# groupeLIAMG/ttcr

Hardware: AMD Instinct MI355X
Metric: Mnodes/s per sweep-iteration (512^3 fp32 grid, first-order FSM) (higher is better)
Workload: dtype f32

## Files before the change

### include/ttcr_amd.h

```cpp
#ifndef TTCR_AMD_H
#define TTCR_AMD_H

#include <stddef.h>
#include <stdint.h>

#ifdef __cplusplus
extern "C" {
#endif

typedef struct ttcr_fsm_grid ttcr_fsm_grid;

enum { TTCR_F32 = 0, TTCR_F64 = 1 };

enum {
    TTCR_OK = 0,
    TTCR_ERR_VALUE = 1,
    TTCR_ERR_RUNTIME = 2,
    TTCR_ERR_DEVICE = 3,
    TTCR_ERR_UNSUPPORTED = 4
};

int ttcr_fsm_device_count(void);

const char* ttcr_fsm_last_error(void);
// ... 142 lines not shown
                        int dtt_on_device, void* dfields, int df_on_device, int schedule, int* passes);
int ttcr_fsm_rjoint_gn(const ttcr_fsm_adjoint* t, const void* v, int v_on_device, const void* v_rcv, int vr_on_device, const void* row_weight,
                       int rw_on_device, const double* rcv_scale, void* out, int out_on_device, void* out_rcv, int or_on_device,
                       int schedule, int* passes_jvp, int* passes_vjp);
int ttcr_fsm_rjoint_solve(ttcr_fsm_adjoint* t, const void* rhs, int rhs_on_device, const void* rhs_rcv, int rr_on_device,
                          const void* row_weight, int rw_on_device, double smooth, const double* smooth_weights, double damp,
                          const double* rcv_damp, const double* rcv_scale, int maxiter, double rtol, int schedule, void* x,
                          int x_on_device, void* x_rcv, int xr_on_device, int* status, int* iterations, double* rho, double* pq, int* passes);
int ttcr_fsm_rcv_release(ttcr_fsm_adjoint* t);

int ttcr_fsm_loc_geometry(const ttcr_fsm_adjoint* t, int* nn, double* dx, double* origin);
int ttcr_fsm_loc_shape(const ttcr_fsm_adjoint* t, int* node_tile, int* hypo_chunk, int* staged);
int ttcr_fsm_loc_grid(const ttcr_fsm_adjoint* t, size_t n_hypo, const long long* hypo_off, const int* pick_field, const double* pick_time,
                      const double* pick_weight, const int* box, long long* node_out, double* t0_out, double* misfit_out,
                      void* volume_out, int volume_on_device);
int ttcr_fsm_loc_release(ttcr_fsm_adjoint* t);

int ttcr_fsm_dd_pairs(ttcr_fsm_adjoint* t, const int* set_row_a, const int* set_row_b, size_t set_n_pairs, size_t* n_pairs, int* row_a,
                      int* row_b, long long* bad_pair);
int ttcr_fsm_dd_apply(const ttcr_fsm_adjoint* t, int mode, const void* x, int x_on_device, const void* row_weight, int rw_on_device,
                      const void* pair_weight, int pw_on_device, void* out, int out_on_device);
int ttcr_fsm_dd_gn(const ttcr_fsm_adjoint* t, int system, int newton, const void* v, int v_on_device, const void* v_b, int vb_on_device,
                   const void* row_weight, int rw_on_device, const void* pair_weight, int pw_on_device, const double* b_scale, void* out,
                   int out_on_device, void* out_b, int ob_on_device, int schedule, int* passes_jvp, int* passes_vjp);
int ttcr_fsm_dd_solve(ttcr_fsm_adjoint* t, int system, const void* rhs, int rhs_on_device, const void* rhs_b, int rb_on_device,
                      const void* row_weight, int rw_on_device, const void* pair_weight, int pw_on_device, double smooth,
                      const double* smooth_weights, double damp, const double* b_damp, const double* b_scale, const void* x0,
                      int x0_on_device, int maxiter, double rtol, int newton, int schedule, void* x, int x_on_device, void* x_b,
                      int xb_on_device, int* status, int* iterations, double* rho, double* pq, int* passes);
int ttcr_fsm_dd_release(ttcr_fsm_adjoint* t);

int ttcr_fsm_raytrace_l(ttcr_fsm_grid* g, int slot, int n_tx, const void* tx, const void* t0, int n_rx,
                        const void* rx, void* tt_out, int with_rays);
int ttcr_fsm_slot_l_size(const ttcr_fsm_grid* g, int slot, size_t* n_rows, size_t* nnz);
int ttcr_fsm_get_slot_l(const ttcr_fsm_grid* g, int slot, long long* row_off, long long* cell, void* v);
int ttcr_fsm_raytrace_multi_l(ttcr_fsm_grid* g, int n_src, const int* tx_off, const void* tx, const void* t0, const int* rx_off,
                              const void* rx, void* tt_out, int with_rays);
int ttcr_fsm_multi_l_size(const ttcr_fsm_grid* g, size_t* n_rows, size_t* nnz);
int ttcr_fsm_get_multi_l(const ttcr_fsm_grid* g, long long* row_off, long long* cell, void* v);

typedef struct {
    double sweep_ms;
    double total_ms;
    long long kernel_launches;
    long long node_updates;
    long long evaluated_updates;
    int iterations;
    int n_sources;
} ttcr_fsm_timing;
int ttcr_fsm_last_timing(const ttcr_fsm_grid* g, ttcr_fsm_timing* out);
int ttcr_fsm_stopping_stats(const ttcr_fsm_grid* g, long long* reference_sums, long long* reference_sums_missed, long long* rounds);
int ttcr_fsm_prefill_swaps(const ttcr_fsm_grid* g, long long* swaps);
int ttcr_fsm_prefill_inline_fills(const ttcr_fsm_grid* g, long long* fills);
int ttcr_fsm_reference_change(ttcr_fsm_grid* g, const void* times, const void* field, int parallel, void* out);
int ttcr_fsm_last_kernel(const ttcr_fsm_grid* g, char* buf, size_t n);
int ttcr_fsm_unit_order(int dim, int dtype, int stage, int by_time, uint32_t nnx, uint32_t nny, uint32_t nnz, uint32_t* out,
                        size_t capacity, size_t* n_units);
int ttcr_fsm_prefill_slice(int dtype, uint64_t n_el, uint32_t n_tickets, uint32_t ticket, uint64_t* slice_len, uint64_t* begin, uint64_t* end);
const char* ttcr_fsm_build_id(void);

#ifdef __cplusplus
}
#endif
#endif
```

### ttcr_amd/_lib.py

```python
import ctypes as C
import os

HERE = os.path.dirname(os.path.abspath(__file__))
LIB_PATH = os.environ.get("TTCR_AMD_LIB") or os.path.join(HERE, "libttcr_amd.so")

TTCR_F32, TTCR_F64 = 0, 1
OK, ERR_VALUE, ERR_RUNTIME, ERR_DEVICE, ERR_UNSUPPORTED = 0, 1, 2, 3, 4

_P = C.c_void_p
_U32 = C.c_uint32
_D = C.c_double
_I = C.c_int


class Timing(C.Structure):
    _fields_ = [("sweep_ms", C.c_double), ("total_ms", C.c_double), ("kernel_launches", C.c_longlong),
                ("node_updates", C.c_longlong), ("evaluated_updates", C.c_longlong), ("iterations", C.c_int),
                ("n_sources", C.c_int)]


SYMBOLS = {
    "ttcr_fsm_device_count": (_I, []),
    "ttcr_fsm_last_error": (C.c_char_p, []),
    "ttcr_fsm3d_create": (_I, [C.POINTER(_P), _I, _I, _U32, _U32, _U32, _D, _D, _D, _D, _D, _I, _I, _I, _I, _I]),
    "ttcr_fsm2d_create": (_I, [C.POINTER(_P), _I, _I, _U32, _U32, _D, _D, _D, _D, _D, _I, _I, _I, _I, _I]),
    "ttcr_fsm3d_create_multi": (_I, [C.POINTER(_P), _I, _I, _U32, _U32, _U32, _D, _D, _D, _D, _D, _I, _I, _I, _I, C.POINTER(_I), _I]),
    "ttcr_fsm2d_create_multi": (_I, [C.POINTER(_P), _I, _I, _U32, _U32, _D, _D, _D, _D, _D, _I, _I, _I, _I, C.POINTER(_I), _I]),
    "ttcr_fsm_n_devices": (_I, [_P]),
    "ttcr_fsm_destroy": (None, [_P]),
    "ttcr_fsm_set_slowness": (_I, [_P, _P, C.c_size_t]),
    "ttcr_fsm_set_slowness_device": (_I, [_P, _P, C.c_size_t]),
    "ttcr_fsm_set_slowness_c_order": (_I, [_P, _P, C.c_size_t]),
    "ttcr_fsm_get_slowness": (_I, [_P, _P, C.c_size_t]),
    "ttcr_fsm_raytrace": (_I, [_P, _I, _I, _P, _P, _I, _P, _P]),
    "ttcr_fsm_raytrace_multi": (_I, [_P, _I, _P, _P, _P, _P, _P, _P]),
    "ttcr_fsm_get_tt": (_I, [_P, _I, _P, C.c_size_t]),
    "ttcr_fsm_get_tt_device": (_I, [_P, _I, C.POINTER(_P)]),
    "ttcr_fsm_get_tt_device_view": (_I, [_P, _I, C.POINTER(_P), C.POINTER(C.c_size_t)]),
    "ttcr_fsm_interp": (_I, [_P, _I, _I, _P, _P]),
    "ttcr_fsm_compute_slowness": (_I, [_P, _I, _P, _I, _P]),
    "ttcr_fsm_get_niter": (_I, [_P, _I, C.POINTER(_I), C.POINTER(_I)]),
    "ttcr_fsm_get_changes": (_I, [_P, _I, C.POINTER(_D), _I, C.POINTER(_D), _I]),
    "ttcr_fsm_get_reference_changes": (_I, [_P, _I, C.POINTER(_D), _I, C.POINTER(_D), _I]),
    "ttcr_fsm_n_slots": (_I, [_P]),
    "ttcr_fsm_n_nodes": (C.c_size_t, [_P]),
    "ttcr_fsm_n_cells": (C.c_size_t, [_P]),
    "ttcr_fsm_set_option": (_I, [_P, C.c_char_p, _D]),
    "ttcr_fsm_last_timing": (_I, [_P, C.POINTER(Timing)]),
    "ttcr_fsm_last_kernel": (_I, [_P, C.c_char_p, C.c_size_t]),
    "ttcr_fsm_build_id": (C.c_char_p, []),
    "ttcr_fsm_unit_order": (_I, [_I, _I, _I, _I, _U32, _U32, _U32, C.POINTER(_U32), C.c_size_t, C.POINTER(C.c_size_t)]),
    "ttcr_fsm_stopping_stats": (_I, [_P, C.POINTER(C.c_longlong), C.POINTER(C.c_longlong), C.POINTER(C.c_longlong)]),
    "ttcr_fsm_prefill_swaps": (_I, [_P, C.POINTER(C.c_longlong)]),
    "ttcr_fsm_prefill_inline_fills": (_I, [_P, C.POINTER(C.c_longlong)]),
    "ttcr_fsm_prefill_slice": (_I, [_I, C.c_uint64, _U32, _U32, C.POINTER(C.c_uint64), C.POINTER(C.c_uint64), C.POINTER(C.c_uint64)]),
    "ttcr_fsm_reference_change": (_I, [_P, C.c_void_p, C.c_void_p, C.c_int, C.c_void_p]),
    "ttcr_fsm_rays_size": (_I, [_P, C.POINTER(C.c_size_t), C.POINTER(C.c_size_t)]),
    "ttcr_fsm_get_rays": (_I, [_P, _P, _P]),
    "ttcr_fsm_raytrace_rays": (_I, [_P, _I, _I, _P, _P, _I, _P, _P]),
    "ttcr_fsm_slot_rays_size": (_I, [_P, _I, C.POINTER(C.c_size_t), C.POINTER(C.c_size_t)]),
    "ttcr_fsm_get_slot_rays": (_I, [_P, _I, _P, _P]),
    "ttcr_fsm_raytrace_m": (_I, [_P, _I, _I, _P, _P, _I, _P, _P]),
    "ttcr_fsm_raytrace_rm": (_I, [_P, _I, _I, _P, _P, _I, _P, _P]),
    "ttcr_fsm_raytrace_multi_m": (_I, [_P, _I, _P, _P, _P, _P, _P, _P, _I]),
    "ttcr_fsm_multi_m_size": (_I, [_P, C.POINTER(C.c_size_t), C.POINTER(C.c_size_t)]),
    "ttcr_fsm_get_multi_m": (_I, [_P, _P, _P, _P]),
    "ttcr_fsm_raytrace_multi_tape": (_I, [_P, _I, _P, _P, _P, _P, _P, _P, C.POINTER(_P)]),
    "ttcr_fsm_tape_size": (_I, [_P, C.POINTER(C.c_size_t), C.POINTER(C.c_size_t), C.POINTER(C.c_size_t)]),
    "ttcr_fsm_tape_bytes": (_I, [_P, C.POINTER(C.c_size_t)]),
    "ttcr_fsm_tape_device": (_I, [_P, C.POINTER(_I)]),
    "ttcr_fsm_tape_get_csr": (_I, [_P, _P, _P, _P]),
    "ttcr_fsm_tape_vjp": (_I, [_P, _P, _I, _P, _I]),
    "ttcr_fsm_tape_free": (_I, [_P]),
    "ttcr_fsm_raytrace_multi_adjoint": (_I, [_P, _I, _P, _P, _P, _P, _P, _P, C.POINTER(_P)]),
    "ttcr_fsm_raytrace_multi_adjoint_cells": (_I, [_P, _I, _P, _P, _P, _P, _P, _P, C.POINTER(_P)]),
    "ttcr_fsm_adjoint_model": (_I, [_P, C.POINTER(_I), C.POINTER(C.c_size_t), C.POINTER(C.c_size_t)]),
    "ttcr_fsm_adjoint_size": (_I, [_P, C.POINTER(C.c_size_t), C.POINTER(C.c_size_t), C.POINTER(C.c_size_t)]),
    "ttcr_fsm_adjoint_bytes": (_I, [_P, C.POINTER(C.c_size_t)]),
    "ttcr_fsm_adjoint_device": (_I, [_P, C.POINTER(_I)]),
    "ttcr_fsm_adjoint_get_field": (_I, [_P, C.c_size_t, _P]),
    "ttcr_fsm_adjoint_vjp": (_I, [_P, _P, _I, _P, _I, _P, _I, _I, C.POINTER(_I)]),
    "ttcr_fsm_adjoint_jvp": (_I, [_P, _P, _I, _P, _I, _P, _I, _I, C.POINTER(_I)]),
    "ttcr_fsm_adjoint_gn": (_I, [_P, _P, _I, _P, _I, _P, _I, _I, C.POINTER(_I), C.POINTER(_I)]),
    "ttcr_fsm_adjoint_points": (_I, [_P, C.POINTER(C.c_size_t), _P]),
    "ttcr_fsm_adjoint_jvp_source": (_I, [_P, _P, _I, _I, _P, _I, _P, _I, _I, C.POINTER(_I)]),
    "ttcr_fsm_adjoint_vjp_source": (_I, [_P, _P, _I, _P, _I, _P, _I, _P, _I, _I, C.POINTER(_I)]),
    "ttcr_fsm_adjoint_hold": (_I, [_P, _P, _I, _P, _I, _P, _I, _I, C.POINTER(_I)]),
    "ttcr_fsm_adjoint_release": (_I, [_P]),
    "ttcr_fsm_adjoint_hvp": (_I, [_P, _P, _I, _P, _I, _I, C.POINTER(_I), C.POINTER(_I)]),
    "ttcr_fsm_adjoint_newton": (_I, [_P, _P, _I, _P, _I, _P, _I, _I, C.POINTER(_I), C.POINTER(_I)]),
    "ttcr_fsm_adjoint_jvp_block": (_I, [_P, _I, _P, _I, _P, _I, _P, _I, _I, C.POINTER(_I)]),
    "ttcr_fsm_adjoint_vjp_block": (_I, [_P, _I, _P, _I, _P, _I, _I, C.POINTER(_I)]),
    "ttcr_fsm_adjoint_gn_block": (_I, [_P, _I, _P, _I, _P, _I, _I, _P, _I, _I, C.POINTER(_I), C.POINTER(_I)]),
    "ttcr_fsm_adjoint_block_release": (_I, [_P]),
    "ttcr_fsm_adjoint_free": (_I, [_P]),
    "ttcr_fsm_normal_tile_edge": (_I, [_I]),
    "ttcr_fsm_normal_smooth": (_I, [_P, _P, _I, C.POINTER(_D), _P, _I]),
    "ttcr_fsm_normal_dot": (_I, [_P, _P, _I, _P, _I, C.POINTER(_D)]),
    "ttcr_fsm_normal_solve": (_I, [_P, _P, _I, _P, _I, _D, C.POINTER(_D), _D, _P, _I, _I, _D, _I, _I, _P, _I, C.POINTER(_I),
                                   C.POINTER(_I), C.POINTER(_D), C.POINTER(_D), C.POINTER(_I)]),
    "ttcr_fsm_normal_release": (_I, [_P]),
    "ttcr_fsm_joint_jvp": (_I, [_P, _P, _I, _P, _I, _P, _I, _P, _I, _I, C.POINTER(_I)]),
    "ttcr_fsm_joint_gn": (_I, [_P, _P, _I, _P, _I, _P, _I, C.POINTER(_D), _P, _I, _P, _I, _I, C.POINTER(_I), C.POINTER(_I)]),
    "ttcr_fsm_joint_solve": (_I, [_P, _P, _I, _P, _I, _P, _I, _D, C.POINTER(_D), _D, C.POINTER(_D), C.POINTER(_D), _I, _D, _I, _P, _I, _P, _I,
                                  C.POINTER(_I), C.POINTER(_I), C.POINTER(_D), C.POINTER(_D), C.POINTER(_I)]),
    "ttcr_fsm_joint_release": (_I, [_P]),
    "ttcr_fsm_rcv_eval": (_I, [_P, C.c_size_t, _P, _I, C.POINTER(_I), _P, _I, _P, _I]),
# ... 84 lines not shown
```

### ttcr_amd/csrc/fsm_capi.hip

```cpp
#include <hip/hip_runtime.h>

#include <algorithm>
#include <atomic>
#include <chrono>
#include <condition_variable>
#include <cmath>
#include <cstdio>
#include <cstdlib>
#include <cstring>
#include <limits>
#include <map>
#include <memory>
#include <mutex>
#include <sstream>
#include <stdexcept>
#include <string>
#include <thread>
#include <vector>

#include "../../include/ttcr_amd.h"
#include "fsm_kernels.h"
#include "fsm_fast_api.h"
#include "fsm_tape_api.h"
#include "fsm_adjoint_api.h"
// ... 78 lines not shown
                                     void* tt_out, TapeRows& out) = 0;
    virtual void raytrace_multi_adjoint(int n_src, const int* tx_off, const void* tx, const void* t0, const int* rx_off, const void* rx,
                                        void* tt_out, AdjSink& sink) = 0;
    virtual void adjoint_geometry(int* nn3, double* spacing, bool wrt_cells) const = 0;
    AdjSink* adj_sink = nullptr;
    std::vector<int> adj_src, adj_row;
    virtual void raytrace_l(int slot, int n_tx, const void* tx, const void* t0, int n_rx, const void* rx, void* tt_out, bool with_rays) = 0;
    virtual void slot_l_size(int slot, size_t* n_rows, size_t* nnz) const = 0;
    virtual void get_slot_l(int slot, long long* row_off, long long* cell, void* v) const = 0;
    virtual void raytrace_multi_l(int n_src, const int* tx_off, const void* tx, const void* t0, const int* rx_off, const void* rx,
                                  void* tt_out, bool with_rays) = 0;
    virtual void multi_l_size(size_t* n_rows, size_t* nnz) const = 0;
    virtual void get_multi_l(long long* row_off, long long* cell, void* v) const = 0;
    virtual void validate_points(int n_tx, const void* tx, int n_rx, const void* rx) = 0;
    struct Request {
        int slot, n_tx, n_rx;
        const void *tx, *t0, *rx;
        void* tt;
        int status = TTCR_OK;
        std::string err;
        bool done = false;
    };
    std::mutex q_mu;
    std::condition_variable q_cv;
    std::vector<Request*> queue;
    bool leader_active = false;
    bool had_company = false;
    std::atomic<int> combine_window_us{200};
    size_t elem_size = 4;
    virtual void get_tt(int slot, void* out, size_t n) = 0;
    virtual void* tt_device(int slot) = 0;
    virtual void* tt_device_view(int slot, size_t* stride) = 0;
    std::mutex mu;
    virtual void interp(int slot, int n, const void* pts, void* out) = 0;
    virtual void compute_slowness(int n, const void* pts, bool translated, void* out) = 0;
    virtual void rays_size(size_t* n_rays, size_t* n_points) const = 0;
    virtual void get_rays(long long* offsets, void* pts) const = 0;
    int dim = 3, dtype = 0, n_slots = 1, device = 0;
    size_t n_nodes = 0, n_cells = 0;
    std::vector<int> niter, niterw;
    std::vector<int> phys;
    int P(int slot) const { return phys.empty() ? slot : phys[slot]; }
    int stopping_shortcuts = 3;
    int stopping_rule = 1;
    long long reference_sums = 0, reference_sums_missed = 0;
    long long refsum_rounds = 0;
    virtual void stopping_stats(long long* sums, long long* missed, long long* rounds) const {
        if (sums) *sums = reference_sums;
        if (missed) *missed = reference_sums_missed;
        if (rounds) *rounds = refsum_rounds;
    }
    virtual void reference_change_host(const void* times, const void* field, bool parallel, void* out) = 0;
    int pair_by_distance = 1;
    virtual void set_pair_layout(int) {}
    virtual long long prefill_inline_count() const { return 0; }
    virtual long long prefill_swap_count() const { return 0; }
    int lone_chunk = 16;
    int arith = 0;
    int prefill = -1;
    int prefill_inline = -1;
    std::vector<std::vector<double>> change_hist, change_histw;
    std::vector<std::vector<double>> ref_hist, ref_histw;
    virtual void get_reference_changes(int slot, double* first, int n_first, double* wen, int n_weno) const {
        if (slot < 0 || slot >= n_slots) throw ValueError("Thread number is larger than number of threads");
        slot = P(slot);
        for (int q = 0; q < n_first; ++q) first[q] = (!ref_hist.empty() && q < (int)ref_hist[slot].size()) ? ref_hist[slot][q] : std::nan("");
        for (int q = 0; q < n_weno; ++q) wen[q] = (!ref_histw.empty() && q < (int)ref_histw[slot].size()) ? ref_histw[slot][q] : std::nan("");
    }
    virtual void get_changes(int slot, double* first, int n_first, double* wen, int n_weno) const {
        if (slot < 0 || slot >= n_slots) throw ValueError("Thread number is larger than number of threads");
        slot = P(slot);
        for (int q = 0; q < n_first; ++q) first[q] = (!change_hist.empty() && q < (int)change_hist[slot].size()) ? change_hist[slot][q] : 0.0;
        for (int q = 0; q < n_weno; ++q) wen[q] = (!change_histw.empty() && q < (int)change_histw[slot].size()) ? change_histw[slot][q] : 0.0;
    }
    bool weno = false;
    bool sweep45_strips = false;
    bool rotated = false;
    int ttrp = 0, interp_vel = 0;
    std::atomic<int> return_rays{0};
    int fixed_iters = 0, max_batch = 0, use_graph = 1;
    int skip = -1;
    int mode = 2;
    Timing timing;
    std::string last_kernel;
    virtual std::string kernel_name() const { return last_kernel; }
    long walk_step_limit = 1000000;
    long walk_records = 0;
    long walk_room(long extent) const { return std::min<long>(walk_step_limit, walk_records > 0 ? walk_records : extent); }
    virtual void apply_option(const std::string& k, double value) {
        if (k == "fixed_iters") fixed_iters = (int)value;
        else if (k == "max_batch") max_batch = (int)value;
        else if (k == "use_graph") use_graph = (int)value;
        else if (k == "combine_window_us") combine_window_us = (int)value;
        else if (k == "mode") mode = (int)value;
        else if (k == "skip") skip = (int)value;
        else if (k == "tt_from_rp") ttrp = value != 0;
        else if (k == "interp_vel") interp_vel = value != 0;
        else if (k == "return_rays") return_rays = value != 0;
        else if (k == "pair_sources") pair_by_distance = value != 0;
        else if (k == "pair_layout") {
            if (value != -1 && value != 0 && value != 1) throw ValueError("option 'pair_layout': -1 (default), 0 or 1");
            set_pair_layout((int)value);
        }
        else if (k == "stopping_rule") stopping_rule = (int)value;
        else if (k == "stopping_shortcuts") { if (value < 0 || value > 3 || value != (double)(int)value) throw ValueError("option stopping_shortcuts: 0 ... 3"); stopping_shortcuts = (int)value; }
        else if (k == "prefill") {
            if (value != -1 && value != 0 && value != 1) throw ValueError("option 'prefill': -1 (default), 0 or 1");
            prefill = (int)value;
        } else if (k == "prefill_inline") {
            if (value != -1 && value != 0 && value != 1) throw ValueError("option 'prefill_inline': -1 (default), 0 or 1");
            prefill_inline = (int)value;
        } else if (k == "lone_chunk") {
            if (value != 8 && value != 16) throw ValueError("option 'lone_chunk': 8 or 16");
            lone_chunk = (int)value;
        }
        else if (k == "arith") {
            if (value != 0 && value != 1 && value != 2)
                throw ValueError("option 'arith': 0 (the reference's arithmetic), 1 (tolerance-grade fp32 where it stays within 1e-5 s RMS) or 2 (the WENO stage as well)");
            arith = (int)value;
        }
        else if (k == "walk_records") {
            if (value != 0 && !(value >= 1 && value <= (double)walk_step_limit && value == (double)(long)value))
                throw ValueError("option 'walk_records': 0 (default) or a whole number from 1 to the step limit of a walk");
            walk_records = (long)value;
        }
        else throw ValueError("unknown option '" + k + "'");
    }
    virtual void get_niter(int slot, int* it, int* itw) const {
        if (slot < 0 || slot >= n_slots) throw ValueError("Thread number is larger than number of threads");
        if (it) *it = niter[P(slot)];
        if (itw) *itw = niterw[P(slot)];
    }
};

template <typename T, int DIM> struct TileCfg;
#ifndef FSM_PJ3
#define FSM_PJ3 16
#endif
#ifndef FSM_PK3
#define FSM_PK3 16
#endif
template <> struct TileCfg<float, 3> { static constexpr int PJ = FSM_PJ3, PK = FSM_PK3, BL = 16; };
template <> struct TileCfg<double, 3> { static constexpr int PJ = 16, PK = 8, BL = 16; };
#ifndef FSM_PJ2
#define FSM_PJ2 64
#endif
#ifndef FSM_CHUNK2
#define FSM_CHUNK2 16
#endif
template <> struct TileCfg<float, 2> { static constexpr int PJ = FSM_PJ2, PK = 1, BL = 32; };
template <> struct TileCfg<double, 2> { static constexpr int PJ = FSM_PJ2, PK = 1, BL = 32; };
template <typename T, int DIM> struct ChunkCfg { static constexpr int C = DIM == 3 ? FSM_CHUNK3 : FSM_CHUNK2; };

template <typename T>
class GridT : public GridBase {
   public:
    uint32_t ncx, ncy, ncz;
    T dx, dz, xmin, ymin, zmin, xmax, ymax, zmax, ox = 0, oy = 0, oz = 0;
    T epsilon;
    int nitermax;
    bool cell, translate;
    bool have_slowness = false;

    hipStream_t stream = nullptr;
    hipEvent_t ev0 = nullptr, ev1 = nullptr;
    DevBuf<T> d_s, d_cells, d_tt, d_rx, d_out;
    DevBuf<T> d_tt_alt;
    bool alt_filled = false;
    hipStream_t fill_stream = nullptr;
    hipEvent_t ev_fill = nullptr;
    long long prefill_swaps = 0;
    long long prefill_swap_count() const override { return prefill_swaps; }
    long long prefill_inline_fills = 0;
    long long prefill_inline_count() const override { return prefill_inline_fills; }
    void set_pair_layout(int v) override { pair_layout = v; }
    DevBuf<int> d_rslot;
    DevBuf<RaySrc> d_rdesc;
    int weno_ch4_min = 8;
    int weno_c16_below = 3;
    int f64_c16_below = 5;
    int pre_min = 2;
    size_t xs_lds_bytes = 40000;
    int xs_lds_below = 2;
    size_t xs_dyn_lds(int batch) const { return (dim == 3 && stage == 0 && batch < xs_lds_below) ? xs_lds_bytes : 0; }
    int time_order_below = 1 << 30;
    DevBuf<T> d_gather;
    DevBuf<T> d_rsrc, d_rt0;
    DevBuf<int> d_rstat;
    DevBuf<T> d_ssh;
    size_t ssh_stride = 0;
    DevBuf<uint32_t> d_mask;
    DevBuf<int> d_bbox, d_slots, d_lmask;
    int* h_lmask = nullptr;
    DevBuf<uint32_t> d_tiles;
    std::vector<int> tile_off, tile_cnt;
    DevBuf<double> d_change;
    DevBuf<unsigned long long> d_prof;
    size_t prof_words = 0;
    DevBuf<uint32_t> d_order;
    DevBuf<uint32_t> d_order_xs[2][2];
    DevBuf<int> d_sync;
    int n_patches = 0;
    int* h_abort = nullptr;
    DevBuf<int> d_stamp;
    DevBuf<unsigned long long> d_cmap;
    int cmap_words = 1;
    DevBuf<unsigned long long> d_sw;
    int sw_sweeps = 0;
    DevBuf<int> d_iter;
    DevBuf<unsigned long long> d_evals;
    int* h_iter = nullptr;
    unsigned launch_epoch = 1;
    bool sync_clean = true;
    size_t sync_words = 0;
    unsigned long long* h_evals = nullptr;
    int nbf = 0, nbj = 0, nbk = 0;
    size_t n_bricks = 0;
    DevBuf<InitPoint<T>> d_pts;
    double* h_change = nullptr;
    int* h_slots = nullptr;
    size_t mask_words = 0;
    SweepGeom geom;
    int n_launch = 0;
    hipGraph_t graphs[2] = {nullptr, nullptr};
    hipGraphExec_t graph_execs[2] = {nullptr, nullptr};
    int graph_batches[2] = {0, 0}, graph_modes[2] = {-1, -1};

    GridT(int dim_, bool cell_, uint32_t nx, uint32_t ny, uint32_t nz, double ddx, double ddz, double minx,
          double miny, double minz, double eps, int maxit, int nslots, bool translate_, int dev, bool weno_) {
        dim = dim_;
        weno = weno_;
        dtype = sizeof(T) == 4 ? TTCR_F32 : TTCR_F64;
        elem_size = sizeof(T);
        cell = cell_;
        translate = translate_;
        ncx = nx; ncy = ny; ncz = nz;
        dx = (T)ddx;
        dz = (T)ddz;
        xmin = (T)minx; ymin = (T)miny; zmin = (T)minz;
        xmax = xmin + (T)nx * dx;
        if (dim == 3) {
            ymax = ymin + (T)ny * dx;
            zmax = zmin + (T)nz * dx;
        } else {
            ymax = ymin;
            zmax = zmin + (T)nz * dz;
        }
        if (translate) {
            ox = xmin; oy = ymin; oz = zmin;
            xmax -= xmin; ymax -= ymin; zmax -= zmin;
            xmin = 0; ymin = 0; zmin = 0;
        }
        n_nodes = dim == 3 ? (size_t)(nx + 1) * (ny + 1) * (nz + 1) : (size_t)(nx + 1) * (nz + 1);
        n_cells = dim == 3 ? (size_t)nx * ny * nz : (size_t)nx * nz;
        if (n_nodes >= (1ull << 32)) throw ValueError("grid too large: node index must fit uint32 (reference T2)");
        epsilon = (T)eps;
        epsilon *= (T)n_nodes;
        nitermax = maxit;
        n_slots = nslots;
        niter.assign(n_slots, 0);
        niterw.assign(n_slots, 0);
        phys.resize(n_slots);
        for (int q = 0; q < n_slots; ++q) phys[q] = q;
        max_batch = n_slots;
        device = dev;
        HIP_CHECK(hipSetDevice(device));
        {
            int cus = 0;
            HIP_CHECK(hipDeviceGetAttribute(&cus, hipDeviceAttributeMultiprocessorCount, device));
            persist_wgs = 8 * std::max(cus, 1);
        }
        HIP_CHECK(hipStreamCreateWithFlags(&stream, hipStreamNonBlocking));
        HIP_CHECK(hipEventCreate(&ev0));
        HIP_CHECK(hipEventCreate(&ev1));
        d_s.reserve(n_nodes, 64);
        {
            long long pair_units_min = 6144;
            if (const char* e = std::getenv("TTCR_FSM_PAIR_UNITS")) pair_units_min = std::atoll(e);
            const long long patches = dim == 3 ? (long long)((ny + 1 + TileCfg<T, 3>::PJ - 1) / TileCfg<T, 3>::PJ) * ((nz + 1 + TileCfg<T, 3>::PK - 1) / TileCfg<T, 3>::PK) : 0;
            NS = (n_slots >= 2 && dim == 3 && !weno && (long long)n_slots * patches > pair_units_min) ? 2 : 1;
            ns_window = NS == 2 && (long long)n_slots * patches <= (5 * pair_units_min) / 2;
        }
        if (const char* e = std::getenv("TTCR_FSM_PAIR")) { NS = (std::atoi(e) != 0 && n_slots >= 2) ? 2 : 1; ns_window = false; }
        if (const char* e = std::getenv("TTCR_FSM_LAYOUT_LO")) layout_lo = std::atof(e);
        if (const char* e = std::getenv("TTCR_FSM_LAYOUT_HI")) layout_hi = std::atof(e);
        d_tt.reserve(n_nodes * tt_fields(), 64);
        mask_words = (n_nodes + 31) / 32;
        d_mask.reserve(mask_words * (size_t)n_slots);
        d_bbox.reserve(6 * (size_t)n_slots);
        d_slots.reserve(n_slots);
        d_lmask.reserve(n_slots);
        HIP_CHECK(hipHostMalloc((void**)&h_lmask, sizeof(int) * n_slots));
        d_change.reserve(n_slots);
        if (std::getenv("TTCR_FSM_PROF")) {
            prof_words = 8 + 4 * (size_t)(1 << 20);
            d_prof.reserve(prof_words);
            HIP_CHECK(hipMemset(d_prof.p, 0, prof_words * sizeof(unsigned long long)));
        }
        HIP_CHECK(hipHostMalloc((void**)&h_change, sizeof(double) * n_slots));
        HIP_CHECK(hipHostMalloc((void**)&h_slots, sizeof(int) * n_slots));
        HIP_CHECK(hipHostMalloc((void**)&h_abort, sizeof(int)));
        *h_abort = 0;
        HIP_CHECK(hipHostMalloc((void**)&h_iter, 2 * sizeof(int)));
        HIP_CHECK(hipHostMalloc((void**)&h_evals, sizeof(unsigned long long) * n_slots));
        HIP_CHECK(hipMemsetAsync(d_tt.p, 0, n_nodes * tt_fields() * sizeof(T), stream));

        if (dim == 3) {
            using C = TileCfg<T, 3>;
            geom.NF = nx + 1; geom.NJ = ny + 1; geom.NK = nz + 1;
            geom.npj = (geom.NJ + C::PJ - 1) / C::PJ;
            geom.npk = (geom.NK + C::PK - 1) / C::PK;
            n_launch = count_launches(C::BL);
        } else {
            using C = TileCfg<T, 2>;
            geom.NF = nz + 1; geom.NJ = nx + 1; geom.NK = 1;
            geom.npj = (geom.NJ + C::PJ - 1) / C::PJ;
            geom.npk = 1;
            n_launch = count_launches(C::BL);
        }
        geom.n_nodes = (uint32_t)n_nodes;
        geom.M = (std::max(geom.NF, geom.NJ) + 1) & ~1;
        geom.MP = geom.M + FSM_XPAD;
        geom.SR = dim == 3 ? ((geom.NJ + 15) / 16) * 32 : 0;
        ssh_stride = (size_t)geom.NK * shear_plane(geom);
        if ((double)(dim == 3 ? 16 : 1) * (double)shear_plane(geom) * sizeof(T) >= 4294967296.0)
            throw ValueError("grid too large for the slowness offsets of the sweep kernel (16 planes of max(nx, ny) x ny nodes must stay below 4 GiB)");
        d_ssh.reserve(ssh_stride * (dim == 3 ? 4 : 2));
        HIP_CHECK(hipMemsetAsync(d_ssh.p, 0, ssh_stride * (dim == 3 ? 4 : 2) * sizeof(T), stream));
        if (dim == 3) build_tile_lists(TileCfg<T, 3>::PJ, TileCfg<T, 3>::PK, TileCfg<T, 3>::BL);
        else build_tile_lists(TileCfg<T, 2>::PJ, TileCfg<T, 2>::PK, TileCfg<T, 2>::BL);
        build_persistent_lists();
        nbf = (geom.NF + FSM_BRICK - 1) / FSM_BRICK;
        nbj = (geom.NJ + FSM_BRICK - 1) / FSM_BRICK;
        nbk = (geom.NK + FSM_BRICK - 1) / FSM_BRICK;
        n_bricks = (size_t)nbf * nbj * nbk;
        d_stamp.reserve(n_bricks * n_slots);
        {
            const int PJ = dim == 3 ? TileCfg<T, 3>::PJ : TileCfg<T, 2>::PJ, PK = dim == 3 ? TileCfg<T, 3>::PK : 1;
            const int max_chunks = (geom.NF + 2 * (PJ + PK)) / 4 + 4;
            cmap_words = max_chunks / 32 + 1;
            d_cmap.reserve((size_t)n_patches * n_slots * (dim == 3 ? 8 : 4) * 2 * cmap_words);
            HIP_CHECK(hipMemset(d_cmap.p, 0, (size_t)n_patches * n_slots * (dim == 3 ? 8 : 4) * 2 * cmap_words * sizeof(unsigned long long)));
            sw_sweeps = (dim == 3 ? 8 : 4) * (2 * std::min(nitermax, 256) + 2);
            d_sw.reserve((size_t)sw_sweeps * n_slots);
        }
        d_iter.reserve(2);
        d_evals.reserve(n_slots);
        if (dim == 2)
            HIP_CHECK(hipFuncSetAttribute(reinterpret_cast<const void*>(&fsm_sweep45_rows<T>),
                                          hipFuncAttributeMaxDynamicSharedMemorySize, 156 * 1024));
        if (const char* e = std::getenv("TTCR_FSM_SWEEP45")) sweep45_strips = std::string(e) == "strips";
        if (const char* e = std::getenv("TTCR_FSM_WENO_CH4_MIN")) weno_ch4_min = std::atoi(e);
        if (const char* e = std::getenv("TTCR_FSM_WENO_C16_BELOW")) weno_c16_below = std::atoi(e);
        if (const char* e = std::getenv("TTCR_FSM_F64_C16_BELOW")) f64_c16_below = std::atoi(e);
        if (const char* e = std::getenv("TTCR_FSM_TIME_ORDER_BELOW")) time_order_below = std::atoi(e);
        if (const char* e = std::getenv("TTCR_FSM_PRE_MIN")) pre_min = std::atoi(e);
        if (const char* e = std::getenv("TTCR_FSM_SKIP")) skip = std::atoi(e);
        if (const char* e = std::getenv("TTCR_FSM_SKIP_UNITS")) skip_units_min = std::atoi(e);
        if (const char* e = std::getenv("TTCR_FSM_SKIP_PROBE_UNITS")) skip_probe_min = std::atoi(e);
        if (const char* e = std::getenv("TTCR_FSM_RS_FIELDS")) rs_fields_max = (size_t)std::max(0, std::atoi(e));
        if (const char* e = std::getenv("TTCR_FSM_WGS")) persist_wgs = std::atoi(e);
        if (const char* e = std::getenv("TTCR_FSM_XS_LDS")) xs_lds_bytes = (size_t)std::atol(e);
        if (const char* e = std::getenv("TTCR_FSM_XS_LDS_BELOW")) xs_lds_below = std::atoi(e);
        if (const char* e = std::getenv("TTCR_FSM_MODE")) mode = std::atoi(e);
        if (const char* e = std::getenv("TTCR_FSM_PREFILL")) prefill = std::atoi(e);
        if (const char* e = std::getenv("TTCR_FSM_LONE_CHUNK")) lone_chunk = std::atoi(e) == 8 ? 8 : 16;
        if (const char* e = std::getenv("TTCR_FSM_ARITH")) arith = std::max(0, std::min(2, std::atoi(e)));
    }

    void build_persistent_lists() {
        const std::vector<uint32_t> order = fsm_diag_order(geom.npj, geom.npk);
        n_patches = (int)order.size();
        d_order.reserve(order.size());
        HIP_CHECK(hipMemcpy(d_order.p, order.data(), order.size() * sizeof(uint32_t), hipMemcpyHostToDevice));
        sync_words = 8 + (size_t)n_patches * n_slots * (dim == 3 ? 8 : 4);
        d_sync.reserve(sync_words);
        HIP_CHECK(hipMemset(d_sync.p, 0, sync_words * sizeof(int)));
        if (geom.npj >= (1 << 14) || geom.npk >= (1 << 14)) throw ValueError("grid too large for the patch index of the sweep kernel");
        for (int st = 0; st < 2; ++st)
            for (int tm = 0; tm < 2; ++tm) {
                const std::vector<uint32_t> xs = xs_order(order, tm != 0, st == 0 ? 1 : 2);
                d_order_xs[st][tm].reserve(xs.size());
                HIP_CHECK(hipMemcpy(d_order_xs[st][tm].p, xs.data(), xs.size() * sizeof(uint32_t), hipMemcpyHostToDevice));
            }
    }

    std::vector<uint32_t> xs_order(const std::vector<uint32_t>& diag_order, bool by_time, int H) const {
        const int PJ = dim == 3 ? TileCfg<T, 3>::PJ : TileCfg<T, 2>::PJ, PK = dim == 3 ? TileCfg<T, 3>::PK : 1;
        const int C = dim == 3 ? ChunkCfg<T, 3>::C : ChunkCfg<T, 2>::C;
        return fsm_xs_order(dim, geom.NF, geom.NJ, geom.NK, PJ, PK, C, H, by_time, diag_order);
    }

    template <int DIM, int H>
    void launch_sweeps_persistent(int batch) {
        constexpr int C0 = ChunkCfg<T, DIM>::C;
        if constexpr (DIM == 3 && C0 == 8) {
            const int below = H == 2 ? weno_c16_below : sizeof(T) == 4 ? std::numeric_limits<int>::max() : f64_c16_below;
            if (NS == 1 && mode == 2 && (lone_chunk == 16 || fast_now<H>()) && batch < below) {
                launch_sweeps_persistent_ns<DIM, H, 1, 16, true>(batch);
                return;
            }
        }
        if (H == 2 && DIM == 3 && NS == 2 && batch >= weno_ch4_min && C0 == 8) {
            if (NS == 2) launch_sweeps_persistent_ns<DIM, H, 2, (H == 2 && DIM == 3) ? 4 : C0>(batch);
            else launch_sweeps_persistent_ns<DIM, H, 1, (H == 2 && DIM == 3) ? 4 : C0>(batch);
        } else {
            if (NS == 2) launch_sweeps_persistent_ns<DIM, H, 2, C0>(batch); else launch_sweeps_persistent_ns<DIM, H, 1, C0>(batch);
        }
    }

    template <int DIM, int H, int NSV, int CH, bool XS_ONLY = false>
    void launch_sweeps_persistent_ns(int batch) {
        using C = TileCfg<T, DIM>;
        PersistArgs<T> pa;
        SweepArgs<T>& a = pa.s;
        constexpr bool NO_PRE = CH == 16 && H == 1 && DIM == 3;
        const size_t dyn_lds = NO_PRE ? 0 : xs_dyn_lds(batch);
        a.tt = d_tt.p;
        a.ts = NS;
        a.lmask = d_lmask.p;
        a.frozen = d_mask.p;
        a.bbox = d_bbox.p;
        a.change = d_change.p;
        a.slots = d_slots.p;
        a.tiles = nullptr;
        a.g = geom;
        a.prof = d_prof.p;
        a.mask_words = (uint32_t)mask_words;
        a.dx = dx;
        a.dz = dz;
        a.w = 0;
        a.variant = DIM == 3 ? 0 : (dx == dz ? 1 : 2);
        pa.order = d_order.p;
        pa.sync = d_sync.p;
        pa.n_patches = n_patches;
        pa.batch = batch;
        pa.timeout_ticks = 300000000ull;
        pa.stamp = d_stamp.p;
        pa.iter_ptr = d_iter.p;
        pa.evals = d_evals.p;
        pa.nbf = nbf; pa.nbj = nbj; pa.nbk = nbk;
        pa.ndir = DIM == 3 ? 8 : 4;
        pa.skip = skip_now(batch) ? (std::getenv("TTCR_FSM_SKIP_ALL_DIRTY") ? 2 : 1) : 0;
        pa.cmap = d_cmap.p;
        pa.cw = cmap_words;
        pa.sw = std::getenv("TTCR_FSM_NO_SW") ? nullptr : d_sw.p;
        pa.n_sw_groups = n_groups();
        pa.n_sw_sweeps = sw_sweeps;
        pa.fill_dst = nullptr;
        pa.fill_slice = 0;
        pa.fill_n = 0;

        const size_t wg_cap = (fsm_looped(DIM == 3, H) && persist_wgs > 0) ? (size_t)persist_wgs : ~(size_t)0;
        const dim3 block(C::PJ * C::PK), grid((unsigned)std::min<size_t>((size_t)n_patches * batch, wg_cap));
        const int ndir = DIM == 3 ? 8 : 4;
        {
            const bool pre_ = mode == 2 && !NO_PRE && (DIM == 2 || batch >= pre_min || dyn_lds > 0);
            char nm[160];
            std::snprintf(nm, sizeof nm, "fsm_sweep_persistent<%s,%d,%d,%d,%s,%s,%d,%d,%s,%s>", sizeof(T) == 4 ? "float" : "double", C::PJ, C::PK, CH,
                          DIM == 3 ? "true" : "false", skip_now(batch) ? "true" : "false", H, NSV, mode == 2 ? "true" : "false", pre_ ? "true" : "false");
            last_kernel = nm;
        }
        if (mode == 2) {
            pa.ssh = d_ssh.p;
            pa.ssh_stride = ssh_stride;
            pa.dir = 0;
            a.rf = a.rj = a.rk = a.rev = 0;
            a.s_sheared = nullptr;
            pa.timeout_ticks = 1000000000ull;
            const dim3 gridx((unsigned)std::min<size_t>((size_t)n_patches * batch * ndir, wg_cap));
            pa.order = d_order_xs[H == 2 ? 1 : 0][batch < time_order_below ? 1 : 0].p;
            const bool pre = DIM == 2 || batch >= pre_min || dyn_lds > 0;
            if (fill_arm) {
                pa.fill_dst = d_tt_alt.p;
                pa.fill_n = n_nodes * tt_fields();
                pa.fill_slice = fsm_fill_slice_len(pa.fill_n, (size_t)n_patches * batch * ndir, 16 / sizeof(T));
                fill_arm = false;
                fill_in_flight = true;
            }
            if constexpr (std::is_same<T, float>::value) {
                if (fast_now<H>() && (H == 1 || NSV == 1)) {
                    const FastCfg fc{H, DIM, NSV, CH, skip_now(batch), NO_PRE ? false : pre};
                    last_kernel.insert(last_kernel.size() - 1, ",1");
                    const hipError_t e = fsm_fast_launch(pa, fc, gridx.x, dyn_lds, stream);
                    if (e == hipErrorInvalidValue) throw std::logic_error("arith = 1: no such kernel (" + last_kernel + ")");
                    HIP_CHECK(e);
                    return;
                }
            }
            if constexpr (NO_PRE) {
                (void)pre;
                if (skip_now(batch))
                    fsm_sweep_persistent<T, C::PJ, C::PK, CH, DIM == 3, true, H, NSV, true><<<gridx, block, dyn_lds, stream>>>(pa);
                else
                    fsm_sweep_persistent<T, C::PJ, C::PK, CH, DIM == 3, false, H, NSV, true><<<gridx, block, dyn_lds, stream>>>(pa);
            } else {
                if (skip_now(batch) && pre)
                    fsm_sweep_persistent<T, C::PJ, C::PK, CH, DIM == 3, true, H, NSV, true, true><<<gridx, block, dyn_lds, stream>>>(pa);
// ... 248 lines not shown
                q.i = (int)(c / ncz);
                q.k = (int)(c - (long)q.i * ncz);
            }
        }
        return q;
    }

    template <int DIM>
    void launch_sweeps(int batch) {
        using C = TileCfg<T, DIM>;
        if (fast_now<1>()) throw ValueError("option 'arith' = 1 needs whole-iteration launches (option 'mode' = 2)");
        SweepArgs<T> a;
        a.tt = d_tt.p;
        a.ts = NS;
        a.lmask = nullptr;
        a.frozen = d_mask.p;
        a.bbox = d_bbox.p;
        a.change = d_change.p;
        a.slots = d_slots.p;
        a.g = geom;
        a.prof = d_prof.p;
        a.mask_words = (uint32_t)mask_words;
        a.dx = dx;
        a.dz = dz;
        a.variant = DIM == 3 ? 0 : (dx == dz ? 1 : 2);
        const dim3 block(C::PJ * C::PK);
        const int ndir = DIM == 3 ? 8 : 4;
        static const int RX2[4] = {0, 1, 1, 0}, RZ2[4] = {0, 0, 1, 1};
        for (int d = 0; d < ndir; ++d) {
            int fam;
            if (DIM == 3) {
                a.rf = d & 1; a.rj = (d >> 1) & 1; a.rk = (d >> 2) & 1;
                a.rev = a.rk;
                fam = (a.rf ^ a.rk) | ((a.rj ^ a.rk) << 1);
            } else {
                a.rj = RX2[d]; a.rf = RZ2[d]; a.rk = 0;
                a.rev = a.rj;
                fam = a.rf ^ a.rj;
            }
            a.s_sheared = d_ssh.p + (size_t)fam * ssh_stride;
            for (int w = 0; w < n_launch; ++w) {
                if (tile_cnt[w] == 0) continue;
                a.w = w;
                a.tiles = d_tiles.p + tile_off[w];
                const dim3 grid(tile_cnt[w], 1, batch);
                fsm_sweep_tile<T, C::PJ, C::PK, C::BL, DIM == 3><<<grid, block, 0, stream>>>(a);
            }
        }
        last_kernel = std::string("fsm_sweep_tile<") + (sizeof(T) == 4 ? "float" : "double") + "," + std::to_string(C::PJ) + "," + std::to_string(C::PK) + "," + std::to_string(C::BL) + "," + (DIM == 3 ? "true" : "false") + ">";
        HIP_CHECK(hipGetLastError());
    }

    int NS = 1;
    bool ns_window = false;
    int pair_layout = -1;
    double last_eval_frac = -1;
    double layout_lo = 0.55, layout_hi = 0.70;
    void choose_layout() {
        if (!ns_window) return;
        int want = NS;
        if (pair_layout >= 0) want = pair_layout ? 2 : 1;
        else if (last_eval_frac >= 0) want = NS == 2 ? (last_eval_frac < layout_lo ? 1 : 2) : (last_eval_frac > layout_hi ? 2 : 1);
        if (want == NS) return;
        NS = want;
        graph_batches[0] = graph_batches[1] = -1;
        for (int q = 0; q < n_slots; ++q) phys[q] = q;
    }
    int n_groups() const { return (n_slots + NS - 1) / NS; }
    size_t tt_fields() const { return (size_t)n_slots + ((ns_window || NS == 2) ? (size_t)(n_slots & 1) : 0); }
    T* tt_ptr(int slot) const { return d_tt.p + (size_t)(slot / NS) * n_nodes * NS + slot % NS; }
    template <int H>
    bool fast_now() const { return sizeof(T) == 4 && (arith == 2 || (arith == 1 && !weno)); }
    bool prefill_on() const {
        if (prefill >= 0) return prefill != 0;
        const size_t bytes = n_nodes * tt_fields() * sizeof(T);
        if (bytes < ((size_t)64 << 20)) return false;
        size_t free_b = 0, total_b = 0;
        if (hipMemGetInfo(&free_b, &total_b) != hipSuccess) return false;
        return d_tt_alt.p || (2 * bytes <= total_b / 2 && bytes + ((size_t)1 << 30) <= free_b);
    }
    bool fill_arm = false;
    bool fill_in_flight = false;
    bool inline_fill_now(int entries) const {
        if (prefill_inline == 0 || !d_tt_alt.p || d_tt_alt.n < n_nodes * tt_fields()) return false;
        if (mode != 2 || stage != 0 || use_graph >= 2) return false;
        if (prefill_inline == 1) return true;
        return dim == 3 && !fast_now<1>() && (long long)n_patches * entries >= skip_units_min;
    }

    int stage = 0;
    int skip_units_min = 2048;
    int skip_probe_min = 1024;
    bool probe_skip = true;
    int probe_off_calls = 0;
    int persist_wgs = 2048;
    bool in_probe_window(int entries) const {
        const long long u = (long long)n_patches * entries;
        return dim == 3 && sizeof(T) == 4 && u >= skip_probe_min && u < skip_units_min;
    }
    int skip_default(int entries) const {
        if (dim != 3) return 1;
        if (stage == 1) return 1;
        if (in_probe_window(entries)) return probe_skip ? 1 : 0;
        return (long long)n_patches * entries >= skip_units_min ? 1 : 0;
    }
    bool persistent_now() const { return mode >= 1 || stage == 1; }
// ... 1 lines not shown
        const int on = skip < 0 ? skip_default(entries) : skip;
        const bool fits = (long long)geom.NF + geom.NJ + geom.NK < (1ll << 22) && nbf <= 32 * FSM_SLAB_WORDS;
        return on != 0 && fits && !(dim == 2 && rotated && !weno && dx == dz);
    }

    void launch_sweep45(int batch) {
        Sweep45Args<T> a;
        a.tt = d_tt.p;
        a.s = d_s.p;
        a.frozen = d_mask.p;
        a.change = d_change.p;
        a.slots = d_slots.p;
        a.lmask = d_lmask.p;
        a.ts = NS;
        a.by_group = persistent_now() ? 1 : 0;
        a.nnx = (int)ncx + 1;
        a.nnz = (int)ncz + 1;
        a.n_nodes = n_nodes;
        a.mask_words = (uint32_t)mask_words;
        a.dx = dx;
        const int blocks = a.by_group ? batch * NS : batch;
        const size_t smem = 4 * ((size_t)a.nnz + 2) * sizeof(T);
        if (smem <= 156 * 1024 && !sweep45_strips) {
            const int threads = (int)std::min<size_t>(1024, (((size_t)a.nnz + 63) / 64) * 64);
            fsm_sweep45_rows<T><<<blocks, threads, smem, stream>>>(a);
        } else {
            constexpr int NTMAX = sizeof(T) == 4 ? 1024 : 512;
            if (a.nnx + 2 <= 256) fsm_sweep45<T, 256><<<blocks, 256, 0, stream>>>(a);
            else fsm_sweep45<T, NTMAX><<<blocks, NTMAX, 0, stream>>>(a);
        }
        HIP_CHECK(hipGetLastError());
    }

    void issue_sweeps(int batch) {
        issue_sweeps_axis(batch);
        if (dim == 2 && rotated && !weno && dx == dz) launch_sweep45(batch);
    }

    void issue_sweeps_axis(int batch) {
        if (stage == 1) {
            if (dim == 3) launch_sweeps_persistent<3, 2>(batch); else launch_sweeps_persistent<2, 2>(batch);
        } else if (mode >= 1) {
            if (dim == 3) launch_sweeps_persistent<3, 1>(batch); else launch_sweeps_persistent<2, 1>(batch);
        } else {
            if (dim == 3) launch_sweeps<3>(batch); else launch_sweeps<2>(batch);
        }
    }

    void run_iteration(int batch) {
        const int ndir = dim == 3 ? 8 : 4;
        if (use_graph >= 2 || (use_graph == 1 && !persistent_now())) {
            hipGraph_t& graph = graphs[stage];
            hipGraphExec_t& graph_exec = graph_execs[stage];
            const int key = mode * 2 + (skip_now(batch) ? 1 : 0);
            if (!graph_exec || graph_batches[stage] != batch || graph_modes[stage] != key) {
                if (graph_exec) { (void)hipGraphExecDestroy(graph_exec); graph_exec = nullptr; }
                if (graph) { (void)hipGraphDestroy(graph); graph = nullptr; }
                HIP_CHECK(hipStreamBeginCapture(stream, hipStreamCaptureModeThreadLocal));
                try {
                    issue_sweeps(batch);
                } catch (...) {
                    hipGraph_t junk = nullptr;
                    (void)hipStreamEndCapture(stream, &junk);
                    if (junk) (void)hipGraphDestroy(junk);
                    throw;
                }
                HIP_CHECK(hipStreamEndCapture(stream, &graph));
                HIP_CHECK(hipGraphInstantiate(&graph_exec, graph, nullptr, nullptr, 0));
                graph_batches[stage] = batch;
                graph_modes[stage] = key;
            }
            HIP_CHECK(hipGraphLaunch(graph_exec, stream));
        } else {
            issue_sweeps(batch);
        }
        timing.launches += mode == 2 ? 1 : persistent_now() ? (long long)ndir : (long long)ndir * n_launch;
    }

    std::map<int, DevBuf<T>> snap;
    std::vector<int> snap_iter;
    std::vector<double> prev_change;
    std::vector<double> prev2_change;
    bool snap_always = false;
    std::vector<int> snap_T;
    bool stamps_ok = false;
    int iter_T = 0;
    bool stamps_live_for(int entries) const { return (stopping_shortcuts & 1) && dim == 3 && !weno && persistent_now() && skip_now(entries) && n_nodes * (size_t)NS < ((size_t)1 << 31); }
    void terms_pass(int gi, T* x0, T* x1, unsigned* c0, unsigned* c1, int since_T) {
        RefTermsArgs<T> ta;
        ta.cur = d_tt.p + (size_t)gi * n_nodes * NS;
        ta.old = snap[gi].p;
        ta.x[0] = x0; ta.x[1] = x1;
        ta.cnt[0] = c0; ta.cnt[1] = c1;
        ta.n_nodes = (uint32_t)n_nodes;
        ta.ns = NS;
        constexpr int V = 16 / (int)sizeof(T);
        const size_t n_el = n_nodes * (size_t)NS;
        const bool vec = n_el % V == 0 && ((uintptr_t)ta.cur | (uintptr_t)ta.old) % 16 == 0;
        const int nodes_per_vec = vec ? std::max(1, V / NS) : 1;
        const bool bricks = since_T >= 0 && geom.NF % nodes_per_vec == 0;
        ta.stamp = bricks ? d_stamp.p + (size_t)gi * n_bricks : nullptr;
        ta.thr = (dim == 3 ? 8 : 4) * since_T + 1;
        ta.NF = geom.NF; ta.NJ = geom.NJ; ta.nbf = nbf; ta.nbj = nbj;
        const unsigned nblk = (unsigned)((n_nodes + FSM_REFSUM_CB - 1) / FSM_REFSUM_CB);
        const unsigned blocks = std::min(nblk, 8192u);
        if (vec) fsm_refsum_terms<T, V><<<blocks, 256, 0, stream>>>(ta);
        else fsm_refsum_terms<T, 1><<<blocks, 256, 0, stream>>>(ta);
// ... 232 lines not shown
                    }
                    need.push_back(f);
                }
                if (!need.empty()) {
                    fsm_refsum_compact<T><<<cgrid, 256, 0, stream>>>(d_rs_x.p, d_rs_xc.p, pitch, n_nodes, d_rs_cnt.p, d_rs_off.p, nblk);
                    HIP_CHECK(hipGetLastError());
                    std::vector<const T*> c2(need.size()), o2(need.size(), nullptr);
                    std::vector<unsigned long long> m2(need.size());
                    for (size_t q = 0; q < need.size(); ++q) { c2[q] = curs[need[q]]; m2[q] = h_m[need[q]]; }
                    d_rs_n2.reserve(std::max<size_t>(need.size(), 64));
                    HIP_CHECK(hipMemcpyAsync(d_rs_n2.p, m2.data(), need.size() * sizeof(unsigned long long), hipMemcpyHostToDevice, stream));
                    const std::vector<T> r = reference_changes(c2, o2, 1, false, epsilon, d_rs_n2.p, &m2);
                    for (size_t q = 0; q < need.size(); ++q) { res[a0 + need[q]] = r[q]; res_known[a0 + need[q]] = 1; }
                }
                a0 = a1;
            }
        }
        for (size_t a = 0; a < ask.size(); ++a) {
            go[ask[a]] = res_known[a] ? res[a] >= epsilon : res_go[a] != 0;
            if (res_known[a]) ref_change_last[active[ask[a]]] = (double)res[a];
            ++reference_sums;
        }
        return go;
    }
    std::vector<double> ref_change_last;

    bool host_prof = std::getenv("TTCR_FSM_HOST_PROF") != nullptr;
    std::chrono::steady_clock::time_point hp_t = std::chrono::steady_clock::now();
    void hp_mark(const char* what) {
        if (!host_prof) return;
        const auto now = std::chrono::steady_clock::now();
        std::fprintf(stderr, "[host] %-28s %8.3f ms\n", what, std::chrono::duration<double, std::milli>(now - hp_t).count());
        hp_t = now;
    }
    void solve_batch(const std::vector<int>& slot_ids, const std::vector<int>& src_ids, const int* tx_off,
                     const T* tx, const T* t0) {
        const int nb = (int)slot_ids.size();
        hp_mark("(before solve_batch)");
        const int nc = ncoord();
        const long long node_updates_before = timing.node_updates;
        size_t tot_pts = 0;
        for (int b = 0; b < nb; ++b) tot_pts += tx_off[src_ids[b] + 1] - tx_off[src_ids[b]];
        std::vector<InitPoint<T>> pts;
        pts.reserve(tot_pts);
        std::vector<size_t> first(nb);
        for (int b = 0; b < nb; ++b) {
            first[b] = pts.size();
            for (int n = tx_off[src_ids[b]]; n < tx_off[src_ids[b] + 1]; ++n) pts.push_back(locate(tx + (size_t)nc * n, t0[n]));
        }
        d_pts.reserve(std::max<size_t>(tot_pts, 1));
        HIP_CHECK(hipMemcpyAsync(d_pts.p, pts.data(), pts.size() * sizeof(InitPoint<T>), hipMemcpyHostToDevice, stream));
        for (int b = 0; b < nb; ++b)
            HIP_CHECK(hipMemsetAsync(d_stamp.p + (size_t)(slot_ids[b] / NS) * n_bricks, 0xFF, n_bricks * sizeof(int), stream));
        std::vector<char> group_filled(n_groups(), 0);
        const bool all_slots = nb == n_slots && prefill_on();
        fill_arm = fill_in_flight = false;
        bool inline_filled = false;
        if (all_slots && alt_filled) {
            HIP_CHECK(hipStreamWaitEvent(stream, ev_fill, 0));
            std::swap(d_tt.p, d_tt_alt.p);
            std::swap(d_tt.n, d_tt_alt.n);
            std::swap(d_tt.guard, d_tt_alt.guard);
            alt_filled = false;
            ++prefill_swaps;
            graph_batches[0] = graph_batches[1] = -1;
            std::fill(group_filled.begin(), group_filled.end(), 1);
        }
        if (NS > 1) {
            std::vector<int> cnt(n_groups(), 0);
            for (int b = 0; b < nb; ++b) cnt[slot_ids[b] / NS] += 1;
            for (int gi = 0; gi < n_groups(); ++gi) {
                if (cnt[gi] != NS || group_filled[gi]) continue;
                const size_t n_el = n_nodes * (size_t)NS;
                const int blocks = (int)std::min<size_t>((n_el + 255) / 256, 16384);
                fsm_fill<T><<<blocks, 256, 0, stream>>>(d_tt.p + (size_t)gi * n_el, n_el, real_traits<T>::max(), 1);
                group_filled[gi] = 1;
            }
        }
        for (int b = 0; b < nb; ++b) {
            const int slot = slot_ids[b];
            T* tt = tt_ptr(slot);
            const int blocks = (int)std::min<size_t>((n_nodes + 255) / 256, 8192);
            if (!group_filled[slot / NS]) fsm_fill<T><<<blocks, 256, 0, stream>>>(tt, n_nodes, real_traits<T>::max(), NS);
            HIP_CHECK(hipMemsetAsync(d_mask.p + (size_t)slot * mask_words, 0, mask_words * sizeof(uint32_t), stream));
            InitArgs<T> ia;
            ia.tt = tt;
            ia.ts = NS;
            ia.slowness = d_s.p;
            ia.frozen = d_mask.p + (size_t)slot * mask_words;
            ia.bbox = d_bbox.p + 6 * (size_t)slot;
            ia.pts = d_pts.p + first[b];
            ia.n_pts = tx_off[src_ids[b] + 1] - tx_off[src_ids[b]];
            ia.npts = weno ? 2 : 1;
            ia.nnx = ncx + 1;
            ia.nny = dim == 3 ? ncy + 1 : 1;
            ia.nnz = ncz + 1;
            ia.dx = dx; ia.dz = dz; ia.xmin = xmin; ia.ymin = ymin; ia.zmin = zmin;
            ia.dim = dim;
            ia.stamp = d_stamp.p + (size_t)(slot / NS) * n_bricks;
            ia.nbf = nbf; ia.nbj = nbj; ia.nbk = nbk;
            fsm_init_source<T><<<1, 128, 0, stream>>>(ia);
            niter[slot] = 0;
            niterw[slot] = 0;
            if (change_hist.empty()) { change_hist.resize(n_slots); change_histw.resize(n_slots); }
            if (ref_hist.empty()) { ref_hist.resize(n_slots); ref_histw.resize(n_slots); }
            change_hist[slot].clear();
            change_histw[slot].clear();
            ref_hist[slot].clear();
            ref_histw[slot].clear();
        }
        HIP_CHECK(hipGetLastError());
        hp_mark("reinit + initFSM issued");
        HIP_CHECK(hipStreamSynchronize(stream));
        hp_mark("reinit + initFSM done");

        const int maxit = fixed_iters > 0 ? fixed_iters : nitermax;
        const int ndir = dim == 3 ? 8 : 4;
        if (!sync_clean || launch_epoch > 0xfffff000u) {
            HIP_CHECK(hipMemsetAsync(d_sync.p, 0, sync_words * sizeof(int), stream));
            HIP_CHECK(hipMemsetAsync(d_cmap.p, 0, (size_t)n_patches * n_slots * ndir * 2 * cmap_words * sizeof(unsigned long long), stream));
            HIP_CHECK(hipStreamSynchronize(stream));
            launch_epoch = 1;
        }
        sync_clean = false;
        snap_always = false;
        if (persistent_now() || weno) HIP_CHECK(hipMemsetAsync(d_sync.p + 8, 0, (sync_words - 8) * sizeof(int), stream));
        if (persistent_now() || weno) HIP_CHECK(hipMemsetAsync(d_sync.p + 4, 0, sizeof(int), stream));
        HIP_CHECK(hipMemsetAsync(d_evals.p, 0, sizeof(unsigned long long) * n_slots, stream));
        HIP_CHECK(hipMemsetAsync(d_sw.p, 0, sizeof(unsigned long long) * (size_t)sw_sweeps * n_groups(), stream));
        HIP_CHECK(hipEventRecord(ev0, stream));
        int it_total = 0;
        for (stage = 0; stage < (weno ? 2 : 1); ++stage) {
            std::vector<int> active(slot_ids);
            int it = 0;
            prev_change.assign(n_slots, std::numeric_limits<double>::infinity());
            prev2_change.assign(n_slots, std::numeric_limits<double>::infinity());
            snap_iter.assign(n_groups(), 0);
            snap_T.assign(n_groups(), -1);
            stamps_ok = false;
            if ((int)ref_change_last.size() != n_slots) ref_change_last.assign(n_slots, std::nan(""));
            std::vector<int> groups;
            for (int s2 : slot_ids)
                if (groups.empty() || groups.back() != s2 / NS) groups.push_back(s2 / NS);
            while (!active.empty() && it < maxit) {
                int n_entries;
                if (persistent_now()) {
                    n_entries = (int)groups.size();
                    for (int b = 0; b < n_entries; ++b) {
                        int m2 = 0;
                        for (int s2 : active)
                            if (s2 / NS == groups[b]) m2 |= 1 << (s2 % NS);
                        h_slots[b] = m2 ? groups[b] : -1;
                        h_lmask[b] = m2;
                    }
                } else {
                    n_entries = nb;
                    for (int b = 0; b < nb; ++b) { h_slots[b] = b < (int)active.size() ? active[b] : -1; h_lmask[b] = 1; }
                }
                HIP_CHECK(hipMemcpyAsync(d_slots.p, h_slots, sizeof(int) * n_entries, hipMemcpyHostToDevice, stream));
                HIP_CHECK(hipMemcpyAsync(d_lmask.p, h_lmask, sizeof(int) * n_entries, hipMemcpyHostToDevice, stream));
                HIP_CHECK(hipMemsetAsync(d_change.p, 0, sizeof(double) * n_slots, stream));
                iter_T = it_total;
                snapshots_before_iteration(active, it + 1);
                if (host_prof) { HIP_CHECK(hipStreamSynchronize(stream)); hp_mark("snapshots"); }
                stamps_ok = (it == 0 ? true : stamps_ok) && stamps_live_for(n_entries);
                h_iter[0] = it_total;
                h_iter[1] = (int)launch_epoch;
                launch_epoch += (persistent_now() && mode == 2) ? 1u : (unsigned)ndir;
                HIP_CHECK(hipMemcpyAsync(d_iter.p, h_iter, 2 * sizeof(int), hipMemcpyHostToDevice, stream));
                fill_arm = it_total == 0 && all_slots && !alt_filled && inline_fill_now(n_entries);
                run_iteration(n_entries);
                fill_arm = false;
                HIP_CHECK(hipMemcpyAsync(h_change, d_change.p, sizeof(double) * n_slots, hipMemcpyDeviceToHost, stream));
                if (persistent_now()) HIP_CHECK(hipMemcpyAsync(h_abort, d_sync.p + 4, sizeof(int), hipMemcpyDeviceToHost, stream));
                HIP_CHECK(hipStreamSynchronize(stream));
                hp_mark("sweep-iteration");
                if (persistent_now() && *h_abort) {
                    HIP_CHECK(hipMemsetAsync(d_sync.p + 4, 0, sizeof(int), stream));
                    stage = 0;
                    throw DeviceError("persistent sweep kernel: a patch timed out waiting for its upwind neighbour");
                }
                if (fill_in_flight) { inline_filled = true; fill_in_flight = false; }
                ++it;
                ++it_total;
                std::vector<int> next;
                if (fixed_iters > 0) ref_change_last.assign(n_slots, std::nan(""));
                const std::vector<char> go = fixed_iters > 0 ? std::vector<char>(active.size(), 1) : decide_go_on(active, it);
                hp_mark("stopping rule");
                for (size_t q = 0; q < active.size(); ++q) {
                    const int s2 = active[q];
                    (stage == 0 ? niter : niterw)[s2] = it;
                    (stage == 0 ? change_hist : change_histw)[s2].push_back(h_change[s2]);
                    (stage == 0 ? ref_hist : ref_histw)[s2].push_back((int)ref_change_last.size() == n_slots ? ref_change_last[s2] : std::nan(""));
                    timing.node_updates += (long long)n_nodes * ndir;
                    prev2_change[s2] = prev_change[s2];
                    prev_change[s2] = h_change[s2];
                    if (go[q]) next.push_back(s2);
                }
                active.swap(next);
            }
            timing.iterations = std::max(timing.iterations, it_total);
            if (stage == 0 && weno) {
                HIP_CHECK(hipMemsetAsync(d_sw.p, 0, sizeof(unsigned long long) * (size_t)sw_sweeps * n_groups(), stream));
                for (int s2 : slot_ids)
                    HIP_CHECK(hipMemsetD32Async((hipDeviceptr_t)(d_stamp.p + (size_t)(s2 / NS) * n_bricks), it_total * (dim == 3 ? 8 : 4),
                                                n_bricks, stream));
            }
        }
        if (std::getenv("TTCR_FSM_DEBUG_SW")) {
            std::vector<unsigned long long> h((size_t)std::min(sw_sweeps, 40) * n_groups());
            HIP_CHECK(hipMemcpy(h.data(), d_sw.p, h.size() * sizeof(unsigned long long), hipMemcpyDeviceToHost));
            for (size_t q = 0; q < h.size(); ++q) std::fprintf(stderr, "%s%u/%u", q % n_groups() == 0 ? "\n[sw] " : " ", (unsigned)h[q], (unsigned)(h[q] >> 32));
            std::fprintf(stderr, "\n");
        }
        const bool was_persistent = mode >= 1 || weno;
        stage = 0;
        sync_clean = true;
        HIP_CHECK(hipEventRecord(ev1, stream));
        if (all_slots && inline_filled) {
            alt_filled = true;
            ++prefill_inline_fills;
        } else if (all_slots) {
            const size_t n_el = n_nodes * tt_fields();
            if (!fill_stream) {
                int lo = 0, hi = 0;
                HIP_CHECK(hipDeviceGetStreamPriorityRange(&lo, &hi));
                HIP_CHECK(hipStreamCreateWithPriority(&fill_stream, hipStreamNonBlocking, lo));
                HIP_CHECK(hipEventCreateWithFlags(&ev_fill, hipEventDisableTiming));
            }
            bool have_alt = true;
            try {
                d_tt_alt.reserve(n_el, 64);
            } catch (const DeviceError&) {
                (void)hipGetLastError();
                have_alt = false;
                prefill = 0;
            }
            if (have_alt) {
            HIP_CHECK(hipStreamWaitEvent(fill_stream, ev1, 0));
            const int blocks = (int)std::min<size_t>((n_el + 255) / 256, 16384);
            fsm_fill<T><<<blocks, 256, 0, fill_stream>>>(d_tt_alt.p, n_el, real_traits<T>::max(), 1);
            HIP_CHECK(hipEventRecord(ev_fill, fill_stream));
            alt_filled = true;
            }
        }
        HIP_CHECK(hipEventSynchronize(ev1));
        if (d_prof.p) {
            unsigned long long h[8];
            HIP_CHECK(hipMemcpy(h, d_prof.p, sizeof(h), hipMemcpyDeviceToHost));
            if (const char* tp = std::getenv("TTCR_FSM_PROF_TRACE")) {
                std::vector<unsigned long long> tr(prof_words);
                HIP_CHECK(hipMemcpy(tr.data(), d_prof.p, prof_words * sizeof(unsigned long long), hipMemcpyDeviceToHost));
                if (FILE* f = std::fopen(tp, "wb")) { std::fwrite(tr.data() + 8, sizeof(unsigned long long), prof_words - 8, f); std::fclose(f); }
            }
            HIP_CHECK(hipMemset(d_prof.p, 0, sizeof(h)));
            if (mode >= 1) {
                const double nb_ = (double)std::max<unsigned long long>(h[7], 1), nu_ = (double)std::max<unsigned long long>(h[6], 1);
                std::fprintf(stderr, "[ttcr_amd prof] units %llu chunks %llu  per unit (us): start %.2f total %.2f | per chunk (us): top %.3f  wait %.3f  stage %.3f  march %.3f  writeback %.3f\n",
                             h[6], h[7], h[5] * 0.01 / nu_, (h[0] + h[1] + h[2] + h[3] + h[4] + h[5]) * 0.01 / nu_, h[0] * 0.01 / nb_,
                             h[1] * 0.01 / nb_, h[2] * 0.01 / nb_, h[3] * 0.01 / nb_, h[4] * 0.01 / nb_);
            } else {
                const double nb_ = (double)std::max<unsigned long long>(h[4], 1);
                std::fprintf(stderr, "[ttcr_amd prof] tiles %llu  per tile (us): setup %.2f  stage %.2f  march %.2f  writeback %.2f\n",
                             h[4], h[0] * 0.01 / nb_, h[1] * 0.01 / nb_, h[2] * 0.01 / nb_, h[3] * 0.01 / nb_);
            }
        }
        hp_mark("after the iterations");
        float ms = 0;
        HIP_CHECK(hipEventElapsedTime(&ms, ev0, ev1));
        timing.sweep_ms += ms;
        const long long evaluated_before = timing.evaluated_updates;
        if (was_persistent) {
            HIP_CHECK(hipMemcpy(h_evals, d_evals.p, sizeof(unsigned long long) * n_slots, hipMemcpyDeviceToHost));
            for (int s2 : slot_ids) timing.evaluated_updates += (long long)h_evals[s2];
        } else {
            timing.evaluated_updates += timing.node_updates - node_updates_before;
        }
        const bool skipped_now = skip_now(n_groups());
        if (nb == n_slots && timing.node_updates > node_updates_before && skipped_now)
            last_eval_frac = (double)(timing.evaluated_updates - evaluated_before) / (double)(timing.node_updates - node_updates_before);
        if (skip < 0 && !weno && in_probe_window((nb + NS - 1) / NS) && timing.node_updates > node_updates_before) {
            if (skipped_now) {
                probe_skip = (double)(timing.evaluated_updates - evaluated_before) / (double)(timing.node_updates - node_updates_before) < 0.6;
                probe_off_calls = 0;
            } else if (++probe_off_calls >= 8) {
                probe_skip = true;
                probe_off_calls = 0;
            }
        }
    }

    void interp(int slot, int n, const void* pts, void* out) override {
        HIP_CHECK(hipSetDevice(device));
        check_slot(slot);
        if (n <= 0) return;
        const int nc = ncoord();
        std::vector<T> p((const T*)pts, (const T*)pts + (size_t)nc * n);
        if (translate)
            for (int m = 0; m < n; ++m) { p[3 * m] -= ox; p[3 * m + 1] -= oy; p[3 * m + 2] -= oz; }
        check_pts(p.data(), n);
        interp_grid_coords(P(slot), n, p.data(), (T*)out);
    }

    void compute_slowness(int n, const void* pts, bool translated, void* out) override {
        HIP_CHECK(hipSetDevice(device));
        if (!have_slowness) throw std::runtime_error("Error: slowness has not been assigned.");
        if (n <= 0) return;
        const int nc = ncoord();
        std::vector<T> p((const T*)pts, (const T*)pts + (size_t)nc * n);
        if (translate && !translated)
            for (int m = 0; m < n; ++m) { p[3 * m] -= ox; p[3 * m + 1] -= oy; p[3 * m + 2] -= oz; }
        check_pts(p.data(), n);
        d_rx.reserve((size_t)nc * n);
        d_out.reserve(n);
        HIP_CHECK(hipMemcpyAsync(d_rx.p, p.data(), sizeof(T) * nc * n, hipMemcpyHostToDevice, stream));
        const int blocks = (n + 63) / 64;
        if (dim == 3) {
            RayGeom<T> rg;
            rg.nnx = ncx + 1; rg.nny = ncy + 1; rg.nnz = ncz + 1;
            rg.dx = dx; rg.xmin = xmin; rg.ymin = ymin; rg.zmin = zmin; rg.xmax = xmax; rg.ymax = ymax; rg.zmax = zmax;
            rg.interp_vel = interp_vel;
            fsm_compute_slowness3d<T><<<blocks, 64, 0, stream>>>(rg, d_s.p, d_rx.p, n, d_out.p);
        } else {
            RayGeom2<T> rg2;
            rg2.nnx = ncx + 1; rg2.nnz = ncz + 1;
            rg2.dx = dx; rg2.dz = dz; rg2.xmin = xmin; rg2.zmin = zmin; rg2.xmax = xmax; rg2.zmax = zmax;
            fsm_compute_slowness2d<T><<<blocks, 64, 0, stream>>>(rg2, d_s.p, d_rx.p, n, d_out.p);
// ... 949 lines not shown
};

class MultiGrid : public GridBase {
   public:
    std::vector<std::unique_ptr<GridBase>> rep;
    int spd = 1;
    std::vector<long long> rays_off{0};
    std::vector<char> rays_pts;
    size_t pt_bytes = 12;

    template <typename Make>
    MultiGrid(int n_slots_, const std::vector<int>& devs, Make&& make) {
        n_slots = n_slots_;
        const int nd = std::min<int>((int)devs.size(), n_slots);
        spd = (n_slots + nd - 1) / nd;
        for (int r = 0; r * spd < n_slots; ++r) rep.emplace_back(make(std::min(spd, n_slots - r * spd), devs[r]));
        const GridBase& g0 = *rep[0];
        dim = g0.dim; dtype = g0.dtype; device = g0.device; n_nodes = g0.n_nodes; n_cells = g0.n_cells;
        elem_size = g0.elem_size; weno = g0.weno;
        pt_bytes = elem_size * (dim == 3 ? 3 : 2);
        niter.assign(n_slots, 0);
        niterw.assign(n_slots, 0);
        for (size_t a = 0; a < rep.size(); ++a)
            for (size_t b = 0; b < rep.size(); ++b)
                if (rep[a]->device != rep[b]->device) {
                    (void)hipSetDevice(rep[a]->device);
                    (void)hipDeviceEnablePeerAccess(rep[b]->device, 0);
                    (void)hipGetLastError();
                }
    }
    GridBase& of(int slot, int& local) const {
        if (slot < 0 || slot >= n_slots) throw ValueError("Thread number is larger than number of threads");
        local = slot % spd;
        return *rep[slot / spd];
    }
    void apply_option(const std::string& k, double value) override {
        GridBase::apply_option(k, value);
        for (auto& r : rep) r->apply_option(k, value);
    }
    void set_slowness(const void* s, size_t n, bool on_device, bool c_order = false) override {
        for (auto& r : rep) r->set_slowness(s, n, on_device, c_order);
    }
    void get_slowness(void* out, size_t n) override { rep[0]->get_slowness(out, n); }
    void validate_points(int n_tx, const void* tx, int n_rx, const void* rx) override { rep[0]->validate_points(n_tx, tx, n_rx, rx); }
    void get_tt(int slot, void* out, size_t n) override { int l; GridBase& g = of(slot, l); g.get_tt(l, out, n); }
    void* tt_device(int slot) override { int l; GridBase& g = of(slot, l); return g.tt_device(l); }
    void* tt_device_view(int slot, size_t* stride) override { int l; GridBase& g = of(slot, l); return g.tt_device_view(l, stride); }
    void interp(int slot, int n, const void* pts, void* out) override { int l; GridBase& g = of(slot, l); g.interp(l, n, pts, out); }
    void compute_slowness(int n, const void* pts, bool translated, void* out) override { rep[0]->compute_slowness(n, pts, translated, out); }
    void get_niter(int slot, int* it, int* itw) const override { int l; GridBase& g = of(slot, l); g.get_niter(l, it, itw); }
    std::string kernel_name() const override { return rep[0]->kernel_name(); }
    long long prefill_swap_count() const override { long long a = 0; for (const auto& r : rep) a += r->prefill_swap_count(); return a; }
    long long prefill_inline_count() const override { long long a = 0; for (const auto& r : rep) a += r->prefill_inline_count(); return a; }
    void stopping_stats(long long* sums, long long* missed, long long* rounds) const override {
        long long a = 0, b = 0, c = 0;
        for (const auto& r : rep) { long long x = 0, y = 0, z = 0; r->stopping_stats(&x, &y, &z); a += x; b += y; c += z; }
        if (sums) *sums = a;
        if (missed) *missed = b;
        if (rounds) *rounds = c;
    }
    void reference_change_host(const void* times, const void* field, bool parallel, void* out) override { rep[0]->reference_change_host(times, field, parallel, out); }
    void get_changes(int slot, double* first, int n_first, double* wen, int n_weno) const override {
        int l; GridBase& g = of(slot, l); g.get_changes(l, first, n_first, wen, n_weno);
    }
    void get_reference_changes(int slot, double* first, int n_first, double* wen, int n_weno) const override {
        int l; GridBase& g = of(slot, l); g.get_reference_changes(l, first, n_first, wen, n_weno);
    }
    void rays_size(size_t* n_rays, size_t* n_points) const override { *n_rays = rays_off.size() - 1; *n_points = (size_t)rays_off.back(); }
    void get_rays(long long* offsets, void* pts) const override {
        std::memcpy(offsets, rays_off.data(), rays_off.size() * sizeof(long long));
        if (!rays_pts.empty()) std::memcpy(pts, rays_pts.data(), rays_pts.size());
    }
    void raytrace_rays(int slot, int n_tx, const void* tx, const void* t0, int n_rx, const void* rx, void* tt_out) override {
        int l; GridBase& g = of(slot, l);
        g.raytrace_rays(l, n_tx, tx, t0, n_rx, rx, tt_out);
        timing = g.timing;
    }
    void raytrace_m(int slot, int n_tx, const void* tx, const void* t0, int n_rx, const void* rx, void* tt_out, bool both) override {
        int l; GridBase& g = of(slot, l);
        g.raytrace_m(l, n_tx, tx, t0, n_rx, rx, tt_out, both);
        timing = g.timing;
    }
    void slot_m_size(int slot, size_t* n_rows, size_t* nnz) const override { int l; GridBase& g = of(slot, l); g.slot_m_size(l, n_rows, nnz); }
    std::vector<long long> mm_off{0}, mm_idx;
    std::vector<char> mm_val;
    template <typename Call, typename Size, typename Get>
    void sharded_matrix_call(int n_src, const int* tx_off, const void* tx_v, const void* t0_v, const int* rx_off, const void* rx_v, void* tt_out_v,
                             Call&& call, Size&& size_of, Get&& get_of) {
        const auto wall0 = std::chrono::steady_clock::now();
        timing = Timing();
        timing.n_sources = n_src;
        mm_off.assign(1, 0); mm_idx.clear(); mm_val.clear();
        rays_off.assign(1, 0); rays_pts.clear();
        if (n_src <= 0) return;
        const char* tx = (const char*)tx_v; const char* t0 = (const char*)t0_v; const char* rx = (const char*)rx_v;
        char* tt_out = (char*)tt_out_v;
        const int nd = (int)rep.size();
        std::vector<int> first(nd + 1, 0);
        {
            long long before = 0;
            for (int d = 0; d < nd; ++d) {
                first[d] = (int)((long long)n_src * before / n_slots);
                before += rep[d]->n_slots;
            }
            first[nd] = n_src;
        }
// ... 1678 lines not shown
}
int ttcr_fsm_get_niter(ttcr_fsm_grid* g, int slot, int* niter, int* niterw) {
    return guarded_on(g, [&] { g->impl->get_niter(slot, niter, niterw); });
}
int ttcr_fsm_get_changes(ttcr_fsm_grid* g, int slot, double* first_order, int n_first, double* weno, int n_weno) {
    return guarded_on(g, [&] {
        if ((n_first > 0 && !first_order) || (n_weno > 0 && !weno) || n_first < 0 || n_weno < 0) throw ValueError("bad output buffers");
        g->impl->get_changes(slot, first_order, n_first, weno, n_weno);
    });
}
int ttcr_fsm_get_reference_changes(ttcr_fsm_grid* g, int slot, double* first_order, int n_first, double* weno, int n_weno) {
    return guarded_on(g, [&] {
        if ((n_first > 0 && !first_order) || (n_weno > 0 && !weno) || n_first < 0 || n_weno < 0) throw ValueError("bad output buffers");
        g->impl->get_reference_changes(slot, first_order, n_first, weno, n_weno);
    });
}
int ttcr_fsm_n_slots(const ttcr_fsm_grid* g) { return g->impl->n_slots; }
size_t ttcr_fsm_n_nodes(const ttcr_fsm_grid* g) { return g->impl->n_nodes; }
size_t ttcr_fsm_n_cells(const ttcr_fsm_grid* g) { return g->impl->n_cells; }

int ttcr_fsm_set_option(ttcr_fsm_grid* g, const char* key, double value) {
    return guarded_on(g, [&] { g->impl->apply_option(std::string(key ? key : ""), value); });
}

int ttcr_fsm_rays_size(const ttcr_fsm_grid* g, size_t* n_rays, size_t* n_points) {
    return guarded_on(g, [&] { g->impl->rays_size(n_rays, n_points); });
}
int ttcr_fsm_get_rays(const ttcr_fsm_grid* g, long long* offsets, void* pts) {
    return guarded_on(g, [&] { g->impl->get_rays(offsets, pts); });
}

int ttcr_fsm_last_timing(const ttcr_fsm_grid* g, ttcr_fsm_timing* out) {
    return guarded_on(g, [&] {
        const Timing& t = g->impl->timing;
        out->sweep_ms = t.sweep_ms;
        out->total_ms = t.total_ms;
        out->kernel_launches = t.launches;
        out->node_updates = t.node_updates;
        out->evaluated_updates = t.evaluated_updates;
        out->iterations = t.iterations;
        out->n_sources = t.n_sources;
    });
}

int ttcr_fsm_stopping_stats(const ttcr_fsm_grid* g, long long* reference_sums, long long* reference_sums_missed, long long* rounds) {
    return guarded_on(g, [&] { g->impl->stopping_stats(reference_sums, reference_sums_missed, rounds); });
}
int ttcr_fsm_prefill_swaps(const ttcr_fsm_grid* g, long long* swaps) {
    return guarded_on(g, [&] { if (swaps) *swaps = g->impl->prefill_swap_count(); });
}
int ttcr_fsm_prefill_inline_fills(const ttcr_fsm_grid* g, long long* fills) {
    return guarded_on(g, [&] { if (fills) *fills = g->impl->prefill_inline_count(); });
}
int ttcr_fsm_reference_change(ttcr_fsm_grid* g, const void* times, const void* field, int parallel, void* out) {
    return guarded_on(g, [&] {
        if (!times || !field || !out) throw ValueError("ttcr_fsm_reference_change: null argument");
        g->impl->reference_change_host(times, field, parallel != 0, out);
    });
}

int ttcr_fsm_last_kernel(const ttcr_fsm_grid* g, char* buf, size_t n) {
    return guarded_on(g, [&] {
        if (!buf || n == 0) throw ValueError("ttcr_fsm_last_kernel: no buffer");
        const std::string k = g->impl->kernel_name();
        std::snprintf(buf, n, "%s", k.c_str());
    });
}

#ifndef TTCR_BUILD_ID
#define TTCR_BUILD_ID "unknown"
#endif
int ttcr_fsm_unit_order(int dim, int dtype, int stage, int by_time, uint32_t nnx, uint32_t nny, uint32_t nnz, uint32_t* out,
                        size_t capacity, size_t* n_units) {
    return guarded([&] {
        if (dim != 2 && dim != 3) throw ValueError("dim must be 2 or 3");
        if (dtype != TTCR_F32 && dtype != TTCR_F64) throw ValueError("dtype must be TTCR_F32 or TTCR_F64");
        if (stage != 0 && stage != 1) throw ValueError("stage must be 0 (first order) or 1 (WENO)");
        if (nnx < 2 || nnz < 2 || (dim == 3 && nny < 2)) throw ValueError("grid needs at least two nodes per axis");
        if (!n_units) throw ValueError("null unit count");
        const uint32_t NF = dim == 3 ? nnx : nnz, NJ = dim == 3 ? nny : nnx, NK = dim == 3 ? nnz : 1;
        int PJ, PK, C;
        if (dtype == TTCR_F32) {
            PJ = dim == 3 ? TileCfg<float, 3>::PJ : TileCfg<float, 2>::PJ; PK = dim == 3 ? TileCfg<float, 3>::PK : 1;
            C = dim == 3 ? ChunkCfg<float, 3>::C : ChunkCfg<float, 2>::C;
        } else {
            PJ = dim == 3 ? TileCfg<double, 3>::PJ : TileCfg<double, 2>::PJ; PK = dim == 3 ? TileCfg<double, 3>::PK : 1;
            C = dim == 3 ? ChunkCfg<double, 3>::C : ChunkCfg<double, 2>::C;
        }
        const uint64_t npj = ((uint64_t)NJ + PJ - 1) / PJ, npk = ((uint64_t)NK + PK - 1) / PK;
        if (NF >= (1u << 30) || npj >= (1u << 14) || npk >= (1u << 14)) throw ValueError("grid too large for the patch index of the sweep kernel");
        *n_units = (size_t)(npj * npk) * (dim == 3 ? 8 : 4);
        if (!out) return;
        if (capacity < *n_units) throw ValueError("output buffer too small for the units of the launch");
        const std::vector<uint32_t> xs = fsm_xs_order(dim, (int)NF, (int)NJ, (int)NK, PJ, PK, C, stage == 0 ? 1 : 2, by_time != 0,
                                                      fsm_diag_order((int)npj, (int)npk));
        std::copy(xs.begin(), xs.end(), out);
    });
}

int ttcr_fsm_prefill_slice(int dtype, uint64_t n_el, uint32_t n_tickets, uint32_t ticket, uint64_t* slice_len, uint64_t* begin, uint64_t* end) {
    return guarded([&] {
        if (dtype != TTCR_F32 && dtype != TTCR_F64) throw ValueError("dtype must be TTCR_F32 or TTCR_F64");
        if (n_tickets == 0) throw ValueError("a launch has at least one ticket");
        const size_t slice = fsm_fill_slice_len((size_t)n_el, n_tickets, dtype == TTCR_F32 ? 4 : 2);
        size_t b = 0, e = 0;
        fsm_fill_slice_range((size_t)n_el, slice, ticket, &b, &e);
        if (slice_len) *slice_len = slice;
        if (begin) *begin = b;
        if (end) *end = e;
    });
}

const char* ttcr_fsm_build_id(void) { return TTCR_BUILD_ID; }

}
```

### ttcr_amd/csrc/fsm_kernels.h

```cpp
#pragma once
#include <hip/hip_runtime.h>
#include <stdint.h>
#include <type_traits>

#include "fsm_prefill_slices.h"

namespace ttcr_amd {

constexpr int FSM_BRICK = 16;

template <typename T> struct real_traits;
template <> struct real_traits<float> {
    static __host__ __device__ constexpr float max() { return 3.402823466e+38f; }
    static __device__ __forceinline__ float inf() { return __builtin_huge_valf(); }
};
template <> struct real_traits<double> {
    static __host__ __device__ constexpr double max() { return 1.7976931348623157e+308; }
    static __device__ __forceinline__ double inf() { return __builtin_huge_val(); }
};

__device__ __forceinline__ uint32_t idx_u32(double v) { return v < 0 ? 0u : (v >= 4294967295.0 ? 4294967295u : (uint32_t)v); }

__device__ __forceinline__ float rmin(float a, float b) { return a < b ? a : b; }
__device__ __forceinline__ double rmin(double a, double b) { return a < b ? a : b; }
// ... 365 lines not shown
            const T ak = vmin(Tt[(row - RJ) * RS + q - 1], Tt[(row + RJ) * RS + q + 1]);
            t = update3(ak, aj, af, s, dx, __builtin_amdgcn_ballot_w64(active));
        } else {
            t = variant == 1 ? update2(aj, af, s, dx) : update2_xz(aj, af, s, dx, dz);
        }
        const bool acc = active & (t < c);
        const T nv = acc ? t : c;
        dec += acc ? c - t : (T)0;
        changed |= acc;
        own[q] = nv;
        Tt[row * RS + q] = nv;
        __syncthreads();
    }

    FSM_PROF_MARK(2)
    if (FSM_ENABLE_PROF && a.prof && tid == 0) atomicAdd(a.prof + 4, 1ull);
    if (__syncthreads_or(changed)) {
        for (int f = tid; f < NT * BL; f += NT) {
            const int c = f / BL, q = f - c * BL;
            const int cj = c % PJ, ck = c / PJ;
            const int jq = j0 + cj, kq = k0 + ck;
            const int ip = L0 + q - jq - kq;
            if (jq < NJ && kq < NK && ip >= 0 && ip < NF) {
                const int i = rf ? NF - 1 - ip : ip;
                const int j = rj ? NJ - 1 - jq : jq;
                const int k = rk ? NK - 1 - kq : kq;
                const int r2 = IS3D ? (ck + 1) * RJ + cj + 1 : cj + 1;
                Tg[(size_t)(((uint32_t)k * NJ + j) * NF + i) * ts] = Tt[r2 * RS + q + 1];
            }
        }
        double accd = (double)dec;
#pragma unroll
        for (int off = 32; off > 0; off >>= 1) accd += __shfl_down(accd, off, 64);
        if ((tid & 63) == 0 && accd != 0.0) atomicAdd(a.change + slot, accd);
        FSM_PROF_MARK(3)
    }
}

template <typename T>
struct PersistArgs {
    SweepArgs<T> s;
    const uint32_t* order;
    int* sync;
    int n_patches, batch;
    unsigned long long timeout_ticks;
    int* stamp;
    const int* iter_ptr;
    unsigned long long* evals;
    int nbf, nbj, nbk;
    int dir, ndir;
    int skip;
    unsigned long long* cmap;
    int cw;
    unsigned long long* sw;
    int n_sw_groups, n_sw_sweeps;
    const T* ssh;
    size_t ssh_stride;
    T* fill_dst;
    size_t fill_slice;
    size_t fill_n;
};



__device__ __forceinline__ float ld_sc1(const float* p) {
    return __uint_as_float(__hip_atomic_load((const unsigned int*)p, __ATOMIC_RELAXED, __HIP_MEMORY_SCOPE_AGENT));
}
__device__ __forceinline__ double ld_sc1(const double* p) {
    return __longlong_as_double(__hip_atomic_load((const long long*)p, __ATOMIC_RELAXED, __HIP_MEMORY_SCOPE_AGENT));
}
__device__ __forceinline__ void st_sc1(float* p, float v) {
    __hip_atomic_store((unsigned int*)p, __float_as_uint(v), __ATOMIC_RELAXED, __HIP_MEMORY_SCOPE_AGENT);
}
__device__ __forceinline__ void st_sc1(double* p, double v) {
    __hip_atomic_store((long long*)p, __double_as_longlong(v), __ATOMIC_RELAXED, __HIP_MEMORY_SCOPE_AGENT);
}

__device__ __forceinline__ double div_h2(double x, double h2, double r2) {
    const double q0 = x * r2;
    return __builtin_fma(__builtin_fma(-q0, h2, x), r2, q0);
}

__device__ __forceinline__ float weno_fwd(float v1, float v2, float v3, float v4, float h, double r2) {
    const float eps = 1.1920928955078125e-07f;
    const float num = (float)(((double)v4 - 2.0 * (double)v3) + (double)v2);
    const float den = (float)(((double)v3 - 2.0 * (double)v2) + (double)v1);
    const float r = (eps + num * num) / (eps + den * den);
    const float w = (float)(1.0 / (1.0 + (2.0 * (double)r) * (double)r));
    const float d31 = v3 - v1;
    const double h2 = 2.0 * (double)h;
    const double ap = div_h2((1.0 - (double)w) * (double)d31, h2, r2) +
                      div_h2((double)w * ((-(double)v4 + 4.0 * (double)v3) - 3.0 * (double)v2), h2, r2);
    return v2 + h * (float)ap;
}
__device__ __forceinline__ float weno_bwd(float v0, float v1, float v2, float v3, float h, double r2) {
    const float eps = 1.1920928955078125e-07f;
    const float num = (float)(((double)v2 - 2.0 * (double)v1) + (double)v0);
    const float den = (float)(((double)v3 - 2.0 * (double)v2) + (double)v1);
    const float r = (eps + num * num) / (eps + den * den);
    const float w = (float)(1.0 / (1.0 + (2.0 * (double)r) * (double)r));
    const float d31 = v3 - v1;
    const double h2 = 2.0 * (double)h;
    const double am = div_h2((1.0 - (double)w) * (double)d31, h2, r2) +
                      div_h2((double)w * ((3.0 * (double)v2 - 4.0 * (double)v1) + (double)v0), h2, r2);
    return v2 - h * (float)am;
}
// ... 164 lines not shown
        t = 0.5 * (a1 + a2 + __builtin_sqrt(2. * fh * fh - (a1 - a2) * (a1 - a2)));
        if (t > a3) {
            t = 1. / 3. * ((a1 + a2 + a3) + __builtin_sqrt(-2. * a1 * a1 + 2. * a1 * a2 - 2. * a2 * a2 + 2. * a1 * a3 +
                                                            2. * a2 * a3 - 2. * a3 * a3 + 3. * fh * fh));
        }
    }
    return t;
}

__device__ __forceinline__ float weno_axis_fast(float m2, float m1, float c, float p1, float p2, int idx, int n) {
    const float eps = 1.1920928955078125e-07f;
    const float d0 = c - m1, d1 = p1 - c, d2 = p2 - p1, dm = m1 - m2;
    const float den = d1 - d0, nF = d2 - d1, nB = d0 - dm;
    const float y = __builtin_amdgcn_rcpf(__builtin_fmaf(den, den, eps));
    const float rF = __builtin_fmaf(nF, nF, eps) * y, rB = __builtin_fmaf(nB, nB, eps) * y;
    const float wF = __builtin_amdgcn_rcpf(__builtin_fmaf(2.0f * rF, rF, 1.0f));
    const float wB = __builtin_amdgcn_rcpf(__builtin_fmaf(2.0f * rB, rB, 1.0f));
    const float d31 = p1 - m1;
    const float F = __builtin_fmaf(0.5f, __builtin_fmaf(wF, __builtin_fmaf(3.0f, d1, -d2) - d31, d31), c);
    const float B = __builtin_fmaf(-0.5f, __builtin_fmaf(wB, __builtin_fmaf(3.0f, d0, -dm) - d31, d31), c);
    const bool c0 = idx == 0;
    const bool c1 = !c0 && idx == 1;
    const bool cn = !c0 && !c1 && idx == n;
    const bool cm = !c0 && !c1 && !cn && idx == n - 1;
    float a = cm ? B : F;
    const float t = c1 ? m1 : (cm ? p1 : B);
    a = a < t ? a : t;
    return c0 ? p1 : (cn ? m1 : a);
}
__device__ __forceinline__ float solve3_literal_fast(float a1, float a2, float a3, float fh) {
    if (a1 > a2) { const float w = a1; a1 = a2; a2 = w; }
    if (a1 > a3) { const float w = a1; a1 = a3; a3 = w; }
    if (a2 > a3) { const float w = a2; a2 = a3; a3 = w; }
    const float t1 = a1 + fh;
    const float df = a1 - a2, d3 = a3 - a1;
    const float df2 = df * df;
    const float t2 = 0.5f * ((a1 + a2) + __builtin_amdgcn_sqrtf(__builtin_fmaf(2.0f * fh, fh, -df2)));
    const float e = d3 + df;
    const float disc3 = __builtin_fmaf(3.0f * fh, fh, -(df2 + __builtin_fmaf(d3, d3, e * e)));
    const float t3 = __builtin_fmaf(1.0f / 3.0f, (d3 - df) + __builtin_amdgcn_sqrtf(disc3), a1);
    return t1 > a2 ? (t2 > a3 ? t3 : t2) : t1;
}

#ifndef FSM_POLL_SLEEP
#define FSM_POLL_SLEEP 2
#endif
#ifndef FSM_MINW
#define FSM_MINW 1
#endif
#ifndef FSM_SLAB_WORDS
#define FSM_SLAB_WORDS 32
#endif
#define FSM_FIN 0x3ffffff0
#ifndef FSM_SKIP_ABL
#define FSM_SKIP_ABL 0
#endif
#ifndef FSM_EARLY_PUB
#define FSM_EARLY_PUB 0
#endif
__device__ __forceinline__ float lane_below(float x, float edge) {
    return __uint_as_float((unsigned)__builtin_amdgcn_update_dpp((int)__float_as_uint(edge), (int)__float_as_uint(x), 0x138, 0xf, 0xf, false));
}
__device__ __forceinline__ float lane_above(float x, float edge) {
    return __uint_as_float((unsigned)__builtin_amdgcn_update_dpp((int)__float_as_uint(edge), (int)__float_as_uint(x), 0x130, 0xf, 0xf, false));
}
__device__ __forceinline__ double lane_below(double x, double edge) {
    const unsigned long long u = (unsigned long long)__double_as_longlong(x), e = (unsigned long long)__double_as_longlong(edge);
    const unsigned lo = (unsigned)__builtin_amdgcn_update_dpp((int)(unsigned)e, (int)(unsigned)u, 0x138, 0xf, 0xf, false);
    const unsigned hi = (unsigned)__builtin_amdgcn_update_dpp((int)(unsigned)(e >> 32), (int)(unsigned)(u >> 32), 0x138, 0xf, 0xf, false);
    return __longlong_as_double((long long)(((unsigned long long)hi << 32) | lo));
}
__device__ __forceinline__ double lane_above(double x, double edge) {
    const unsigned long long u = (unsigned long long)__double_as_longlong(x), e = (unsigned long long)__double_as_longlong(edge);
    const unsigned lo = (unsigned)__builtin_amdgcn_update_dpp((int)(unsigned)e, (int)(unsigned)u, 0x130, 0xf, 0xf, false);
    const unsigned hi = (unsigned)__builtin_amdgcn_update_dpp((int)(unsigned)(e >> 32), (int)(unsigned)(u >> 32), 0x130, 0xf, 0xf, false);
    return __longlong_as_double((long long)(((unsigned long long)hi << 32) | lo));
}

template <typename T, int NS> struct Pack;
template <typename T> struct Pack<T, 1> { T v[1]; };
template <typename T> struct alignas(2 * sizeof(T)) Pack<T, 2> { T v[2]; };

template <typename T, int NS>
__device__ __forceinline__ Pack<T, NS> pack_fill(T x) {
    Pack<T, NS> p;
#pragma unroll
    for (int l = 0; l < NS; ++l) p.v[l] = x;
    return p;
}
__device__ __forceinline__ Pack<float, 1> ld_sc1(const Pack<float, 1>* p) { Pack<float, 1> r; r.v[0] = ld_sc1(&p->v[0]); return r; }
__device__ __forceinline__ Pack<double, 1> ld_sc1(const Pack<double, 1>* p) { Pack<double, 1> r; r.v[0] = ld_sc1(&p->v[0]); return r; }
__device__ __forceinline__ Pack<float, 2> ld_sc1(const Pack<float, 2>* p) {
    const unsigned long long u = __hip_atomic_load((const unsigned long long*)p, __ATOMIC_RELAXED, __HIP_MEMORY_SCOPE_AGENT);
    Pack<float, 2> r;
    r.v[0] = __uint_as_float((unsigned)u);
    r.v[1] = __uint_as_float((unsigned)(u >> 32));
    return r;
}
__device__ __forceinline__ Pack<double, 2> ld_sc1(const Pack<double, 2>* p) {
    Pack<double, 2> r;
    r.v[0] = ld_sc1(&p->v[0]);
    r.v[1] = ld_sc1(&p->v[1]);
    return r;
}
__device__ __forceinline__ void st_sc1(Pack<float, 1>* p, Pack<float, 1> x) { st_sc1(&p->v[0], x.v[0]); }
__device__ __forceinline__ void st_sc1(Pack<double, 1>* p, Pack<double, 1> x) { st_sc1(&p->v[0], x.v[0]); }
__device__ __forceinline__ void st_sc1(Pack<float, 2>* p, Pack<float, 2> x) {
    const unsigned long long u = (unsigned long long)__float_as_uint(x.v[0]) | ((unsigned long long)__float_as_uint(x.v[1]) << 32);
    __hip_atomic_store((unsigned long long*)p, u, __ATOMIC_RELAXED, __HIP_MEMORY_SCOPE_AGENT);
}
__device__ __forceinline__ void st_sc1(Pack<double, 2>* p, Pack<double, 2> x) {
    st_sc1(&p->v[0], x.v[0]);
    st_sc1(&p->v[1], x.v[1]);
}

__host__ __device__ constexpr bool fsm_looped(bool is3d, int h) { return is3d && h == 1; }

__device__ __forceinline__ int kmaxp_of(int k0, int NK, int PK) { return (k0 + PK < NK ? k0 + PK : NK) - 1; }
template <typename T, int PJ, int PK, int C, bool IS3D, bool SKIP, int H, int NS, bool XS, bool PRE, int AR = 0>
__device__ __forceinline__ bool fsm_sweep_unit(const PersistArgs<T>& pa) {
    static_assert(AR == 0 || std::is_same<T, float>::value, "tolerance-grade arithmetic: fp32 kernels");
    constexpr bool LOOPED = fsm_looped(IS3D, H);
    using P = Pack<T, NS>;
    constexpr int NT = PJ * PK;
    constexpr int RJ = PJ + 2 * H;
    constexpr int NROWS = IS3D ? RJ * (PK + 2 * H) : RJ;
    constexpr int NQ = C + 2 * H;
    constexpr int RS = NQ | 1;
    constexpr int NUP = IS3D ? H * (PJ + PK) : H;
    constexpr int NDH = IS3D ? H * (PJ + PK) : H;
    constexpr int RPI = NT / C;
    constexpr int NOWN = C;
    constexpr int NHI = (NDH + RPI - 1) / RPI;
    constexpr int NUPI = (NUP + RPI - 1) / RPI;
    static_assert(NT % C == 0 && (IS3D || PK == 1) && C <= FSM_BRICK && (H == 1 || H == 2), "tile shape");
    static_assert(C - 1 <= FSM_XPAD, "the rows of a chunk are read from the sheared copies without a wrap");
    static_assert(!(SKIP && FSM_EARLY_PUB > 0), "FSM_EARLY_PUB is a tuning option of the kernels without exact skipping");
    const SweepArgs<T>& a = pa.s;
    const unsigned epoch = (unsigned)pa.iter_ptr[1] + (XS ? 0u : (unsigned)pa.dir);
    const int e2 = (int)(epoch % 3u) + 1;
    auto dec_prog = [&](int raw_) -> int { return (int)((unsigned)raw_ >> 30) == e2 ? (raw_ & 0x3fffffff) : 0; };
    auto ld_raw = [&](const int* p_) -> int { return __hip_atomic_load(p_, __ATOMIC_RELAXED, __HIP_MEMORY_SCOPE_AGENT); };
    auto ld_prog = [&](const int* p_) -> int { return dec_prog(ld_raw(p_)); };
    auto st_prog = [&](int* p_, int v_) {
        __hip_atomic_store(p_, (int)(((unsigned)e2 << 30) | (unsigned)v_), __ATOMIC_RELAXED, __HIP_MEMORY_SCOPE_AGENT);
    };
    auto ld_cmap = [&](const unsigned long long* p_) -> unsigned {
        const unsigned long long v_ = __hip_atomic_load(p_, __ATOMIC_RELAXED, __HIP_MEMORY_SCOPE_AGENT);
        return (unsigned)(v_ >> 32) == epoch ? (unsigned)v_ : 0u;
    };
    auto st_cmap = [&](unsigned long long* p_, unsigned v_) {
        __hip_atomic_store(p_, ((unsigned long long)epoch << 32) | v_, __ATOMIC_RELAXED, __HIP_MEMORY_SCOPE_AGENT);
    };

    __shared__ P Tt[NROWS * RS];
    __shared__ int s_ticket, s_abort;
    __shared__ int s_anychg;
    constexpr int SLABW = SKIP ? FSM_SLAB_WORDS : 1;
    __shared__ unsigned s_stamped[SKIP ? 9 : 1][SLABW];
    __shared__ unsigned s_slab[SLABW];
    __shared__ int s_next, s_act;
    __shared__ int s_cwi[2], s_cwl[2];
    __shared__ unsigned s_cwv[2];
    __shared__ int s_mywi;
    __shared__ unsigned s_mywv[2];
    enum { U_THR, U_RSJLO, U_RSKLO, U_RSNJ, U_RSNK, U_LCF, U_UPLCF0, U_UPLCF1, U_HIST, U_EVER, U_UCHG, U_PENDV, U_LCHG, U_N };
    __shared__ int s_u[U_N];

    int tid = threadIdx.x;
    if constexpr (LOOPED) asm volatile("" : "+v"(tid));
    unsigned long long prof_t = (FSM_ENABLE_PROF && a.prof) ? wall_clock64() : 0ull;
    unsigned long long pacc[6] = {0, 0, 0, 0, 0, 0};
    unsigned pchunks = 0;
    unsigned long long twait = 0;
    constexpr int FSM_TRACE_UNITS = FSM_ENABLE_PROF == 2 ? (1 << 20) : 65536;
    const unsigned long long trace_t0 = prof_t;
    unsigned long long* prec = nullptr;
    __shared__ unsigned long long s_pacc[FSM_ENABLE_PROF == 2 ? 8 : 1];
    if constexpr (FSM_ENABLE_PROF == 2) {
        if (tid == 0) {
            for (int q = 0; q < 6; ++q) s_pacc[q] = 0;
            s_pacc[6] = prof_t;
        }
    }
#define FSM_PMARK(slot_)                                                          \
    if constexpr (FSM_ENABLE_PROF == 2) {                                         \
        if (a.prof && tid == 0) {                                                 \
            const unsigned long long now_ = wall_clock64();                       \
            s_pacc[slot_] += now_ - s_pacc[6];                                    \
            s_pacc[6] = now_;                                                     \
        }                                                                         \
    }                                                                             \
    if (FSM_ENABLE_PROF == 1 && a.prof && tid == 0) {                             \
        const unsigned long long now_ = wall_clock64();                           \
        pacc[slot_] += now_ - prof_t;                                             \
        prof_t = now_;                                                            \
         \
        if ((slot_) < 5 && prec && pchunks < 80u) prec[pchunks * 5u + (slot_)] = now_; \
    }
    const int NF = a.g.NF, NJ = a.g.NJ, NK = a.g.NK;
    const int npj = a.g.npj;
    auto prev_sweep_counter = [&](int d, int TJ_, int TK_, int z_, int lane) -> const int* {
        const int pd = d - 1;
        int crj, crk, prj, prk;
        if (IS3D) { crj = (d >> 1) & 1; crk = (d >> 2) & 1; prj = (pd >> 1) & 1; prk = (pd >> 2) & 1; }
        else { crj = (d == 1) | (d == 2); crk = 0; prj = (pd == 1) | (pd == 2); prk = 0; }
        const int j0_ = TJ_ * PJ, k0_ = TK_ * PK;
        const int jm_ = (j0_ + PJ < NJ ? j0_ + PJ : NJ) - 1, km_ = (k0_ + PK < NK ? k0_ + PK : NK) - 1;
        int ja = j0_ - 2 * H, jb = jm_ + 2 * H, ka = k0_ - 2 * H, kb = km_ + 2 * H;
        ja = ja < 0 ? 0 : ja; jb = jb > NJ - 1 ? NJ - 1 : jb;
        ka = ka < 0 ? 0 : ka; kb = kb > NK - 1 ? NK - 1 : kb;
        const int ja2 = (crj != prj) ? NJ - 1 - jb : ja, jb2 = (crj != prj) ? NJ - 1 - ja : jb;
        const int ka2 = (crk != prk) ? NK - 1 - kb : ka, kb2 = (crk != prk) ? NK - 1 - ka : kb;
        const int tja = ja2 / PJ, ntj = jb2 / PJ - tja + 1;
        const int tka = IS3D ? ka2 / PK : 0, ntk = IS3D ? kb2 / PK - tka + 1 : 1;
        const int ia = lane & 3, ib = lane >> 2;
        if (ia >= ntj || ib >= ntk) return nullptr;
        return pa.sync + 8 + ((size_t)pd * pa.batch + z_) * pa.n_patches + ((tka + ib) * npj + tja + ia);
    };
// ... 157 lines not shown
    auto lds_row = [&](int cj, int ck) { return (IS3D ? (ck + H) * RJ + cj + H : cj + H) * RS; };
    auto nat_row = [&](int jq, int kq) {
        return ((uint32_t)(rk ? NK - 1 - kq : kq) * NJ + (rj ? NJ - 1 - jq : jq)) * NF;
    };

    const int e = tid % C, rsub = tid / C;
    int ipb[NOWN + NHI];
    uint32_t abase[NOWN + NHI];
    int lrow[NOWN + NHI];
#pragma unroll
    for (int it = 0; it < NOWN + NHI; ++it) {
        int cj, ck;
        bool ok = true;
        if (it < NOWN) {
            const int rid = rsub + RPI * it;
            cj = rid % PJ;
            ck = rid / PJ;
        } else {
            const int h = rsub + RPI * (it - NOWN);
            ok = h < NDH;
            if (IS3D) {
                if (h < H * PK) { cj = PJ + h / PK; ck = h % PK; } else { cj = (h - H * PK) % PJ; ck = PK + (h - H * PK) / PJ; }
            } else {
                cj = PJ + h; ck = 0;
            }
        }
        const int jq = j0 + cj, kq = k0 + ck;
        ok = ok && jq < NJ && kq < NK;
        const int b = H + e - jq - kq;
        ipb[it] = ok ? b : -(1 << 29);
        abase[it] = nat_row(jq, kq) + (uint32_t)(rf ? NF - 1 - b : b);
        lrow[it] = lds_row(cj, ck) + e + 2 * H;
    }
    int uipb[NUPI];
    uint32_t uabase[NUPI];
    int ulrow[NUPI];
#pragma unroll
    for (int it = 0; it < NUPI; ++it) {
        const int h = rsub + RPI * it;
        int cj, ck;
        bool ok = h < NUP;
        if (IS3D) {
            if (h < H * PK) { cj = -1 - h / PK; ck = h % PK; } else { cj = (h - H * PK) % PJ; ck = -1 - (h - H * PK) / PJ; }
        } else {
            cj = -1 - h; ck = 0;
        }
        const int jq = j0 + cj, kq = k0 + ck;
        ok = ok && jq >= 0 && jq < NJ && kq >= 0 && kq < NK;
        const int b = -1 + e - jq - kq;
        uipb[it] = ok ? b : -(1 << 29);
        uabase[it] = nat_row(jq >= 0 ? jq : 0, kq >= 0 ? kq : 0) + (uint32_t)(rf ? NF - 1 - b : b);
        ulrow[it] = (h < NUP) ? lds_row(cj, ck) + e + H - 1 : -1;
    }
    int xipb = -(1 << 29), xlrow = -1;
    uint32_t xabase = 0;
    bool x_up = false;
    if (H == 2) {
        constexpr int NX1 = IS3D ? (PJ + PK) : 1;
        static_assert(H != 2 || 3 * NX1 <= NT, "extras fit one pass");
        if (tid < 3 * NX1) {
            const bool up = tid >= NX1;
            const int dist = tid >= 2 * NX1 ? 2 : 1;
            const int h = tid % NX1;
            int cj, ck;
            if (IS3D) {
                if (h < PK) { cj = up ? -dist : PJ; ck = h; } else { cj = h - PK; ck = up ? -dist : PK; }
            } else {
                cj = up ? -dist : PJ; ck = 0;
            }
            const int jq = j0 + cj, kq = k0 + ck;
            const bool ok = jq >= 0 && jq < NJ && kq >= 0 && kq < NK;
            const int lev = up ? -2 : 1;
            const int b = lev - jq - kq;
            xipb = ok ? b : -(1 << 29);
            xabase = nat_row(jq >= 0 ? jq : 0, kq >= 0 ? kq : 0) + (uint32_t)(rf ? NF - 1 - b : b);
            xlrow = lds_row(cj, ck) + lev + H;
            x_up = up;
        }
    }

    const int m = TJ + TK;
    int Lc = Ls - (((Ls - m) % C + C) % C);

    T sv[C];
    P tv[NOWN + NHI];
    int xs_next = 0, xs_level = -(1 << 30);
    auto issue_static = [&](int L) {
        int x;
        if (L == xs_level) {
            x = xs_next;
        } else {
            x = (rev ? NF + NJ + NK - 3 - L : L) % M;
            x = x < 0 ? x + M : x;
        }
        x = __builtin_amdgcn_readfirstlane(x);
        int xlo = rev ? x - (C - 1) : x;
        if (xlo < 0) { xlo %= M; xlo = xlo < 0 ? xlo + M : xlo; }
        constexpr bool paired = IS3D;
        const uint32_t SRB = (paired ? (uint32_t)a.g.SR : (uint32_t)NJ) * (uint32_t)sizeof(T);
        const char* rowp = reinterpret_cast<const char*>(Sg + (size_t)skx_min * shear_plane(a.g)) + (size_t)(paired ? (uint32_t)xlo >> 1 : (uint32_t)xlo) * SRB;
        auto ld_row = [&](int half) -> T {
            asm volatile("" : "+s"(rowp));
            return *reinterpret_cast<const T*>(rowp + half * 16 * (int)sizeof(T) + stoff);
        };
        if constexpr (paired) {
            if ((xlo & 1) == 0) {
#pragma unroll
                for (int q = 0; q < C; ++q) {
                    sv[q] = ld_row(q & 1);
                    if (q & 1) rowp += SRB;
                }
            } else {
#pragma unroll
                for (int q = 0; q < C; ++q) {
                    if (!(q & 1)) { sv[q] = ld_row(1); rowp += SRB; } else sv[q] = ld_row(0);
                }
            }
        } else {
#pragma unroll
            for (int q = 0; q < C; ++q) {
                sv[q] = ld_row(0);
                rowp += SRB;
            }
        }
        x = rev ? x - C : x + C;
        if (x < 0 || x >= M) { x %= M; x = x < 0 ? x + M : x; }
        xs_next = x;
        xs_level = L + C;
        const int sL = sf * L;
#pragma unroll
        for (int it = 0; it < NOWN + NHI; ++it) {
            P v = PFILL;
            if ((unsigned)(L + ipb[it]) < (unsigned)NF) v = XS ? ld_sc1(Tg + (abase[it] + sL)) : Tg[abase[it] + sL];
            tv[it] = v;
        }
    };

    unsigned long long nevals = 0;

    T dec[NS];
#pragma unroll
    for (int l = 0; l < NS; ++l) dec[l] = 0;
    P carry[2 * H];
#pragma unroll
    for (int q = 0; q < 2 * H; ++q) carry[q] = PFILL;
    bool have_prev = false;
    int pref_for = -(1 << 30);
    int pending = 0;
    int n_done = 0;
    int pre_j = -1, pre_k = -1;
    int smp_j = 0, smp_k = 0;
    P uvn[NUPI];
    int uvn_for = -(1 << 30);
    int near_lo[NS], near_hi[NS];
    {
        const int jlo = rj ? NJ - 1 - jmaxp : j0, jhi = rj ? NJ - 1 - j0 : jmaxp;
        const int klo = rk ? NK - 1 - kmaxp : k0, khi = rk ? NK - 1 - k0 : kmaxp;
#pragma unroll
        for (int l = 0; l < NS; ++l) {
            const int* b6 = bb + 6 * l;
            const int b0 = rf ? NF - 1 - b6[1] : b6[0], b1 = rf ? NF - 1 - b6[0] : b6[1];
            const bool jk = !(jhi < b6[2] || jlo > b6[3] || khi < b6[4] || klo > b6[5]) && b0 <= NF - 1 && b1 >= 0;
            near_lo[l] = jk ? b0 - (C - 1) + j0 + k0 : 1;
            near_hi[l] = jk ? b1 + jmaxp + kmaxp : 0;
        }
    }
    if (!FSM_EXP_NOWAIT && XS && dir > 0 && !chase) {
        if (tid < 16) {
            const int* pp = prev_sweep_counter(dir, TJ, TK, z, tid);
            if (pp) {
                const unsigned long long t0 = wall_clock64();
                int spins = 0;
                while (ld_prog(pp) < (SKIP ? FSM_FIN : 0x3fffffff)) {
                    if ((++spins & 63) == 0) {
                        if (__hip_atomic_load(pa.sync + 4, __ATOMIC_RELAXED, __HIP_MEMORY_SCOPE_AGENT)) break;
                        if (wall_clock64() - t0 > pa.timeout_ticks) {
                            __hip_atomic_store(pa.sync + 4, 1, __ATOMIC_RELAXED, __HIP_MEMORY_SCOPE_AGENT);
                            break;
                        }
                    }
                    __builtin_amdgcn_s_sleep(8);
                }
            }
        }
        __syncthreads();
    }
    if (CHASE_OK && chase) chase_wait(Lc - C, -1, false);
    if (!SKIP) { issue_static(Lc); pref_for = Lc; }
    if constexpr (SKIP) {
        const int nsw = (pa.nbf + 31) >> 5;
        for (int w = tid; w < nsw; w += NT) s_slab[w] = 0u;
        for (int w = tid; w < 9 * SLABW; w += NT) s_stamped[w / SLABW][w % SLABW] = 0u;
        if (tid == 0) {
            s_cwi[0] = -1; s_cwi[1] = -1; s_mywi = -1;
            const int ja = j0 - H < 0 ? 0 : j0 - H, jb = jmaxp + H > NJ - 1 ? NJ - 1 : jmaxp + H;
            const int ka = k0 - H < 0 ? 0 : k0 - H, kb = kmaxp + H > NK - 1 ? NK - 1 : kmaxp + H;
            const int jlo = (rj ? NJ - 1 - jb : ja) / FSM_BRICK, jhi = (rj ? NJ - 1 - ja : jb) / FSM_BRICK;
            const int klo = (rk ? NK - 1 - kb : ka) / FSM_BRICK, khi = (rk ? NK - 1 - ka : kb) / FSM_BRICK;
            s_u[U_RSJLO] = jlo; s_u[U_RSNJ] = jhi - jlo + 1;
            s_u[U_RSKLO] = klo; s_u[U_RSNK] = khi - klo + 1;
            const int sg = pa.ndir * pa.iter_ptr[0] + dir + 1;
            s_u[U_THR] = pa.skip == 2 ? -(1 << 30) : (sg - 1 > 0 ? sg - 1 : 0);
            s_u[U_LCF] = Lc;
            const int lsj = Ls - PJ, lsk = Ls - PK, mu = TJ + TK - 1;
            s_u[U_UPLCF0] = lsj - (((lsj - mu) % C + C) % C);
            s_u[U_UPLCF1] = lsk - (((lsk - mu) % C + C) % C);
            s_u[U_HIST] = 0; s_u[U_EVER] = 0; s_u[U_UCHG] = 0; s_u[U_PENDV] = 0; s_u[U_LCHG] = 0;
        }
        __syncthreads();
        {
            const int jlo = s_u[U_RSJLO], nj = s_u[U_RSNJ], klo = s_u[U_RSKLO], nk = s_u[U_RSNK], thr = s_u[U_THR];
            const int* __restrict__ stamp = pa.stamp + (size_t)grp * pa.nbf * pa.nbj * pa.nbk;
            const int total = pa.nbf * nj * nk;
            for (int b = tid; b < total; b += NT) {
                const int bf = b % pa.nbf, jk = b / pa.nbf;
                const int bj = jlo + jk % nj, bk = klo + jk / nj;
                const int v = __hip_atomic_load(stamp + ((size_t)bk * pa.nbj + bj) * pa.nbf + bf, __ATOMIC_RELAXED, __HIP_MEMORY_SCOPE_AGENT);
                if (v >= thr) atomicOr(&s_slab[bf >> 5], 1u << (bf & 31));
            }
        }
        __syncthreads();
    }
    FSM_PMARK(5)
    const unsigned long long trace_t1 = (FSM_ENABLE_PROF && a.prof) ? wall_clock64() : 0ull;
    auto cmap_of = [&](int pidx, int e) -> unsigned long long* {
        return pa.cmap + ((((size_t)(XS ? dir : 0) * pa.batch + z) * pa.n_patches + (size_t)pidx) * 2 + e) * pa.cw;
    };
    auto slab_any = [&](int flo, int fhi) -> bool {
        const int b0 = flo / FSM_BRICK, b1 = fhi / FSM_BRICK;
        for (int w = b0 >> 5; w <= (b1 >> 5); ++w) {
            const int lo = w == (b0 >> 5) ? (b0 & 31) : 0, hi = w == (b1 >> 5) ? (b1 & 31) : 31;
            const unsigned msk = (hi == 31 ? 0xffffffffu : ((2u << hi) - 1u)) & ~((1u << lo) - 1u);
            if (s_slab[w] & msk) return true;
        }
        return false;
    };
    auto chunk_frange = [&](int L, int ext, int& flo, int& fhi) {
        int ia = L - ext - jmaxp - kmaxp, ib = L + C - 1 + ext - j0 - k0;
        ia = ia < 0 ? 0 : ia;
        ib = ib > NF - 1 ? NF - 1 : ib;
        flo = rf ? NF - 1 - ib : ia;
        fhi = rf ? NF - 1 - ia : ib;
    };
    auto up_dirty = [&](int v, int need, int e) -> bool {
        if (v >= FSM_FIN && !((v >> e) & 1)) return false;
        for (int p2 = 0; p2 < H; ++p2) {
            const int nd = need - p2 * C;
            const int ulcf = s_u[U_UPLCF0 + e];
            const int ciu = (nd - C - ulcf) / C;
            if (nd - C - ulcf < 0) continue;
            int bit;
            const int d = v >= FSM_FIN ? 4 : ((v >> 8) - nd) / C;
            if (d < 4) {
                bit = (v >> (2 * d + e)) & 1;
            } else {
                const int w = ciu >> 5;
                if (w >= pa.cw) continue;
                if (s_cwi[e] != w || s_cwl[e] < nd) {
                    s_cwl[e] = v >= FSM_FIN ? 0x7fffffff : (v >> 8);
                    const unsigned long long* um = cmap_of(e == 0 ? TK * npj + TJ - 1 : (TK - 1) * npj + TJ, e);
                    s_cwv[e] = ld_cmap(um + w);
                    s_cwi[e] = w;
                }
                bit = (s_cwv[e] >> (ciu & 31)) & 1u;
            }
            if (bit) return true;
        }
        return false;
    };
    auto poll_until = [&](const int* ptr, int want, bool& ok) -> int {
        unsigned long long t0 = 0;
        int spins = 0;
        for (;;) {
            const int v = ld_prog(ptr);
            if (v >= want) {
                if (FSM_ENABLE_PROF == 2 && spins) twait += wall_clock64() - t0;
                return v;
            }
            if (spins == 0) t0 = wall_clock64();
            if ((++spins & 63) == 0) {
                if (__hip_atomic_load(pa.sync + 4, __ATOMIC_RELAXED, __HIP_MEMORY_SCOPE_AGENT)) { ok = false; return v; }
                if (wall_clock64() - t0 > pa.timeout_ticks) {
                    __hip_atomic_store(pa.sync + 4, 1, __ATOMIC_RELAXED, __HIP_MEMORY_SCOPE_AGENT);
                    ok = false;
                    return v;
                }
            }
            __builtin_amdgcn_s_sleep(FSM_POLL_SLEEP);
        }
    };
    for (; Lc <= Le; Lc += C) {
        if constexpr (PRE) {
            pre_j = dec_prog(smp_j);
            pre_k = dec_prog(smp_k);
        }
        if constexpr (SKIP) {
            FSM_PMARK(0)
            if (tid == 0) {
                int L = Lc, act = 1, h = s_u[U_HIST];
                const int lcf = s_u[U_LCF];
                const bool follow = s_u[U_LCHG] != 0 && L <= Le;
                s_u[U_LCHG] = 0;
                for (;;) {
                    if (L > Le) { act = 0; break; }
                    if (follow) {
                        const int need8 = (L + C - 1) << 8;
                        bool ok = true;
                        if (up_j && pre_j < need8) pre_j = poll_until(up_j, need8, ok);
                        if (up_k && ok && pre_k < need8) pre_k = poll_until(up_k, need8, ok);
                        if (!ok) act = 0;
                        break;
                    }
                    const int need = L + C - 1, need8 = need << 8;
                    int vj = FSM_FIN, vk = FSM_FIN;
                    bool ok = true;
                    if (up_j) { vj = pre_j >= need8 ? pre_j : poll_until(up_j, need8, ok); pre_j = vj; }
                    if (up_k && ok) { vk = pre_k >= need8 ? pre_k : poll_until(up_k, need8, ok); pre_k = vk; }
                    if (!ok) { act = 0; break; }
                    if (L == lcf && vj >= FSM_FIN && !(vj & 1) && vk >= FSM_FIN && !(vk & 2)) {
                        bool any = false;
                        for (int w = 0; w < ((pa.nbf + 31) >> 5); ++w) any |= s_slab[w] != 0u;
                        if (!any) {
                            st_prog(my_prog, FSM_FIN);
                            L = Le + 1;
                            act = 0;
                            break;
                        }
                    }
                    int flo, fhi;
                    chunk_frange(L, H, flo, fhi);
                    bool dirty = slab_any(flo, fhi);
                    if (!dirty && up_j) dirty = up_dirty(vj, need, 0);
                    if (!dirty && up_k) dirty = up_dirty(vk, need, 1);
                    if (dirty) break;
                    if (pending) { act = 2; break; }
                    L += C;
                    h = (h << 2) & 0xff;
                    if (L > Le && s_u[U_UCHG]) {
                        s_u[U_PENDV] = FSM_FIN | s_u[U_EVER];
                    } else {
                        st_prog(my_prog, L > Le ? (FSM_FIN | s_u[U_EVER]) : ((L << 8) | h));
                    }
                }
                s_u[U_HIST] = h;
                s_next = L;
                s_act = act;
            }
            __syncthreads();
            const int act = __builtin_amdgcn_readfirstlane(s_act), Ln = __builtin_amdgcn_readfirstlane(s_next);
            if (Ln != Lc) {
                have_prev = false;
                Lc = Ln;
            }
            if (act == 2) {
                asm volatile("s_waitcnt vmcnt(0)" ::: "memory");
                __syncthreads();
                if (tid == 0) st_prog(my_prog, s_u[U_PENDV]);
                pending = 0;
                Lc -= C;
                continue;
            }
            if (act == 0) break;
        }
        const int L0 = Lc;
        const int eoff = jp + kp - L0;
        const int ea = col_ok ? (eoff > 0 ? eoff : 0) : C;
        const int eb = eoff + NF - 1 < C - 1 ? eoff + NF - 1 : C - 1;
        if constexpr (!SKIP) { FSM_PMARK(0) }

        if constexpr (!SKIP) {
        if (CHASE_OK && chase) {
            chase_wait(L0, pre_j, true);
        } else if (tid == 0 && (up_j || up_k) && !((up_j ? pre_j : 0x3fffffff) >= L0 + C - 1 && (up_k ? pre_k : 0x3fffffff) >= L0 + C - 1)) {
            const int need = L0 + C - 1;
            unsigned long long t0 = 0;
            int spins = 0;
            for (;;) {
                const int vj = up_j ? ld_prog(up_j) : need;
                const int vk = up_k ? ld_prog(up_k) : need;
                if (vj >= need && vk >= need) break;
                if (spins == 0) t0 = wall_clock64();
                if ((++spins & 63) == 0) {
                    if (__hip_atomic_load(pa.sync + 4, __ATOMIC_RELAXED, __HIP_MEMORY_SCOPE_AGENT)) break;
                    if (wall_clock64() - t0 > pa.timeout_ticks) {
                        __hip_atomic_store(pa.sync + 4, 1, __ATOMIC_RELAXED, __HIP_MEMORY_SCOPE_AGENT);
                        break;
                    }
                }
                __builtin_amdgcn_s_sleep(FSM_POLL_SLEEP);
            }
        }
        __syncthreads();
        }
        if (tid == 0) s_anychg = 0;
        FSM_PMARK(1)
        if (pref_for != L0) issue_static(L0);
        nevals += (eb >= ea) ? (unsigned)(eb - ea + 1) : 0u;

        P uv[NUPI];
        if (PRE && uvn_for == L0) {
#pragma unroll
            for (int it = 0; it < NUPI; ++it) uv[it] = uvn[it];
        } else {
#pragma unroll
            for (int it = 0; it < NUPI; ++it) {
                P v = PFILL;
                if ((unsigned)(L0 + uipb[it]) < (unsigned)NF) v = ld_sc1(Tg + (uabase[it] + sf * L0));
                uv[it] = v;
            }
        }
        P xv = PFILL;
        if (H == 2 && (unsigned)(L0 + xipb) < (unsigned)NF) {
            const P* src = Tg + (xabase + sf * L0);
            if (x_up || XS) xv = ld_sc1(src); else xv = *src;
        }
#pragma unroll
        for (int it = 0; it < NOWN + NHI; ++it)
            if (it < NOWN || rsub + RPI * (it - NOWN) < NDH) Tt[lrow[it]] = tv[it];
        if (!have_prev) {
#pragma unroll
            for (int q = 0; q < 2 * H; ++q) {
                const int ip = L0 - H + q - jp - kp;
                P v = PFILL;
                if (col_ok && (unsigned)ip < (unsigned)NF) {
                    const P* src = Tg + (colbase + (rf ? NF - 1 - ip : ip));
                    v = XS ? ld_sc1(src) : *src;
                }
                carry[q] = v;
            }
            have_prev = true;
        }
#pragma unroll
        for (int q = 0; q < 2 * H; ++q) Tt[row * RS + q] = carry[q];
        asm volatile("s_waitcnt vmcnt(0)" ::: "memory");
#pragma unroll
        for (int it = 0; it < NUPI; ++it)
            if (ulrow[it] >= 0) Tt[ulrow[it]] = uv[it];
        if (H == 2 && xlrow >= 0) Tt[xlrow] = xv;
        __syncthreads();
        if (tid == 0 && pending) st_prog(my_prog, SKIP ? s_u[U_PENDV] : pending);
        pending = 0;
        if (PRE && Lc + C <= Le) {
            const int need_n = SKIP ? (L0 + 2 * C - 1) << 8 : L0 + 2 * C - 1;
            const int sj = up_j ? __builtin_amdgcn_readfirstlane(pre_j) : 0x7fffffff;
            const int sk = up_k ? __builtin_amdgcn_readfirstlane(pre_k) : 0x7fffffff;
            if (sj >= need_n && sk >= need_n) {
#pragma unroll
                for (int it = 0; it < NUPI; ++it) {
                    P v = PFILL;
                    if ((unsigned)(L0 + C + uipb[it]) < (unsigned)NF) v = ld_sc1(Tg + (uabase[it] + sf * (L0 + C)));
                    uvn[it] = v;
                }
                uvn_for = L0 + C;
            }
        }
        if (PRE && (tid & 63) == 0 && Lc + C <= Le) {
            if (up_j) smp_j = ld_raw(up_j);
            if (up_k) smp_k = ld_raw(up_k);
        }
        if (PRE && CHASE_OK && chase_ptr && Lc + C <= Le)
            smp_j = ld_raw(chase_ptr);

        bool near_src[NS];
#pragma unroll
        for (int l = 0; l < NS; ++l) near_src[l] = L0 >= near_lo[l] && L0 <= near_hi[l];

        P own[NQ];
#pragma unroll
        for (int q = 0; q < 2 * H; ++q) own[q] = carry[q];
#pragma unroll
        for (int q = 2 * H; q < NQ; ++q) own[q] = Tt[row * RS + q];
        T sc[C];
#pragma unroll
        for (int q = 0; q < C; ++q) sc[q] = rev ? sv[C - 1 - q] : sv[q];
        FSM_PMARK(2)

        if (Lc + C <= Le) { issue_static(Lc + C); pref_for = Lc + C; }

        constexpr bool WAVE2D = !IS3D && NT == 64 && H == 1;
        P hup[WAVE2D ? C : 1], hdn[WAVE2D ? C : 1];
        if (WAVE2D) {
#pragma unroll
            for (int ee = 0; ee < C; ++ee) {
                hup[ee] = Tt[(H - 1) * RS + ee + H - 1];
                hdn[ee] = Tt[(PJ + H) * RS + ee + H + 1];
            }
        }
        bool changed = false;
        constexpr bool DUP = H == 1 && !IS3D;
        if constexpr (!DUP) {
#define FSM_SIMPLE false
#define FSM_VAR 0
#include "fsm_march_levels.inc"
#undef FSM_SIMPLE
#undef FSM_VAR
        } else {
            bool near_any = false;
#pragma unroll
            for (int l = 0; l < NS; ++l) near_any |= near_src[l];
            const bool full_wave = !near_any && __builtin_amdgcn_ballot_w64(ea == 0 && eb == C - 1) == ~0ull;
            if (!full_wave) {
#define FSM_SIMPLE false
#define FSM_VAR 0
#include "fsm_march_levels.inc"
#undef FSM_SIMPLE
#undef FSM_VAR
            } else if (variant == 1) {
#define FSM_SIMPLE true
#define FSM_VAR 1
#include "fsm_march_levels.inc"
#undef FSM_SIMPLE
#undef FSM_VAR
            } else {
#define FSM_SIMPLE true
#define FSM_VAR 2
#include "fsm_march_levels.inc"
#undef FSM_SIMPLE
#undef FSM_VAR
            }
        }
#pragma unroll
        for (int q = 0; q < 2 * H; ++q) carry[q] = own[C + q];
        FSM_PMARK(3)
        if (FSM_ENABLE_PROF) ++pchunks;

        if constexpr (SKIP) {
            const bool ej = changed && jp + H > jmaxp, ek = IS3D && changed && kp + H > kmaxp;
            const int f = (wave_any(changed) ? 1 : 0) | (wave_any(ej) ? 2 : 0) | (wave_any(ek) ? 4 : 0);
            if (f && (tid & 63) == 0) atomicOr(&s_anychg, f);
            if (!(FSM_SKIP_ABL & 2) && changed) {
                const int ip0 = L0 - jp - kp;
                const int ia = ip0 + ea, ib = ip0 + eb;
                const int ba = (rf ? NF - 1 - ib : ia) / FSM_BRICK, bb2 = (rf ? NF - 1 - ia : ib) / FSM_BRICK;
                const int my_bj = (rj ? NJ - 1 - jp : jp) / FSM_BRICK - s_u[U_RSJLO], my_bk = (rk ? NK - 1 - kp : kp) / FSM_BRICK - s_u[U_RSKLO];
                const int jk = my_bk * s_u[U_RSNJ] + my_bj;
                atomicOr(&s_stamped[jk][ba >> 5], 1u << (ba & 31));
                if (bb2 != ba) atomicOr(&s_stamped[jk][bb2 >> 5], 1u << (bb2 & 31));
            }
        } else {
            if (wave_any(changed) && (tid & 63) == 0) s_anychg = 1;
        }
        __syncthreads();
        const int chg_flags = SKIP ? __builtin_amdgcn_readfirstlane(s_anychg) : s_anychg;
        const bool any_changed = chg_flags != 0;
        if (any_changed) {
#pragma unroll
            for (int it = 0; it < NOWN; ++it) {
                const int ipm = L0 + ipb[it] - H;
                if ((unsigned)ipm < (unsigned)NF) {
                    const int rid = rsub + RPI * it;
                    const int cj = rid % PJ, ck = rid / PJ;
                    P* dst = Tg + (abase[it] + sf * (L0 - H));
                    const P v = Tt[lrow[it] - H];
                    if (XS || cj >= PJ - H || (IS3D && ck >= PK - H)) st_sc1(dst, v); else *dst = v;
                }
            }
        }
        if constexpr (SKIP) {
            if (!(FSM_SKIP_ABL & 4) && tid == 0) {
                if (any_changed) {
                    int flo, fhi;
                    chunk_frange(L0, 0, flo, fhi);
                    for (int b = flo / FSM_BRICK; b <= fhi / FSM_BRICK; ++b) s_slab[b >> 5] |= 1u << (b & 31);
                    const int ci = (L0 - s_u[U_LCF]) / C, w = ci >> 5;
                    if ((chg_flags & 6) && w < pa.cw) {
                        if (s_mywi != w) { s_mywi = w; s_mywv[0] = 0u; s_mywv[1] = 0u; }
                        for (int e2 = 0; e2 < 2; ++e2)
                            if (chg_flags & (2 << e2)) {
                                s_mywv[e2] |= 1u << (ci & 31);
                                st_cmap(cmap_of(TK * npj + TJ, e2) + w, s_mywv[e2]);
                            }
                    }
                    s_u[U_UCHG] = 1;
                    s_u[U_LCHG] = 1;
                }
                const int h2 = ((s_u[U_HIST] << 2) | (chg_flags >> 1)) & 0xff, ev2 = s_u[U_EVER] | (chg_flags >> 1);
                s_u[U_HIST] = h2;
                s_u[U_EVER] = ev2;
                s_u[U_PENDV] = Lc + C > Le ? (FSM_FIN | ev2) : (((Lc + C) << 8) | h2);
            }
        }
        if constexpr (SKIP) pending = 1;
        else pending = Lc + C > Le ? 0x3fffffff : Lc + C;
        if (FSM_EARLY_PUB > 0 && n_done < FSM_EARLY_PUB) {
            asm volatile("s_waitcnt vmcnt(0)" ::: "memory");
            __syncthreads();
            if (tid == 0) st_prog(my_prog, SKIP ? s_u[U_PENDV] : pending);
            pending = 0;
        }
        ++n_done;
        FSM_PMARK(4)
    }
    if constexpr (SKIP) {
        __syncthreads();
        if (s_u[U_UCHG]) {
            const int nsw = (pa.nbf + 31) >> 5;
            const int rs_jlo = s_u[U_RSJLO], rs_nj = s_u[U_RSNJ], rs_klo = s_u[U_RSKLO], njk = rs_nj * s_u[U_RSNK];
            int* __restrict__ stamp = pa.stamp + (size_t)grp * pa.nbf * pa.nbj * pa.nbk;
            const int sigma = pa.ndir * pa.iter_ptr[0] + dir + 1;
            for (int q = tid; q < njk * nsw * 32; q += NT) {
                const int jk = q / (nsw * 32), bf = q % (nsw * 32);
                if (bf < pa.nbf && ((s_stamped[jk][bf >> 5] >> (bf & 31)) & 1u))
                    atomicMax(stamp + ((size_t)(rs_klo + jk / rs_nj) * pa.nbj + rs_jlo + jk % rs_nj) * pa.nbf + bf, sigma);
            }
            pending = 1;
        }
    }
    if (pending) {
        asm volatile("s_waitcnt vmcnt(0)" ::: "memory");
        __syncthreads();
        if (tid == 0) st_prog(my_prog, SKIP ? s_u[U_PENDV] : pending);
    }
    if constexpr (SKIP) {
        const int sigma0 = pa.ndir * pa.iter_ptr[0] + dir;
        if (tid == 0 && pa.sw && sigma0 < pa.n_sw_sweeps)
            atomicAdd(pa.sw + (size_t)sigma0 * pa.n_sw_groups + grp, 1ull | (s_u[U_UCHG] ? (1ull << 32) : 0ull));
    }

    if (FSM_ENABLE_PROF && a.prof && tid == 0) {
        if constexpr (FSM_ENABLE_PROF == 2) {
            for (int q = 0; q < 6; ++q) atomicAdd(a.prof + q, s_pacc[q]);
            atomicAdd(a.prof + 6, 1ull);
            atomicAdd(a.prof + 7, (unsigned long long)pchunks);
        }
        if (FSM_ENABLE_PROF == 1) {
#pragma unroll
            for (int q = 0; q < 6; ++q) atomicAdd(a.prof + q, pacc[q]);
            atomicAdd(a.prof + 6, 1ull);
            atomicAdd(a.prof + 7, (unsigned long long)pchunks);
        }
        if (ticket < FSM_TRACE_UNITS) {
            unsigned long long* tr = a.prof + 8 + 4 * (size_t)ticket;
            tr[0] = trace_t0; tr[1] = FSM_ENABLE_PROF == 2 ? ((trace_t1 - trace_t0) & 0xffffffffull) | (twait << 32) : trace_t1; tr[2] = wall_clock64();
            tr[3] = (unsigned long long)TJ | ((unsigned long long)TK << 16) | ((unsigned long long)dir << 32) | ((unsigned long long)z << 40) |
                    ((unsigned long long)pchunks << 48);
        }
    }
#undef FSM_PMARK
#pragma unroll
    for (int off = 32; off > 0; off >>= 1) nevals += __shfl_down(nevals, off, 64);
#pragma unroll
    for (int l = 0; l < NS; ++l) {
        double accd = (double)dec[l];
#pragma unroll
        for (int off = 32; off > 0; off >>= 1) accd += __shfl_down(accd, off, 64);
        if ((tid & 63) == 0 && accd != 0.0) atomicAdd(a.change + grp * NS + l, accd);
        if ((tid & 63) == 0 && nevals && ((lm >> l) & 1)) atomicAdd(pa.evals + grp * NS + l, nevals);
    }
    return true;
}

template <typename T, int PJ, int PK, int C, bool IS3D, bool SKIP, int H, int NS, bool XS, bool PRE = false, int AR = 0>
#ifndef FSM_WENO_MINW
#define FSM_WENO_MINW FSM_MINW
#endif
__global__ __launch_bounds__(PJ* PK, (SKIP && IS3D && H == 1 && NS == 2 && sizeof(T) == 4) ? 3
                                     : (IS3D && H == 2 && NS == 1 && sizeof(T) == 4) ? FSM_WENO_MINW : FSM_MINW) void fsm_sweep_persistent(const PersistArgs<T> pa) {
    if constexpr (fsm_looped(IS3D, H)) {
        (void)pa;
        for (;;) {
            auto kp = __builtin_amdgcn_kernarg_segment_ptr();
            asm volatile("" : "+s"(kp));
            if (!fsm_sweep_unit<T, PJ, PK, C, IS3D, SKIP, H, NS, XS, PRE, AR>(*(const PersistArgs<T>*)kp)) break;
        }
    } else {
        fsm_sweep_unit<T, PJ, PK, C, IS3D, SKIP, H, NS, XS, PRE, AR>(pa);
    }
}

template <typename T>
struct Sweep45Args {
    T* tt;
    const T* s;
    const uint32_t* frozen;
    double* change;
    const int* slots;
    const int* lmask;
    int ts, by_group;
    int nnx, nnz;
    size_t n_nodes;
    uint32_t mask_words;
    T dx;
};

template <typename T, int NT>
__global__ __launch_bounds__(NT) void fsm_sweep45(const Sweep45Args<T> a) {
    constexpr int W = 16, C = 8;
    __shared__ T ring[NT * W];
    int slot;
    if (a.by_group) {
        const int z = blockIdx.x / a.ts, l = blockIdx.x % a.ts;
        const int grp = a.slots[z];
        if (grp < 0 || !((a.lmask[z] >> l) & 1)) return;
        slot = grp * a.ts + l;
    } else {
        slot = a.slots[blockIdx.x];
        if (slot < 0) return;
    }
    T* __restrict__ Tg = a.tt + ((size_t)(slot / a.ts) * a.n_nodes * a.ts + slot % a.ts);
    const uint32_t* __restrict__ Fz = a.frozen + (size_t)slot * a.mask_words;
// ... 763 lines not shown
                        sum = first ? v : sum + v;
                        first = false;
                    }
        }
        const int cnt = ni * nj * nk;
        sn[n] = cnt == 1 ? sum : (cnt == 2 ? (T)(0.5 * sum) : (cnt == 4 ? (T)(0.25 * sum) : (T)(0.125 * sum)));
    }
}

template <typename T>
__global__ void fsm_cells_to_nodes2d(const T* __restrict__ sc, T* __restrict__ sn, int ncx, int ncz) {
    const int nnx = ncx + 1, nnz = ncz + 1;
    const size_t N = (size_t)nnx * nnz;
    for (size_t n = blockIdx.x * (size_t)blockDim.x + threadIdx.x; n < N; n += (size_t)gridDim.x * blockDim.x) {
        const int j = n % nnz, i = n / nnz;
        int ci[2], cj[2], ni = 0, nj = 0;
        if (i < ncx) ci[ni++] = i;
        if (i > 0) ci[ni++] = i - 1;
        if (j < ncz) cj[nj++] = j;
        if (j > 0) cj[nj++] = j - 1;
        T sum = 0;
        bool first = true;
        for (int a = 0; a < ni; ++a)
            for (int b = 0; b < nj; ++b) {
                const T v = sc[(size_t)ci[a] * ncz + cj[b]];
                sum = first ? v : sum + v;
                first = false;
            }
        const int cnt = ni * nj;
        sn[n] = cnt == 1 ? sum : (cnt == 2 ? (T)(0.5 * sum) : (T)(0.25 * sum));
    }
}

template <typename T>
struct InitPoint {
    T x, y, z, t0;
    int i, j, k;
    int on_node;
};

template <typename T>
struct InitArgs {
    T* tt;
    int ts;
    const T* slowness;
    uint32_t* frozen;
    int* bbox;
    const InitPoint<T>* pts;
    int n_pts, npts;
    int nnx, nny, nnz;
    T dx, dz, xmin, ymin, zmin;
    int dim;
    int* stamp;
    int nbf, nbj, nbk;
};

template <typename T>
__device__ __forceinline__ T node_coord(T cmin, uint32_t n, T d) { return cmin + (T)n * d; }

template <typename T>
__global__ void fsm_init_source(const InitArgs<T> a) {
    const int tid = threadIdx.x;
    int lo[3] = {1 << 30, 1 << 30, 1 << 30}, hi[3] = {-1, -1, -1};
    for (int n = 0; n < a.n_pts; ++n) {
        const InitPoint<T> p = a.pts[n];
        const int npts = a.npts;
        const int b0 = p.on_node ? -npts : -(npts - 1);
        const int w = npts - b0 + 1;
        const int nbox = a.dim == 3 ? w * w * w : w * w;
        if (p.on_node && tid == 0) {
            const size_t nn = a.dim == 3 ? ((size_t)p.k * a.nny + p.j) * a.nnx + p.i : (size_t)p.i * a.nnz + p.k;
            a.tt[nn * a.ts] = p.t0;
            atomicOr(&a.frozen[nn >> 5], 1u << (nn & 31));
        }
        __syncthreads();
        for (int b = tid; b < nbox; b += blockDim.x) {
            if (a.dim == 3) {
                const int ii = p.i + b0 + b % w, jj = p.j + b0 + (b / w) % w, kk = p.k + b0 + b / (w * w);
                if (ii < 0 || ii >= a.nnx || jj < 0 || jj >= a.nny || kk < 0 || kk >= a.nnz) continue;
                if (ii == p.i && jj == p.j && kk == p.k) continue;
                const size_t m = ((size_t)kk * a.nny + jj) * a.nnx + ii;
                const T x = node_coord(a.xmin, ii, a.dx), y = node_coord(a.ymin, jj, a.dx), z = node_coord(a.zmin, kk, a.dx);
                const T d2 = (x - p.x) * (x - p.x) + (y - p.y) * (y - p.y) + (z - p.z) * (z - p.z);
                const T d = (T)__builtin_sqrt((double)d2);
                a.tt[m * a.ts] = p.t0 + d * a.slowness[m];
                atomicOr(&a.frozen[m >> 5], 1u << (m & 31));
            } else {
                const int ii = p.i + b0 + b / w, kk = p.k + b0 + b % w;
                if (ii < 0 || ii >= a.nnx || kk < 0 || kk >= a.nnz) continue;
                if (p.on_node && ii == p.i && kk == p.k) continue;
                const size_t m = (size_t)ii * a.nnz + kk;
                const T x = node_coord(a.xmin, ii, a.dx), z = node_coord(a.zmin, kk, a.dz);
                const T d2 = (x - p.x) * (x - p.x) + (z - p.z) * (z - p.z);
                const T d = (T)__builtin_sqrt((double)d2);
                T tt;
                if (p.on_node) {
                    const size_t nn = (size_t)p.i * a.nnz + p.k;
                    const T ssum = a.slowness[m] + a.slowness[nn];
                    tt = (T)((double)p.t0 + ((double)d * 0.5) * (double)ssum);
                } else {
                    tt = p.t0 + d * a.slowness[m];
                }
                a.tt[m * a.ts] = tt;
                atomicOr(&a.frozen[m >> 5], 1u << (m & 31));
            }
        }
        __syncthreads();
        const int ci[3] = {p.i, p.j, p.k};
        const int nn3[3] = {a.nnx, a.dim == 3 ? a.nny : 1, a.nnz};
        for (int d = 0; d < 3; ++d) {
            if (a.dim == 2 && d == 1) { lo[1] = 0; hi[1] = 0; continue; }
            int l = ci[d] + b0, h = ci[d] + npts;
            l = l < 0 ? 0 : l;
            h = h > nn3[d] - 1 ? nn3[d] - 1 : h;
            lo[d] = l < lo[d] ? l : lo[d];
            hi[d] = h > hi[d] ? h : hi[d];
        }
    }
    if (tid == 0) {
        if (a.dim == 3) {
            a.bbox[0] = lo[0]; a.bbox[1] = hi[0]; a.bbox[2] = lo[1]; a.bbox[3] = hi[1]; a.bbox[4] = lo[2]; a.bbox[5] = hi[2];
        } else {
            a.bbox[0] = lo[2]; a.bbox[1] = hi[2]; a.bbox[2] = lo[0]; a.bbox[3] = hi[0]; a.bbox[4] = 0; a.bbox[5] = 0;
        }
        if (a.stamp) {
            for (int bk = a.bbox[4] / FSM_BRICK; bk <= a.bbox[5] / FSM_BRICK; ++bk)
                for (int bj = a.bbox[2] / FSM_BRICK; bj <= a.bbox[3] / FSM_BRICK; ++bj)
                    for (int bf = a.bbox[0] / FSM_BRICK; bf <= a.bbox[1] / FSM_BRICK; ++bf)
                        a.stamp[((size_t)bk * a.nbj + bj) * a.nbf + bf] = 0;
        }
    }
}

template <typename T>
__device__ __forceinline__ T interp3d_pt(const T* __restrict__ Tn, int ts, T px, T py, T pz, int nnx, int nny, int nnz, T dx,
                                         T xmin, T ymin, T zmin) {
    const double small2 = 1.e-4 * 1.e-4;
    const T dy = dx, dz = dx;
    const uint32_t i = idx_u32(small2 + (double)((px - xmin) / dx));
    const uint32_t j = idx_u32(small2 + (double)((py - ymin) / dy));
    const uint32_t k = idx_u32(small2 + (double)((pz - zmin) / dz));
    auto ab = [](T v) { return v < 0 ? -v : v; };
    const bool onx = (double)ab(px - (xmin + (T)i * dx)) < small2;
    const bool ony = (double)ab(py - (ymin + (T)j * dy)) < small2;
    const bool onz = (double)ab(pz - (zmin + (T)k * dz)) < small2;
    auto cl = [](uint32_t v, int n) { return v < (uint32_t)n ? v : (uint32_t)n - 1u; };
#define TT(ii, jj, kk) Tn[(((size_t)cl(kk, nnz) * nny + cl(jj, nny)) * nnx + cl(ii, nnx)) * ts]
    T tt;
    if (onx && ony && onz) {
        tt = TT(i, j, k);
    } else if (onx && ony) {
        T t1 = TT(i, j, k), t2 = TT(i, j, k + 1);
        T w1 = (zmin + (T)(k + 1) * dz - pz) / dz, w2 = (pz - (zmin + (T)k * dz)) / dz;
        tt = t1 * w1 + t2 * w2;
    } else if (onx && onz) {
        T t1 = TT(i, j, k), t2 = TT(i, j + 1, k);
        T w1 = (ymin + (T)(j + 1) * dy - py) / dy, w2 = (py - (ymin + (T)j * dy)) / dy;
        tt = t1 * w1 + t2 * w2;
    } else if (ony && onz) {
        T t1 = TT(i, j, k), t2 = TT(i + 1, j, k);
        T w1 = (xmin + (T)(i + 1) * dx - px) / dx, w2 = (px - (xmin + (T)i * dx)) / dx;
        tt = t1 * w1 + t2 * w2;
    } else if (onx) {
        T t1 = TT(i, j, k), t2 = TT(i, j, k + 1), t3 = TT(i, j + 1, k), t4 = TT(i, j + 1, k + 1);
        T w1 = (zmin + (T)(k + 1) * dz - pz) / dz, w2 = (pz - (zmin + (T)k * dz)) / dz;
        t1 = t1 * w1 + t2 * w2;
        t2 = t3 * w1 + t4 * w2;
        w1 = (ymin + (T)(j + 1) * dy - py) / dy;
        w2 = (py - (ymin + (T)j * dy)) / dy;
        tt = t1 * w1 + t2 * w2;
    } else if (ony) {
        T t1 = TT(i, j, k), t2 = TT(i, j, k + 1), t3 = TT(i + 1, j, k), t4 = TT(i + 1, j, k + 1);
        T w1 = (zmin + (T)(k + 1) * dz - pz) / dz, w2 = (pz - (zmin + (T)k * dz)) / dz;
        t1 = t1 * w1 + t2 * w2;
        t2 = t3 * w1 + t4 * w2;
        w1 = (xmin + (T)(i + 1) * dx - px) / dx;
        w2 = (px - (xmin + (T)i * dx)) / dx;
        tt = t1 * w1 + t2 * w2;
    } else if (onz) {
        T t1 = TT(i, j, k), t2 = TT(i, j + 1, k), t3 = TT(i + 1, j, k), t4 = TT(i + 1, j + 1, k);
        T w1 = (ymin + (T)(j + 1) * dy - py) / dy, w2 = (py - (ymin + (T)j * dy)) / dy;
        t1 = t1 * w1 + t2 * w2;
// ... 798 lines not shown
```

### ttcr_amd/csrc/fsm_march_levels.inc

```
#ifndef FSM_EXP_NOEXCH
#define FSM_EXP_NOEXCH 0
#endif
#ifndef FSM_WFA
#define FSM_WFA 1
#endif
#ifndef FSM_WFS
#define FSM_WFS 1
#endif
#pragma unroll
        for (int ee = 0; ee < C; ++ee) {
            const int q = ee + H;
            const bool in_grid = FSM_SIMPLE ? true : (ee >= ea) & (ee <= eb);
            const unsigned long long grid_lanes =
                FSM_SIMPLE ? ~0ull : __builtin_amdgcn_sicmp(ea, ee, 41) & __builtin_amdgcn_sicmp(eb, ee, 39);
            const int ip = L0 + ee - jp - kp;
            const P c = own[q];
            const P fm1 = own[q - 1], fp1 = own[q + 1];
            P jm1, jp1;
            if (WAVE2D) {
#pragma unroll
                for (int l = 0; l < NS; ++l) {
                    jm1.v[l] = lane_below(own[q - 1].v[l], hup[WAVE2D ? ee : 0].v[l]);
                    jp1.v[l] = lane_above(own[q + 1].v[l], hdn[WAVE2D ? ee : 0].v[l]);
                }
            } else {
#if FSM_EXP_NOEXCH
                jm1 = own[q - 1];
#else
                jm1 = Tt[(row - 1) * RS + q - 1];
#endif
                jp1 = Tt[(row + 1) * RS + q + 1];
            }
            P km1 = PINF, kp1 = PINF;
#if FSM_EXP_NOEXCH
            if (IS3D) { km1 = own[q - 1]; kp1 = Tt[(row + RJ) * RS + q + 1]; }
#else
            if (IS3D) { km1 = Tt[(row - RJ) * RS + q - 1]; kp1 = Tt[(row + RJ) * RS + q + 1]; }
#endif
            constexpr int HH = H == 2 ? 2 : 1;
            P fm2 = PINF, fp2 = PINF, jm2 = PINF, jp2 = PINF, km2 = PINF, kp2 = PINF;
            if (H == 2) {
                fm2 = own[q - HH]; fp2 = own[q + HH];
                jm2 = Tt[(row - HH) * RS + q - HH]; jp2 = Tt[(row + HH) * RS + q + HH];
                if (IS3D) { km2 = Tt[(row - HH * RJ) * RS + q - HH]; kp2 = Tt[(row + HH * RJ) * RS + q + HH]; }
            }
            P nv;
#pragma unroll
            for (int l = 0; l < NS; ++l) {
                bool active = in_grid & ((lm >> l) & 1);
                unsigned long long live_lanes = ((lm >> l) & 1) ? grid_lanes : 0ull;
                if (!FSM_SIMPLE && near_src[l]) {
                    int ipn = ip;
                    asm volatile("" : "+v"(ipn));
                    if (active) {
                        const uint32_t n = colbase + (rf ? NF - 1 - ipn : ipn);
                        active = !((Fz[(size_t)l * a.mask_words + (n >> 5)] >> (n & 31)) & 1u);
                    }
                    live_lanes = __builtin_amdgcn_ballot_w64(active);
                }
                T t;
                if (H == 1) {
                    const T af = vmin(fm1.v[l], fp1.v[l]);
                    const T aj = vmin(jm1.v[l], jp1.v[l]);
                    if (IS3D) {
                        const T ak = vmin(km1.v[l], kp1.v[l]);
                        if constexpr (AR == 1) t = update3_fast(ak, aj, af, sc[ee], dx);
                        else t = update3(ak, aj, af, sc[ee], dx, live_lanes);
                    } else if constexpr (AR == 1) {
                        if (FSM_VAR == 1) t = update2_fast(aj, af, sc[ee], dx);
                        else if (FSM_VAR == 2) t = update2_xz(aj, af, sc[ee], dx, dz);
                        else t = variant == 1 ? update2_fast(aj, af, sc[ee], dx) : update2_xz(aj, af, sc[ee], dx, dz);
                    } else {
                        if (FSM_VAR == 1) t = update2(aj, af, sc[ee], dx);
                        else if (FSM_VAR == 2) t = update2_xz(aj, af, sc[ee], dx, dz);
                        else t = variant == 1 ? update2(aj, af, sc[ee], dx) : update2_xz(aj, af, sc[ee], dx, dz);
                    }
                } else {
                    const int in = rf ? NF - 1 - ip : ip;
                    const T hF = IS3D ? dx : (variant == 2 ? dz : dx);
                    const double r2F = IS3D ? r2x : (variant == 2 ? r2z : r2x);
                    const T cc = c.v[l];
                    T aF, aJ, aK = 0;
                    if constexpr (AR == 1 && FSM_WFA) {
                        aF = weno_axis_fast(rf ? fp2.v[l] : fm2.v[l], rf ? fp1.v[l] : fm1.v[l], cc, rf ? fm1.v[l] : fp1.v[l], rf ? fm2.v[l] : fp2.v[l], in, NF - 1);
                        aJ = weno_axis_fast(rj ? jp2.v[l] : jm2.v[l], rj ? jp1.v[l] : jm1.v[l], cc, rj ? jm1.v[l] : jp1.v[l], rj ? jm2.v[l] : jp2.v[l], jn, NJ - 1);
                        if (IS3D)
                            aK = weno_axis_fast(rk ? kp2.v[l] : km2.v[l], rk ? kp1.v[l] : km1.v[l], cc, rk ? km1.v[l] : kp1.v[l], rk ? km2.v[l] : kp2.v[l], kn, NK - 1);
                    } else if constexpr (std::is_same<T, float>::value && !FSM_WENO_PLAIN) {
                        const float vF[5] = {rf ? fp2.v[l] : fm2.v[l], rf ? fp1.v[l] : fm1.v[l], cc, rf ? fm1.v[l] : fp1.v[l], rf ? fm2.v[l] : fp2.v[l]};
                        const float vJ[5] = {rj ? jp2.v[l] : jm2.v[l], rj ? jp1.v[l] : jm1.v[l], cc, rj ? jm1.v[l] : jp1.v[l], rj ? jm2.v[l] : jp2.v[l]};
                        const float vK[5] = {rk ? kp2.v[l] : km2.v[l], rk ? kp1.v[l] : km1.v[l], cc, rk ? km1.v[l] : kp1.v[l], rk ? km2.v[l] : kp2.v[l]};
                        weno_axes<IS3D>(vF, vJ, vK, in, NF - 1, jn, NJ - 1, kn, NK - 1, hF, r2F, dx, r2x, aF, aJ, aK);
                    } else {
                        aF = weno_axis(rf ? fp2.v[l] : fm2.v[l], rf ? fp1.v[l] : fm1.v[l], cc, rf ? fm1.v[l] : fp1.v[l],
                                       rf ? fm2.v[l] : fp2.v[l], in, NF - 1, hF, r2F);
                        aJ = weno_axis(rj ? jp2.v[l] : jm2.v[l], rj ? jp1.v[l] : jm1.v[l], cc, rj ? jm1.v[l] : jp1.v[l],
                                       rj ? jm2.v[l] : jp2.v[l], jn, NJ - 1, dx, r2x);
                        if (IS3D)
                            aK = weno_axis(rk ? kp2.v[l] : km2.v[l], rk ? kp1.v[l] : km1.v[l], cc, rk ? km1.v[l] : kp1.v[l],
                                           rk ? km2.v[l] : kp2.v[l], kn, NK - 1, dx, r2x);
                    }
                    if (IS3D) {
                        if constexpr (AR == 1 && FSM_WFS) t = solve3_literal_fast(aK, aJ, aF, sc[ee] * dx);
                        else t = solve3_literal(aK, aJ, aF, sc[ee] * dx);
                    } else if constexpr (AR == 1) {
                        t = variant == 1 ? update2_fast(aJ, aF, sc[ee], dx) : update2_xz(aJ, aF, sc[ee], dx, dz);
                    } else {
                        t = variant == 1 ? update2(aJ, aF, sc[ee], dx) : update2_xz(aJ, aF, sc[ee], dx, dz);
                    }
                }
                const bool acc = active & (t < c.v[l]);
                nv.v[l] = acc ? t : c.v[l];
                dec[l] += acc ? c.v[l] - t : (T)0;
                changed |= acc;
            }
            own[q] = nv;
            Tt[row * RS + q] = nv;
#if !FSM_EXP_NOEXCH
            if (!WAVE2D) __syncthreads();
#endif
        }
```

### ttcr_amd/rgrid.py

```python
import collections
import ctypes as C
import math

import numpy as np

from . import _lib

_verbose = 0


def set_verbose(v):
    global _verbose
    _verbose = int(v)


def _ptr(a):
    return a.ctypes.data_as(C.c_void_p)


def _row_groups(a):
    key = np.ascontiguousarray(a, dtype=np.float64) + 0.0
    n = key.shape[0]
    if n == 0:
        return np.zeros(0, dtype=np.intp), np.zeros(1, dtype=np.intp), key
# ... 55 lines not shown
        self._use_pool = bool(use_thread_pool)

    def set_traveltime_from_raypath(self, traveltime_from_raypath):
        self.set_option("tt_from_rp", 1 if traveltime_from_raypath else 0)
        self.tt_from_rp = bool(traveltime_from_raypath)

    def set_option(self, key, value):
        _lib.check(self._lib.ttcr_fsm_set_option(self._h, key.encode(), float(value)))

    def set_slowness_device(self, device_ptr, n):
        _lib.check(self._lib.ttcr_fsm_set_slowness_device(self._h, C.c_void_p(int(device_ptr)), int(n)))

    def get_niter(self, thread_no=0):
        a, b = C.c_int(), C.c_int()
        _lib.check(self._lib.ttcr_fsm_get_niter(self._h, int(thread_no), C.byref(a), C.byref(b)))
        return a.value

    def get_niterw(self, thread_no=0):
        a, b = C.c_int(), C.c_int()
        _lib.check(self._lib.ttcr_fsm_get_niter(self._h, int(thread_no), C.byref(a), C.byref(b)))
        return b.value

    def get_changes(self, thread_no=0):
        n1, n2 = self.get_niter(thread_no), self.get_niterw(thread_no)
        a, b = (C.c_double * max(n1, 1))(), (C.c_double * max(n2, 1))()
        _lib.check(self._lib.ttcr_fsm_get_changes(self._h, int(thread_no), a, n1, b, n2))
        return np.array(a[:n1]), np.array(b[:n2])

    def get_reference_changes(self, thread_no=0):
        n1, n2 = self.get_niter(thread_no), self.get_niterw(thread_no)
        a, b = (C.c_double * max(n1, 1))(), (C.c_double * max(n2, 1))()
        _lib.check(self._lib.ttcr_fsm_get_reference_changes(self._h, int(thread_no), a, n1, b, n2))
        return np.array(a[:n1]), np.array(b[:n2])

    def timing(self):
        t = _lib.Timing()
        _lib.check(self._lib.ttcr_fsm_last_timing(self._h, C.byref(t)))
        return {k: getattr(t, k) for k, _ in t._fields_}

    def stopping_stats(self):
        a, b, c = C.c_longlong(0), C.c_longlong(0), C.c_longlong(0)
        _lib.check(self._lib.ttcr_fsm_stopping_stats(self._h, C.byref(a), C.byref(b), C.byref(c)))
        return {"reference_sums": a.value, "reference_sums_missed": b.value, "rounds": c.value}

    def prefill_swaps(self):
        a = C.c_longlong(0)
        _lib.check(self._lib.ttcr_fsm_prefill_swaps(self._h, C.byref(a)))
        return a.value

    def prefill_inline_fills(self):
        a = C.c_longlong(0)
        _lib.check(self._lib.ttcr_fsm_prefill_inline_fills(self._h, C.byref(a)))
        return a.value

    def reference_change(self, times, field, parallel=True):
        dt = self._dtype
        a = np.ascontiguousarray(times, dtype=dt).ravel()
        b = np.ascontiguousarray(field, dtype=dt).ravel()
        n = self.get_number_of_nodes()
        if a.size != n or b.size != n:
            raise ValueError('reference_change: fields of get_number_of_nodes() values expected')
        out = np.zeros(1, dtype=dt)
        _lib.check(self._lib.ttcr_fsm_reference_change(self._h, a.ctypes.data, b.ctypes.data, 1 if parallel else 0, out.ctypes.data))
        return out[0]

    def last_kernel(self):
        buf = C.create_string_buffer(256)
        _lib.check(self._lib.ttcr_fsm_last_kernel(self._h, buf, 256))
        return buf.value.decode()

    def _flat_tt(self, thread_no):
        if thread_no >= self._n_threads:
            raise ValueError('Thread number is larger than number of threads')
        n = self.get_number_of_nodes()
        out = np.empty(n, dtype=self._dtype)
        _lib.check(self._lib.ttcr_fsm_get_tt(self._h, int(thread_no), _ptr(out), n))
        return out

    def get_s0(self, hypo, slowness=None):
        nd = self._ndim
        hypo = np.asarray(hypo)
        if hypo.ndim != 2 or hypo.shape[1] != nd + 2:
            raise ValueError('hypo should be npts x %d' % (nd + 2))
        src = hypo[:, 2:2 + nd]
        evID = hypo[:, 0]
        eid = np.sort(np.unique(evID))
        if slowness is not None:
            self.set_slowness(slowness)
        first = np.array([int(np.nonzero(evID == e)[0][0]) for e in eid], dtype=np.int64)
        pts = np.ascontiguousarray(src[first, :], dtype=self._dtype)
        out = np.empty(max(len(eid), 1), dtype=self._dtype)
        _lib.check(self._lib.ttcr_fsm_compute_slowness(self._h, len(eid), _ptr(pts), 0, _ptr(out)))
        s0 = np.zeros((src.shape[0],))
        for n, e in enumerate(eid):
            s0[evID == e] = out[n]
        return s0

    def tt_device_ptr(self, thread_no=0):
        p = C.c_void_p()
        _lib.check(self._lib.ttcr_fsm_get_tt_device(self._h, int(thread_no), C.byref(p)))
        return p.value

    def tt_device_view(self, thread_no=0):
        p, st = C.c_void_p(), C.c_size_t()
        _lib.check(self._lib.ttcr_fsm_get_tt_device_view(self._h, int(thread_no), C.byref(p), C.byref(st)))
        return p.value, st.value
# ... 1709 lines not shown
```

Before: 97840.

## Track dirty bricks per paired source to mask clean-source updates

When two sources are swept together in one paired kernel, the dirty-brick stamps, change maps and chunk history flags are now kept separately for each source. A chunk can then skip evaluating the lane of a source whose upstream data did not change, instead of recomputing both whenever either changed. To support this it adds per-source stamp arrays, wider flag encodings, counters kept in LDS, and a grid-size check that turns pairing off when the wider level encoding would overflow. The extra bookkeeping raises LDS use, atomics and memsets, and risks lower occupancy or overhead if little masking happens.

```diff
diff --git a/include/ttcr_amd.h b/include/ttcr_amd.h
--- a/include/ttcr_amd.h
+++ b/include/ttcr_amd.h
@@ -218,11 +218,13 @@
 int ttcr_fsm_stopping_stats(const ttcr_fsm_grid* g, long long* reference_sums, long long* reference_sums_missed, long long* rounds);
 int ttcr_fsm_prefill_swaps(const ttcr_fsm_grid* g, long long* swaps);
 int ttcr_fsm_prefill_inline_fills(const ttcr_fsm_grid* g, long long* fills);
+int ttcr_fsm_masked_updates(const ttcr_fsm_grid* g, long long* masked_updates, long long* both_clean_chunks);
 int ttcr_fsm_reference_change(ttcr_fsm_grid* g, const void* times, const void* field, int parallel, void* out);
 int ttcr_fsm_last_kernel(const ttcr_fsm_grid* g, char* buf, size_t n);
 int ttcr_fsm_unit_order(int dim, int dtype, int stage, int by_time, uint32_t nnx, uint32_t nny, uint32_t nnz, uint32_t* out,
                         size_t capacity, size_t* n_units);
 int ttcr_fsm_prefill_slice(int dtype, uint64_t n_el, uint32_t n_tickets, uint32_t ticket, uint64_t* slice_len, uint64_t* begin, uint64_t* end);
+int ttcr_fsm_pair_layout_fits(int dim, uint32_t nx, uint32_t ny, uint32_t nz, int* fits);
 const char* ttcr_fsm_build_id(void);
 
 #ifdef __cplusplus
diff --git a/ttcr_amd/_lib.py b/ttcr_amd/_lib.py
--- a/ttcr_amd/_lib.py
+++ b/ttcr_amd/_lib.py
@@ -53,6 +53,8 @@
     "ttcr_fsm_stopping_stats": (_I, [_P, C.POINTER(C.c_longlong), C.POINTER(C.c_longlong), C.POINTER(C.c_longlong)]),
     "ttcr_fsm_prefill_swaps": (_I, [_P, C.POINTER(C.c_longlong)]),
     "ttcr_fsm_prefill_inline_fills": (_I, [_P, C.POINTER(C.c_longlong)]),
+    "ttcr_fsm_masked_updates": (_I, [_P, C.POINTER(C.c_longlong), C.POINTER(C.c_longlong)]),
+    "ttcr_fsm_pair_layout_fits": (_I, [_I, _U32, _U32, _U32, C.POINTER(_I)]),
     "ttcr_fsm_prefill_slice": (_I, [_I, C.c_uint64, _U32, _U32, C.POINTER(C.c_uint64), C.POINTER(C.c_uint64), C.POINTER(C.c_uint64)]),
     "ttcr_fsm_reference_change": (_I, [_P, C.c_void_p, C.c_void_p, C.c_int, C.c_void_p]),
     "ttcr_fsm_rays_size": (_I, [_P, C.POINTER(C.c_size_t), C.POINTER(C.c_size_t)]),
diff --git a/ttcr_amd/csrc/fsm_capi.hip b/ttcr_amd/csrc/fsm_capi.hip
--- a/ttcr_amd/csrc/fsm_capi.hip
+++ b/ttcr_amd/csrc/fsm_capi.hip
@@ -154,6 +154,8 @@
     }
     virtual void reference_change_host(const void* times, const void* field, bool parallel, void* out) = 0;
     int pair_by_distance = 1;
+    int source_mask = 1;
+    virtual long long masked_update_count(long long* both_clean) const { if (both_clean) *both_clean = 0; return 0; }
     virtual void set_pair_layout(int) {}
     virtual long long prefill_inline_count() const { return 0; }
     virtual long long prefill_swap_count() const { return 0; }
@@ -200,6 +202,10 @@
         else if (k == "interp_vel") interp_vel = value != 0;
         else if (k == "return_rays") return_rays = value != 0;
         else if (k == "pair_sources") pair_by_distance = value != 0;
+        else if (k == "source_mask") {
+            if (value != 0 && value != 1) throw ValueError("option 'source_mask': 0 or 1");
+            source_mask = (int)value;
+        }
         else if (k == "pair_layout") {
             if (value != -1 && value != 0 && value != 1) throw ValueError("option 'pair_layout': -1 (default), 0 or 1");
             set_pair_layout((int)value);
@@ -305,8 +311,13 @@
     int n_patches = 0;
     int* h_abort = nullptr;
     DevBuf<int> d_stamp;
+    DevBuf<int> d_stamp_src;
+    DevBuf<unsigned long long> d_mstat;
+    long long masked_updates = 0, both_clean_chunks = 0;
+    long long masked_update_count(long long* both_clean) const override { if (both_clean) *both_clean = both_clean_chunks; return masked_updates; }
     DevBuf<unsigned long long> d_cmap;
     int cmap_words = 1;
+    size_t cmap_total() const { return (size_t)n_patches * (size_t)(n_slots + 1) * (dim == 3 ? 8 : 4) * 2 * cmap_words; }
     DevBuf<unsigned long long> d_sw;
     int sw_sweeps = 0;
     DevBuf<int> d_iter;
@@ -384,6 +395,7 @@
             ns_window = NS == 2 && (long long)n_slots * patches <= (5 * pair_units_min) / 2;
         }
         if (const char* e = std::getenv("TTCR_FSM_PAIR")) { NS = (std::atoi(e) != 0 && n_slots >= 2) ? 2 : 1; ns_window = false; }
+        if (!pair_levels_fit(dim, nx, ny, nz)) { NS = 1; ns_window = false; }
         if (const char* e = std::getenv("TTCR_FSM_LAYOUT_LO")) layout_lo = std::atof(e);
         if (const char* e = std::getenv("TTCR_FSM_LAYOUT_HI")) layout_hi = std::atof(e);
         d_tt.reserve(n_nodes * tt_fields(), 64);
@@ -437,12 +449,14 @@
         nbk = (geom.NK + FSM_BRICK - 1) / FSM_BRICK;
         n_bricks = (size_t)nbf * nbj * nbk;
         d_stamp.reserve(n_bricks * n_slots);
+        if (NS == 2 || ns_window) d_stamp_src.reserve(n_bricks * (size_t)(n_slots + 1));
+        d_mstat.reserve(2);
         {
             const int PJ = dim == 3 ? TileCfg<T, 3>::PJ : TileCfg<T, 2>::PJ, PK = dim == 3 ? TileCfg<T, 3>::PK : 1;
             const int max_chunks = (geom.NF + 2 * (PJ + PK)) / 4 + 4;
             cmap_words = max_chunks / 32 + 1;
-            d_cmap.reserve((size_t)n_patches * n_slots * (dim == 3 ? 8 : 4) * 2 * cmap_words);
-            HIP_CHECK(hipMemset(d_cmap.p, 0, (size_t)n_patches * n_slots * (dim == 3 ? 8 : 4) * 2 * cmap_words * sizeof(unsigned long long)));
+            d_cmap.reserve(cmap_total());
+            HIP_CHECK(hipMemset(d_cmap.p, 0, cmap_total() * sizeof(unsigned long long)));
             sw_sweeps = (dim == 3 ? 8 : 4) * (2 * std::min(nitermax, 256) + 2);
             d_sw.reserve((size_t)sw_sweeps * n_slots);
         }
@@ -546,6 +560,9 @@
         pa.skip = skip_now(batch) ? (std::getenv("TTCR_FSM_SKIP_ALL_DIRTY") ? 2 : 1) : 0;
         pa.cmap = d_cmap.p;
         pa.cw = cmap_words;
+        pa.stamp_src = d_stamp_src.p;
+        pa.src_mask = (source_mask && NSV == 2 && d_stamp_src.p) ? 1 : 0;
+        pa.mstat = d_mstat.p;
         pa.sw = std::getenv("TTCR_FSM_NO_SW") ? nullptr : d_sw.p;
         pa.n_sw_groups = n_groups();
         pa.n_sw_sweeps = sw_sweeps;
@@ -900,6 +917,9 @@
     }
 
     int NS = 1;
+    static bool pair_levels_fit(int dim_, uint32_t nx, uint32_t ny, uint32_t nz) {
+        return dim_ == 3 ? fsm_pair_levels_fit((long long)nx + 1, (long long)ny + 1, (long long)nz + 1) : fsm_pair_levels_fit((long long)nz + 1, (long long)nx + 1, 1);
+    }
     bool ns_window = false;
     int pair_layout = -1;
     double last_eval_frac = -1;
@@ -1007,7 +1027,7 @@
         if (use_graph >= 2 || (use_graph == 1 && !persistent_now())) {
             hipGraph_t& graph = graphs[stage];
             hipGraphExec_t& graph_exec = graph_execs[stage];
-            const int key = mode * 2 + (skip_now(batch) ? 1 : 0);
+            const int key = (mode * 2 + (skip_now(batch) ? 1 : 0)) * 2 + (source_mask ? 1 : 0);
             if (!graph_exec || graph_batches[stage] != batch || graph_modes[stage] != key) {
                 if (graph_exec) { (void)hipGraphExecDestroy(graph_exec); graph_exec = nullptr; }
                 if (graph) { (void)hipGraphDestroy(graph); graph = nullptr; }
@@ -1346,6 +1366,9 @@
         HIP_CHECK(hipMemcpyAsync(d_pts.p, pts.data(), pts.size() * sizeof(InitPoint<T>), hipMemcpyHostToDevice, stream));
         for (int b = 0; b < nb; ++b)
             HIP_CHECK(hipMemsetAsync(d_stamp.p + (size_t)(slot_ids[b] / NS) * n_bricks, 0xFF, n_bricks * sizeof(int), stream));
+        if (NS == 2)
+            for (int b = 0; b < nb; ++b)
+                HIP_CHECK(hipMemsetAsync(d_stamp_src.p + (size_t)slot_ids[b] * n_bricks, 0xFF, n_bricks * sizeof(int), stream));
         std::vector<char> group_filled(n_groups(), 0);
         const bool all_slots = nb == n_slots && prefill_on();
         fill_arm = fill_in_flight = false;
@@ -1392,6 +1415,7 @@
             ia.dx = dx; ia.dz = dz; ia.xmin = xmin; ia.ymin = ymin; ia.zmin = zmin;
             ia.dim = dim;
             ia.stamp = d_stamp.p + (size_t)(slot / NS) * n_bricks;
+            ia.stamp_src = NS == 2 ? d_stamp_src.p + (size_t)slot * n_bricks : nullptr;
             ia.nbf = nbf; ia.nbj = nbj; ia.nbk = nbk;
             fsm_init_source<T><<<1, 128, 0, stream>>>(ia);
             niter[slot] = 0;
@@ -1412,7 +1436,7 @@
         const int ndir = dim == 3 ? 8 : 4;
         if (!sync_clean || launch_epoch > 0xfffff000u) {
             HIP_CHECK(hipMemsetAsync(d_sync.p, 0, sync_words * sizeof(int), stream));
-            HIP_CHECK(hipMemsetAsync(d_cmap.p, 0, (size_t)n_patches * n_slots * ndir * 2 * cmap_words * sizeof(unsigned long long), stream));
+            HIP_CHECK(hipMemsetAsync(d_cmap.p, 0, cmap_total() * sizeof(unsigned long long), stream));
             HIP_CHECK(hipStreamSynchronize(stream));
             launch_epoch = 1;
         }
@@ -1421,6 +1445,7 @@
         if (persistent_now() || weno) HIP_CHECK(hipMemsetAsync(d_sync.p + 8, 0, (sync_words - 8) * sizeof(int), stream));
         if (persistent_now() || weno) HIP_CHECK(hipMemsetAsync(d_sync.p + 4, 0, sizeof(int), stream));
         HIP_CHECK(hipMemsetAsync(d_evals.p, 0, sizeof(unsigned long long) * n_slots, stream));
+        HIP_CHECK(hipMemsetAsync(d_mstat.p, 0, sizeof(unsigned long long) * 2, stream));
         HIP_CHECK(hipMemsetAsync(d_sw.p, 0, sizeof(unsigned long long) * (size_t)sw_sweeps * n_groups(), stream));
         HIP_CHECK(hipEventRecord(ev0, stream));
         int it_total = 0;
@@ -1499,6 +1524,10 @@
                 for (int s2 : slot_ids)
                     HIP_CHECK(hipMemsetD32Async((hipDeviceptr_t)(d_stamp.p + (size_t)(s2 / NS) * n_bricks), it_total * (dim == 3 ? 8 : 4),
                                                 n_bricks, stream));
+                if (NS == 2)
+                    for (int s2 : slot_ids)
+                        HIP_CHECK(hipMemsetD32Async((hipDeviceptr_t)(d_stamp_src.p + (size_t)s2 * n_bricks), it_total * (dim == 3 ? 8 : 4),
+                                                    n_bricks, stream));
             }
         }
         if (std::getenv("TTCR_FSM_DEBUG_SW")) {
@@ -1567,6 +1596,12 @@
         if (was_persistent) {
             HIP_CHECK(hipMemcpy(h_evals, d_evals.p, sizeof(unsigned long long) * n_slots, hipMemcpyDeviceToHost));
             for (int s2 : slot_ids) timing.evaluated_updates += (long long)h_evals[s2];
+            if (NS == 2) {
+                unsigned long long ms2[2] = {0, 0};
+                HIP_CHECK(hipMemcpy(ms2, d_mstat.p, sizeof(ms2), hipMemcpyDeviceToHost));
+                masked_updates += (long long)ms2[0];
+                both_clean_chunks += (long long)ms2[1];
+            }
         } else {
             timing.evaluated_updates += timing.node_updates - node_updates_before;
         }
@@ -2622,6 +2657,12 @@
     std::string kernel_name() const override { return rep[0]->kernel_name(); }
     long long prefill_swap_count() const override { long long a = 0; for (const auto& r : rep) a += r->prefill_swap_count(); return a; }
     long long prefill_inline_count() const override { long long a = 0; for (const auto& r : rep) a += r->prefill_inline_count(); return a; }
+    long long masked_update_count(long long* both_clean) const override {
+        long long a = 0, b = 0;
+        for (const auto& r : rep) { long long y = 0; a += r->masked_update_count(&y); b += y; }
+        if (both_clean) *both_clean = b;
+        return a;
+    }
     void stopping_stats(long long* sums, long long* missed, long long* rounds) const override {
         long long a = 0, b = 0, c = 0;
         for (const auto& r : rep) { long long x = 0, y = 0, z = 0; r->stopping_stats(&x, &y, &z); a += x; b += y; c += z; }
@@ -4406,6 +4447,14 @@
 int ttcr_fsm_prefill_inline_fills(const ttcr_fsm_grid* g, long long* fills) {
     return guarded_on(g, [&] { if (fills) *fills = g->impl->prefill_inline_count(); });
 }
+int ttcr_fsm_masked_updates(const ttcr_fsm_grid* g, long long* masked_updates, long long* both_clean_chunks) {
+    return guarded_on(g, [&] {
+        long long b = 0;
+        const long long a = g->impl->masked_update_count(&b);
+        if (masked_updates) *masked_updates = a;
+        if (both_clean_chunks) *both_clean_chunks = b;
+    });
+}
 int ttcr_fsm_reference_change(ttcr_fsm_grid* g, const void* times, const void* field, int parallel, void* out) {
     return guarded_on(g, [&] {
         if (!times || !field || !out) throw ValueError("ttcr_fsm_reference_change: null argument");
@@ -4465,6 +4514,13 @@
     });
 }
 
+int ttcr_fsm_pair_layout_fits(int dim, uint32_t nx, uint32_t ny, uint32_t nz, int* fits) {
+    return guarded([&] {
+        if (dim != 2 && dim != 3) throw ValueError("dim must be 2 or 3");
+        if (fits) *fits = GridT<float>::pair_levels_fit(dim, nx, ny, nz) ? 1 : 0;
+    });
+}
+
 const char* ttcr_fsm_build_id(void) { return TTCR_BUILD_ID; }
 
 }
diff --git a/ttcr_amd/csrc/fsm_kernels.h b/ttcr_amd/csrc/fsm_kernels.h
--- a/ttcr_amd/csrc/fsm_kernels.h
+++ b/ttcr_amd/csrc/fsm_kernels.h
@@ -441,6 +441,9 @@
     int skip;
     unsigned long long* cmap;
     int cw;
+    int* stamp_src;
+    int src_mask;
+    unsigned long long* mstat;
     unsigned long long* sw;
     int n_sw_groups, n_sw_sweeps;
     const T* ssh;
@@ -711,6 +714,8 @@
 #define FSM_SLAB_WORDS 32
 #endif
 #define FSM_FIN 0x3ffffff0
+__host__ __device__ constexpr int fsm_flag_bits(bool skip, int ns) { return skip && ns == 2 ? 16 : 8; }
+__host__ __device__ constexpr bool fsm_pair_levels_fit(long long nf, long long nj, long long nk) { return nf + nj + nk - 2 + 16 < 16382; }
 #ifndef FSM_SKIP_ABL
 #define FSM_SKIP_ABL 0
 #endif
@@ -816,14 +821,21 @@
     __shared__ int s_ticket, s_abort;
     __shared__ int s_anychg;
     constexpr int SLABW = SKIP ? FSM_SLAB_WORDS : 1;
-    __shared__ unsigned s_stamped[SKIP ? 9 : 1][SLABW];
-    __shared__ unsigned s_slab[SLABW];
+    constexpr bool SRCM = SKIP && NS == 2;
+    constexpr int NSL = SRCM ? 2 : 1;
+    constexpr int FBITS = fsm_flag_bits(SKIP, NS);
+    constexpr int FPC = FBITS / 4;
+    constexpr int FMASK = (1 << FBITS) - 1;
+    constexpr int EDGE_J = SRCM ? 0x5 : 0x1, EDGE_K = SRCM ? 0xa : 0x2;
+    __shared__ unsigned s_stamped[SKIP ? 9 : 1][NSL * SLABW];
+    __shared__ unsigned s_slab[SRCM ? 3 : 1][SLABW];
     __shared__ int s_next, s_act;
-    __shared__ int s_cwi[2], s_cwl[2];
-    __shared__ unsigned s_cwv[2];
+    __shared__ int s_msk;
+    __shared__ int s_cwi[2 * NSL], s_cwl[2 * NSL];
+    __shared__ unsigned s_cwv[2 * NSL];
     __shared__ int s_mywi;
-    __shared__ unsigned s_mywv[2];
-    enum { U_THR, U_RSJLO, U_RSKLO, U_RSNJ, U_RSNK, U_LCF, U_UPLCF0, U_UPLCF1, U_HIST, U_EVER, U_UCHG, U_PENDV, U_LCHG, U_N };
+    __shared__ unsigned s_mywv[2 * NSL];
+    enum { U_THR, U_RSJLO, U_RSKLO, U_RSNJ, U_RSNK, U_LCF, U_UPLCF0, U_UPLCF1, U_HIST, U_EVER, U_UCHG, U_PENDV, U_LCHG, U_BOTHC, U_SRCM, U_N };
     __shared__ int s_u[U_N];
 
     int tid = threadIdx.x;
@@ -1087,6 +1099,20 @@
         uabase[it] = nat_row(jq >= 0 ? jq : 0, kq >= 0 ? kq : 0) + (uint32_t)(rf ? NF - 1 - b : b);
         ulrow[it] = (h < NUP) ? lds_row(cj, ck) + e + H - 1 : -1;
     }
+    constexpr bool UPLDS = SRCM && H == 1;
+    __shared__ int s_up[UPLDS ? 3 * NUPI + 1 : 1][UPLDS ? NT : 1];
+    if constexpr (UPLDS) {
+#pragma unroll
+        for (int it = 0; it < NUPI; ++it) {
+            s_up[3 * it][tid] = uipb[it];
+            s_up[3 * it + 1][tid] = (int)uabase[it];
+            s_up[3 * it + 2][tid] = ulrow[it];
+        }
+        s_up[3 * NUPI][tid] = (int)stoff;
+    }
+    auto up_ipb = [&](int it) -> int { if constexpr (UPLDS) return s_up[3 * it][tid]; else return uipb[it]; };
+    auto up_abase = [&](int it) -> uint32_t { if constexpr (UPLDS) return (uint32_t)s_up[3 * it + 1][tid]; else return uabase[it]; };
+    auto up_lrow = [&](int it) -> int { if constexpr (UPLDS) return s_up[3 * it + 2][tid]; else return ulrow[it]; };
     int xipb = -(1 << 29), xlrow = -1;
     uint32_t xabase = 0;
     bool x_up = false;
@@ -1134,9 +1160,11 @@
         constexpr bool paired = IS3D;
         const uint32_t SRB = (paired ? (uint32_t)a.g.SR : (uint32_t)NJ) * (uint32_t)sizeof(T);
         const char* rowp = reinterpret_cast<const char*>(Sg + (size_t)skx_min * shear_plane(a.g)) + (size_t)(paired ? (uint32_t)xlo >> 1 : (uint32_t)xlo) * SRB;
+        uint32_t so = stoff;
+        if constexpr (UPLDS) so = (uint32_t)s_up[3 * NUPI][tid];
         auto ld_row = [&](int half) -> T {
             asm volatile("" : "+s"(rowp));
-            return *reinterpret_cast<const T*>(rowp + half * 16 * (int)sizeof(T) + stoff);
+            return *reinterpret_cast<const T*>(rowp + half * 16 * (int)sizeof(T) + so);
         };
         if constexpr (paired) {
             if ((xlo & 1) == 0) {
@@ -1171,7 +1199,9 @@
         }
     };
 
-    unsigned long long nevals = 0;
+    __shared__ unsigned s_cnt[SRCM ? 2 : 1][NT];
+    s_cnt[0][tid] = 0u;
+    if constexpr (SRCM) s_cnt[1][tid] = 0u;
 
     T dec[NS];
 #pragma unroll
@@ -1223,11 +1253,11 @@
     if (CHASE_OK && chase) chase_wait(Lc - C, -1, false);
     if (!SKIP) { issue_static(Lc); pref_for = Lc; }
     if constexpr (SKIP) {
-        const int nsw = (pa.nbf + 31) >> 5;
-        for (int w = tid; w < nsw; w += NT) s_slab[w] = 0u;
-        for (int w = tid; w < 9 * SLABW; w += NT) s_stamped[w / SLABW][w % SLABW] = 0u;
+        for (int w = tid; w < (SRCM ? 3 : 1) * SLABW; w += NT) s_slab[w / SLABW][w % SLABW] = 0u;
+        for (int w = tid; w < 9 * NSL * SLABW; w += NT) s_stamped[w / (NSL * SLABW)][w % (NSL * SLABW)] = 0u;
         if (tid == 0) {
-            s_cwi[0] = -1; s_cwi[1] = -1; s_mywi = -1;
+            for (int q = 0; q < 2 * NSL; ++q) s_cwi[q] = -1;
+            s_mywi = -1;
             const int ja = j0 - H < 0 ? 0 : j0 - H, jb = jmaxp + H > NJ - 1 ? NJ - 1 : jmaxp + H;
             const int ka = k0 - H < 0 ? 0 : k0 - H, kb = kmaxp + H > NK - 1 ? NK - 1 : kmaxp + H;
             const int jlo = (rj ? NJ - 1 - jb : ja) / FSM_BRICK, jhi = (rj ? NJ - 1 - ja : jb) / FSM_BRICK;
@@ -1240,7 +1270,8 @@
             const int lsj = Ls - PJ, lsk = Ls - PK, mu = TJ + TK - 1;
             s_u[U_UPLCF0] = lsj - (((lsj - mu) % C + C) % C);
             s_u[U_UPLCF1] = lsk - (((lsk - mu) % C + C) % C);
-            s_u[U_HIST] = 0; s_u[U_EVER] = 0; s_u[U_UCHG] = 0; s_u[U_PENDV] = 0; s_u[U_LCHG] = 0;
+            s_u[U_HIST] = 0; s_u[U_EVER] = 0; s_u[U_UCHG] = 0; s_u[U_PENDV] = 0; s_u[U_LCHG] = 0; s_u[U_BOTHC] = 0;
+            s_u[U_SRCM] = SRCM ? pa.src_mask : 0;
         }
         __syncthreads();
         {
@@ -1250,8 +1281,18 @@
             for (int b = tid; b < total; b += NT) {
                 const int bf = b % pa.nbf, jk = b / pa.nbf;
                 const int bj = jlo + jk % nj, bk = klo + jk / nj;
-                const int v = __hip_atomic_load(stamp + ((size_t)bk * pa.nbj + bj) * pa.nbf + bf, __ATOMIC_RELAXED, __HIP_MEMORY_SCOPE_AGENT);
-                if (v >= thr) atomicOr(&s_slab[bf >> 5], 1u << (bf & 31));
+                const size_t bi = ((size_t)bk * pa.nbj + bj) * pa.nbf + bf;
+                const int v = __hip_atomic_load(stamp + bi, __ATOMIC_RELAXED, __HIP_MEMORY_SCOPE_AGENT);
+                if (v >= thr) atomicOr(&s_slab[0][bf >> 5], 1u << (bf & 31));
+                if constexpr (SRCM) {
+                    if (pa.src_mask) {
+                        const size_t nb = (size_t)pa.nbf * pa.nbj * pa.nbk;
+                        const int v0 = __hip_atomic_load(pa.stamp_src + (size_t)(2 * grp) * nb + bi, __ATOMIC_RELAXED, __HIP_MEMORY_SCOPE_AGENT);
+                        const int v1 = __hip_atomic_load(pa.stamp_src + (size_t)(2 * grp + 1) * nb + bi, __ATOMIC_RELAXED, __HIP_MEMORY_SCOPE_AGENT);
+                        if (v0 >= thr) atomicOr(&s_slab[1][bf >> 5], 1u << (bf & 31));
+                        if (v1 >= thr) atomicOr(&s_slab[2][bf >> 5], 1u << (bf & 31));
+                    }
+                }
             }
         }
         __syncthreads();
@@ -1259,14 +1300,14 @@
     FSM_PMARK(5)
     const unsigned long long trace_t1 = (FSM_ENABLE_PROF && a.prof) ? wall_clock64() : 0ull;
     auto cmap_of = [&](int pidx, int e) -> unsigned long long* {
-        return pa.cmap + ((((size_t)(XS ? dir : 0) * pa.batch + z) * pa.n_patches + (size_t)pidx) * 2 + e) * pa.cw;
+        return pa.cmap + ((((size_t)(XS ? dir : 0) * pa.batch + z) * pa.n_patches + (size_t)pidx) * (2 * NSL) + e) * pa.cw;
     };
-    auto slab_any = [&](int flo, int fhi) -> bool {
+    auto slab_any = [&](int which, int flo, int fhi) -> bool {
         const int b0 = flo / FSM_BRICK, b1 = fhi / FSM_BRICK;
         for (int w = b0 >> 5; w <= (b1 >> 5); ++w) {
             const int lo = w == (b0 >> 5) ? (b0 & 31) : 0, hi = w == (b1 >> 5) ? (b1 & 31) : 31;
             const unsigned msk = (hi == 31 ? 0xffffffffu : ((2u << hi) - 1u)) & ~((1u << lo) - 1u);
-            if (s_slab[w] & msk) return true;
+            if (s_slab[which][w] & msk) return true;
         }
         return false;
     };
@@ -1277,31 +1318,38 @@
         flo = rf ? NF - 1 - ib : ia;
         fhi = rf ? NF - 1 - ia : ib;
     };
-    auto up_dirty = [&](int v, int need, int e) -> bool {
-        if (v >= FSM_FIN && !((v >> e) & 1)) return false;
+    constexpr int SRC_ALL = (1 << NSL) - 1;
+    auto edge_bits = [&](int flags, int e) -> int {
+        return SRCM ? (((flags >> e) & 1) | (((flags >> (2 + e)) & 1) << 1)) : ((flags >> e) & 1);
+    };
+    auto up_dirty = [&](int v, int need, int e) -> int {
+        if (v >= FSM_FIN && !edge_bits(v, e)) return 0;
+        int bits = 0;
         for (int p2 = 0; p2 < H; ++p2) {
             const int nd = need - p2 * C;
             const int ulcf = s_u[U_UPLCF0 + e];
             const int ciu = (nd - C - ulcf) / C;
             if (nd - C - ulcf < 0) continue;
-            int bit;
-            const int d = v >= FSM_FIN ? 4 : ((v >> 8) - nd) / C;
+            const int d = v >= FSM_FIN ? 4 : ((v >> FBITS) - nd) / C;
             if (d < 4) {
-                bit = (v >> (2 * d + e)) & 1;
+                bits |= edge_bits(v >> (FPC * d), e);
             } else {
                 const int w = ciu >> 5;
                 if (w >= pa.cw) continue;
-                if (s_cwi[e] != w || s_cwl[e] < nd) {
-                    s_cwl[e] = v >= FSM_FIN ? 0x7fffffff : (v >> 8);
-                    const unsigned long long* um = cmap_of(e == 0 ? TK * npj + TJ - 1 : (TK - 1) * npj + TJ, e);
-                    s_cwv[e] = ld_cmap(um + w);
-                    s_cwi[e] = w;
+                for (int l = 0; l < NSL; ++l) {
+                    const int fi = 2 * l + e;
+                    if (s_cwi[fi] != w || s_cwl[fi] < nd) {
+                        s_cwl[fi] = v >= FSM_FIN ? 0x7fffffff : (v >> FBITS);
+                        const unsigned long long* um = cmap_of(e == 0 ? TK * npj + TJ - 1 : (TK - 1) * npj + TJ, fi);
+                        s_cwv[fi] = ld_cmap(um + w);
+                        s_cwi[fi] = w;
+                    }
+                    bits |= (int)((s_cwv[fi] >> (ciu & 31)) & 1u) << l;
                 }
-                bit = (s_cwv[e] >> (ciu & 31)) & 1u;
-            }
-            if (bit) return true;
-        }
-        return false;
+            }
+            if (bits == SRC_ALL) break;
+        }
+        return bits;
     };
     auto poll_until = [&](const int* ptr, int want, bool& ok) -> int {
         unsigned long long t0 = 0;
@@ -1334,27 +1382,28 @@
             if (tid == 0) {
                 int L = Lc, act = 1, h = s_u[U_HIST];
                 const int lcf = s_u[U_LCF];
-                const bool follow = s_u[U_LCHG] != 0 && L <= Le;
+                const int lchg = s_u[U_LCHG];
+                const bool follow = lchg != 0 && L <= Le;
                 s_u[U_LCHG] = 0;
                 for (;;) {
                     if (L > Le) { act = 0; break; }
                     if (follow) {
-                        const int need8 = (L + C - 1) << 8;
+                        const int need8 = (L + C - 1) << FBITS;
                         bool ok = true;
                         if (up_j && pre_j < need8) pre_j = poll_until(up_j, need8, ok);
                         if (up_k && ok && pre_k < need8) pre_k = poll_until(up_k, need8, ok);
                         if (!ok) act = 0;
                         break;
                     }
-                    const int need = L + C - 1, need8 = need << 8;
+                    const int need = L + C - 1, need8 = need << FBITS;
                     int vj = FSM_FIN, vk = FSM_FIN;
                     bool ok = true;
                     if (up_j) { vj = pre_j >= need8 ? pre_j : poll_until(up_j, need8, ok); pre_j = vj; }
                     if (up_k && ok) { vk = pre_k >= need8 ? pre_k : poll_until(up_k, need8, ok); pre_k = vk; }
                     if (!ok) { act = 0; break; }
-                    if (L == lcf && vj >= FSM_FIN && !(vj & 1) && vk >= FSM_FIN && !(vk & 2)) {
+                    if (L == lcf && vj >= FSM_FIN && !(vj & EDGE_J) && vk >= FSM_FIN && !(vk & EDGE_K)) {
                         bool any = false;
-                        for (int w = 0; w < ((pa.nbf + 31) >> 5); ++w) any |= s_slab[w] != 0u;
+                        for (int w = 0; w < ((pa.nbf + 31) >> 5); ++w) any |= s_slab[0][w] != 0u;
                         if (!any) {
                             st_prog(my_prog, FSM_FIN);
                             L = Le + 1;
@@ -1364,18 +1413,36 @@
                     }
                     int flo, fhi;
                     chunk_frange(L, H, flo, fhi);
-                    bool dirty = slab_any(flo, fhi);
-                    if (!dirty && up_j) dirty = up_dirty(vj, need, 0);
-                    if (!dirty && up_k) dirty = up_dirty(vk, need, 1);
+                    bool dirty = slab_any(0, flo, fhi);
+#pragma nounroll
+                    for (int e2 = 0; e2 < 2 && !dirty; ++e2)
+                        if (e2 == 0 ? up_j != nullptr : up_k != nullptr) dirty = up_dirty(e2 == 0 ? vj : vk, need, e2) != 0;
                     if (dirty) break;
                     if (pending) { act = 2; break; }
                     L += C;
-                    h = (h << 2) & 0xff;
+                    h = (h << FPC) & FMASK;
                     if (L > Le && s_u[U_UCHG]) {
                         s_u[U_PENDV] = FSM_FIN | s_u[U_EVER];
                     } else {
-                        st_prog(my_prog, L > Le ? (FSM_FIN | s_u[U_EVER]) : ((L << 8) | h));
+                        st_prog(my_prog, L > Le ? (FSM_FIN | s_u[U_EVER]) : ((L << FBITS) | h));
                     }
+                }
+                if constexpr (SRCM) {
+                    int msk = SRC_ALL;
+                    if (act == 1 && s_u[U_SRCM] && lm == SRC_ALL) {
+                        msk = follow ? lchg : 0;
+                        if (msk != SRC_ALL) {
+                            int flo, fhi;
+                            chunk_frange(L, H, flo, fhi);
+                            for (int l = 0; l < NS; ++l)
+                                if (!((msk >> l) & 1) && ((L >= near_lo[l] && L <= near_hi[l]) || slab_any(1 + l, flo, fhi))) msk |= 1 << l;
+#pragma nounroll
+                            for (int e2 = 0; e2 < 2 && msk != SRC_ALL; ++e2)
+                                if (e2 == 0 ? up_j != nullptr : up_k != nullptr) msk |= up_dirty(e2 == 0 ? pre_j : pre_k, L + C - 1, e2);
+                            if (msk == 0) { msk = SRC_ALL; s_u[U_BOTHC] += 1; }
+                        }
+                    }
+                    s_msk = msk;
                 }
                 s_u[U_HIST] = h;
                 s_next = L;
@@ -1430,8 +1497,6 @@
         if (tid == 0) s_anychg = 0;
         FSM_PMARK(1)
         if (pref_for != L0) issue_static(L0);
-        nevals += (eb >= ea) ? (unsigned)(eb - ea + 1) : 0u;
-
         P uv[NUPI];
         if (PRE && uvn_for == L0) {
 #pragma unroll
@@ -1440,7 +1505,7 @@
 #pragma unroll
             for (int it = 0; it < NUPI; ++it) {
                 P v = PFILL;
-                if ((unsigned)(L0 + uipb[it]) < (unsigned)NF) v = ld_sc1(Tg + (uabase[it] + sf * L0));
+                if ((unsigned)(L0 + up_ipb(it)) < (unsigned)NF) v = ld_sc1(Tg + (up_abase(it) + sf * L0));
                 uv[it] = v;
             }
         }
@@ -1470,20 +1535,23 @@
         asm volatile("s_waitcnt vmcnt(0)" ::: "memory");
 #pragma unroll
         for (int it = 0; it < NUPI; ++it)
-            if (ulrow[it] >= 0) Tt[ulrow[it]] = uv[it];
+        {
+            const int ur = up_lrow(it);
+            if (ur >= 0) Tt[ur] = uv[it];
+        }
         if (H == 2 && xlrow >= 0) Tt[xlrow] = xv;
         __syncthreads();
         if (tid == 0 && pending) st_prog(my_prog, SKIP ? s_u[U_PENDV] : pending);
         pending = 0;
         if (PRE && Lc + C <= Le) {
-            const int need_n = SKIP ? (L0 + 2 * C - 1) << 8 : L0 + 2 * C - 1;
+            const int need_n = SKIP ? (L0 + 2 * C - 1) << FBITS : L0 + 2 * C - 1;
             const int sj = up_j ? __builtin_amdgcn_readfirstlane(pre_j) : 0x7fffffff;
             const int sk = up_k ? __builtin_amdgcn_readfirstlane(pre_k) : 0x7fffffff;
             if (sj >= need_n && sk >= need_n) {
 #pragma unroll
                 for (int it = 0; it < NUPI; ++it) {
                     P v = PFILL;
-                    if ((unsigned)(L0 + C + uipb[it]) < (unsigned)NF) v = ld_sc1(Tg + (uabase[it] + sf * (L0 + C)));
+                    if ((unsigned)(L0 + C + up_ipb(it)) < (unsigned)NF) v = ld_sc1(Tg + (up_abase(it) + sf * (L0 + C)));
                     uvn[it] = v;
                 }
                 uvn_for = L0 + C;
@@ -1521,7 +1589,17 @@
                 hdn[ee] = Tt[(PJ + H) * RS + ee + H + 1];
             }
         }
-        bool changed = false;
+        bool chg[NS];
+#pragma unroll
+        for (int l = 0; l < NS; ++l) chg[l] = false;
+        int lmc = lm;
+        if constexpr (SRCM) lmc = lm & __builtin_amdgcn_readfirstlane(s_msk);
+        if (eb >= ea) {
+            atomicAdd(&s_cnt[0][tid], (unsigned)(eb - ea + 1));
+            if constexpr (SRCM) {
+                if (lmc != lm) atomicAdd(&s_cnt[1][tid], (unsigned)(eb - ea + 1));
+            }
+        }
         constexpr bool DUP = H == 1 && !IS3D;
         if constexpr (!DUP) {
 #define FSM_SIMPLE false
@@ -1559,9 +1637,17 @@
         FSM_PMARK(3)
         if (FSM_ENABLE_PROF) ++pchunks;
 
+        bool changed = false;
+#pragma unroll
+        for (int l = 0; l < NS; ++l) changed |= chg[l];
         if constexpr (SKIP) {
-            const bool ej = changed && jp + H > jmaxp, ek = IS3D && changed && kp + H > kmaxp;
-            const int f = (wave_any(changed) ? 1 : 0) | (wave_any(ej) ? 2 : 0) | (wave_any(ek) ? 4 : 0);
+            int f = 0;
+#pragma unroll
+            for (int l = 0; l < NSL; ++l) {
+                const bool c = SRCM ? chg[l] : changed;
+                const bool ej = c && jp + H > jmaxp, ek = IS3D && c && kp + H > kmaxp;
+                f |= ((wave_any(c) ? 1 : 0) | (wave_any(ej) ? 2 : 0) | (wave_any(ek) ? 4 : 0)) << (3 * l);
+            }
             if (f && (tid & 63) == 0) atomicOr(&s_anychg, f);
             if (!(FSM_SKIP_ABL & 2) && changed) {
                 const int ip0 = L0 - jp - kp;
@@ -1569,8 +1655,10 @@
                 const int ba = (rf ? NF - 1 - ib : ia) / FSM_BRICK, bb2 = (rf ? NF - 1 - ia : ib) / FSM_BRICK;
                 const int my_bj = (rj ? NJ - 1 - jp : jp) / FSM_BRICK - s_u[U_RSJLO], my_bk = (rk ? NK - 1 - kp : kp) / FSM_BRICK - s_u[U_RSKLO];
                 const int jk = my_bk * s_u[U_RSNJ] + my_bj;
-                atomicOr(&s_stamped[jk][ba >> 5], 1u << (ba & 31));
-                if (bb2 != ba) atomicOr(&s_stamped[jk][bb2 >> 5], 1u << (bb2 & 31));
+                unsigned sb = 1u;
+                if constexpr (SRCM) sb = (chg[0] ? 1u : 0u) | (chg[1] ? 2u : 0u);
+                atomicOr(&s_stamped[jk][(NSL * ba) >> 5], sb << ((NSL * ba) & 31));
+                if (bb2 != ba) atomicOr(&s_stamped[jk][(NSL * bb2) >> 5], sb << ((NSL * bb2) & 31));
             }
         } else {
             if (wave_any(changed) && (tid & 63) == 0) s_anychg = 1;
@@ -1593,26 +1681,37 @@
         }
         if constexpr (SKIP) {
             if (!(FSM_SKIP_ABL & 4) && tid == 0) {
+                const int eflags = SRCM ? (((chg_flags >> 1) & 3) | (((chg_flags >> 4) & 3) << 2)) : (chg_flags >> 1);
+                const int schg = SRCM ? ((chg_flags & 1) | (((chg_flags >> 3) & 1) << 1)) : (chg_flags & 1);
                 if (any_changed) {
                     int flo, fhi;
                     chunk_frange(L0, 0, flo, fhi);
-                    for (int b = flo / FSM_BRICK; b <= fhi / FSM_BRICK; ++b) s_slab[b >> 5] |= 1u << (b & 31);
+                    for (int b = flo / FSM_BRICK; b <= fhi / FSM_BRICK; ++b) {
+                        s_slab[0][b >> 5] |= 1u << (b & 31);
+                        if constexpr (SRCM) {
+                            if (schg & 1) s_slab[1][b >> 5] |= 1u << (b & 31);
+                            if (schg & 2) s_slab[2][b >> 5] |= 1u << (b & 31);
+                        }
+                    }
                     const int ci = (L0 - s_u[U_LCF]) / C, w = ci >> 5;
-                    if ((chg_flags & 6) && w < pa.cw) {
-                        if (s_mywi != w) { s_mywi = w; s_mywv[0] = 0u; s_mywv[1] = 0u; }
-                        for (int e2 = 0; e2 < 2; ++e2)
-                            if (chg_flags & (2 << e2)) {
+                    if (eflags && w < pa.cw) {
+                        if (s_mywi != w) {
+                            s_mywi = w;
+                            for (int e2 = 0; e2 < 2 * NSL; ++e2) s_mywv[e2] = 0u;
+                        }
+                        for (int e2 = 0; e2 < 2 * NSL; ++e2)
+                            if (eflags & (1 << e2)) {
                                 s_mywv[e2] |= 1u << (ci & 31);
                                 st_cmap(cmap_of(TK * npj + TJ, e2) + w, s_mywv[e2]);
                             }
                     }
                     s_u[U_UCHG] = 1;
-                    s_u[U_LCHG] = 1;
+                    s_u[U_LCHG] = schg;
                 }
-                const int h2 = ((s_u[U_HIST] << 2) | (chg_flags >> 1)) & 0xff, ev2 = s_u[U_EVER] | (chg_flags >> 1);
+                const int h2 = ((s_u[U_HIST] << FPC) | eflags) & FMASK, ev2 = s_u[U_EVER] | eflags;
                 s_u[U_HIST] = h2;
                 s_u[U_EVER] = ev2;
-                s_u[U_PENDV] = Lc + C > Le ? (FSM_FIN | ev2) : (((Lc + C) << 8) | h2);
+                s_u[U_PENDV] = Lc + C > Le ? (FSM_FIN | ev2) : (((Lc + C) << FBITS) | h2);
             }
         }
         if constexpr (SKIP) pending = 1;
@@ -1635,8 +1734,18 @@
             const int sigma = pa.ndir * pa.iter_ptr[0] + dir + 1;
             for (int q = tid; q < njk * nsw * 32; q += NT) {
                 const int jk = q / (nsw * 32), bf = q % (nsw * 32);
-                if (bf < pa.nbf && ((s_stamped[jk][bf >> 5] >> (bf & 31)) & 1u))
-                    atomicMax(stamp + ((size_t)(rs_klo + jk / rs_nj) * pa.nbj + rs_jlo + jk % rs_nj) * pa.nbf + bf, sigma);
+                if (bf >= pa.nbf) continue;
+                const size_t bi = ((size_t)(rs_klo + jk / rs_nj) * pa.nbj + rs_jlo + jk % rs_nj) * pa.nbf + bf;
+                const unsigned sbits = s_stamped[jk][(NSL * bf) >> 5] >> ((NSL * bf) & 31);
+                const unsigned b0 = sbits & 1u, b1 = SRCM ? (sbits >> 1) & 1u : 0u;
+                if (b0 | b1) atomicMax(stamp + bi, sigma);
+                if constexpr (SRCM) {
+                    if (s_u[U_SRCM]) {
+                        const size_t nb = (size_t)pa.nbf * pa.nbj * pa.nbk;
+                        if (b0) atomicMax(pa.stamp_src + (size_t)(2 * grp) * nb + bi, sigma);
+                        if (b1) atomicMax(pa.stamp_src + (size_t)(2 * grp + 1) * nb + bi, sigma);
+                    }
+                }
             }
             pending = 1;
         }
@@ -1672,15 +1781,23 @@
         }
     }
 #undef FSM_PMARK
+    unsigned nevals = s_cnt[0][tid];
 #pragma unroll
     for (int off = 32; off > 0; off >>= 1) nevals += __shfl_down(nevals, off, 64);
+    if constexpr (SRCM) {
+        unsigned nmasked = s_cnt[1][tid];
+#pragma unroll
+        for (int off = 32; off > 0; off >>= 1) nmasked += __shfl_down(nmasked, off, 64);
+        if ((tid & 63) == 0 && nmasked) atomicAdd(pa.mstat, (unsigned long long)nmasked);
+        if (tid == 0 && s_u[U_BOTHC]) atomicAdd(pa.mstat + 1, (unsigned long long)s_u[U_BOTHC]);
+    }
 #pragma unroll
     for (int l = 0; l < NS; ++l) {
         double accd = (double)dec[l];
 #pragma unroll
         for (int off = 32; off > 0; off >>= 1) accd += __shfl_down(accd, off, 64);
         if ((tid & 63) == 0 && accd != 0.0) atomicAdd(a.change + grp * NS + l, accd);
-        if ((tid & 63) == 0 && nevals && ((lm >> l) & 1)) atomicAdd(pa.evals + grp * NS + l, nevals);
+        if ((tid & 63) == 0 && nevals && ((lm >> l) & 1)) atomicAdd(pa.evals + grp * NS + l, (unsigned long long)nevals);
     }
     return true;
 }
@@ -2550,6 +2667,7 @@
     T dx, dz, xmin, ymin, zmin;
     int dim;
     int* stamp;
+    int* stamp_src;
     int nbf, nbj, nbk;
 };
 
@@ -2624,8 +2742,10 @@
         if (a.stamp) {
             for (int bk = a.bbox[4] / FSM_BRICK; bk <= a.bbox[5] / FSM_BRICK; ++bk)
                 for (int bj = a.bbox[2] / FSM_BRICK; bj <= a.bbox[3] / FSM_BRICK; ++bj)
-                    for (int bf = a.bbox[0] / FSM_BRICK; bf <= a.bbox[1] / FSM_BRICK; ++bf)
+                    for (int bf = a.bbox[0] / FSM_BRICK; bf <= a.bbox[1] / FSM_BRICK; ++bf) {
                         a.stamp[((size_t)bk * a.nbj + bj) * a.nbf + bf] = 0;
+                        if (a.stamp_src) a.stamp_src[((size_t)bk * a.nbj + bj) * a.nbf + bf] = 0;
+                    }
         }
     }
 }
diff --git a/ttcr_amd/csrc/fsm_march_levels.inc b/ttcr_amd/csrc/fsm_march_levels.inc
--- a/ttcr_amd/csrc/fsm_march_levels.inc
+++ b/ttcr_amd/csrc/fsm_march_levels.inc
@@ -47,8 +47,8 @@
             P nv;
 #pragma unroll
             for (int l = 0; l < NS; ++l) {
-                bool active = in_grid & ((lm >> l) & 1);
-                unsigned long long live_lanes = ((lm >> l) & 1) ? grid_lanes : 0ull;
+                bool active = in_grid & ((lmc >> l) & 1);
+                unsigned long long live_lanes = ((lmc >> l) & 1) ? grid_lanes : 0ull;
                 if (!FSM_SIMPLE && near_src[l]) {
                     int ipn = ip;
                     asm volatile("" : "+v"(ipn));
@@ -112,7 +112,7 @@
                 const bool acc = active & (t < c.v[l]);
                 nv.v[l] = acc ? t : c.v[l];
                 dec[l] += acc ? c.v[l] - t : (T)0;
-                changed |= acc;
+                chg[l] |= acc;
             }
             own[q] = nv;
             Tt[row * RS + q] = nv;
diff --git a/ttcr_amd/rgrid.py b/ttcr_amd/rgrid.py
--- a/ttcr_amd/rgrid.py
+++ b/ttcr_amd/rgrid.py
@@ -131,6 +131,11 @@
         a = C.c_longlong(0)
         _lib.check(self._lib.ttcr_fsm_prefill_inline_fills(self._h, C.byref(a)))
         return a.value
+
+    def masked_updates(self):
+        a, b = C.c_longlong(0), C.c_longlong(0)
+        _lib.check(self._lib.ttcr_fsm_masked_updates(self._h, C.byref(a), C.byref(b)))
+        return {"masked_updates": a.value, "both_clean_chunks": b.value}
 
     def reference_change(self, times, field, parallel=True):
         dt = self._dtype
```

New measurement: 91980. 0.94x the previous value.
